# MichaelVorndran/InconsistencyMasks

Measured on AMD Instinct MI355X. Metric: images/sec per IM generation (ensemble infer + IM build + 1 train epoch), 256x256, higher is better.
Workload: dtype f16; 1 GPU; ISIC-2018 binary 256x256x3, 2-model IM ensemble, tiny U-Net alpha=0.5 on MI355X (configs[1]); outputs=1, unlabeled_images=2335, unlabeled_images_per_gpu=2335, labeled_images=259, n_models=2, infer_batch=584, infer_batch_rule=functions.infer_batch_size: 584 at alpha<=0.5 else 128; short tail spread, train_batch_per_gpu=32, global_batch=32, parallelism=dp1, epoch_steps=80, kept=2307, train_images=2566

## Files before the change

inconsistencymasks_amd/csrc/imk_conv.hip:

```cpp
#include <cstdlib>
#include "imk_kernels.h"
#include "imk_elem.h"

#include "imk_stage.h"
#include "imk_switches.h"

#ifndef IMK_INF_WAVES
#define IMK_INF_WAVES 4
#endif
IMK_STAMP_TABLE(conv)
IMK_WGSTAMP_TABLE(conv)

namespace {


struct ImkConvGeom { int tiles_x, tiles_y, mt_total, nc8, nc8p, n_pass, ps, nsp; unsigned magic_tx, magic_pi; };
__host__ __device__ inline size_t imk_chain_w2_offset(size_t stage1_bytes, size_t out_bytes) {
    return ((stage1_bytes > out_bytes ? stage1_bytes : out_bytes) + 15) & ~(size_t)15;
}

template <int TH, int MT, int LM, bool CHAIN = false>
__device__ __forceinline__ void conv_mfma_body(const ImkConvArgs &a, const ImkConvGeom &gm, int bx, int by) {
    const int tiles_x = gm.tiles_x, tiles_y = gm.tiles_y, mt_total = gm.mt_total, nc8 = gm.nc8, nc8p = gm.nc8p;
    const int n_pass = gm.n_pass, ps = gm.ps, nsp = gm.nsp;
    constexpr int NW = 4, NT = 64 * NW;
    constexpr int P = TH / NW;
    extern __shared__ __attribute__((aligned(16))) uint8_t smem[];
    const int ks3 = (a.ksize == 3);
    const int halo = ks3 ? 1 : 0;
    const int T = ks3 ? 9 : 1;
    const int HT = TH + 2 * halo, WT = TW + 2 * halo;
    uint8_t *s_tile = smem;
    float *s_aff = reinterpret_cast<float *>(smem + (size_t)HT * WT * ps * 16);
    f16 *s_w = reinterpret_cast<f16 *>(s_aff + 4 * a.x.cs_in);
    f16 *s_w2 = reinterpret_cast<f16 *>(smem + imk_chain_w2_offset((size_t)HT * WT * ps * 16 + 4 * (size_t)a.x.cs_in * sizeof(float) +
                                                                   (size_t)MT * nsp * 1024, (size_t)TH * 16 * (MT * 16 + 8) * sizeof(f16)));
    const int t = threadIdx.x;
    const int H = a.H, W = a.W;
    const int per_img = tiles_x * tiles_y;
    const int tb = gm.magic_pi ? (int)(((unsigned long long)(unsigned)bx * gm.magic_pi) >> 32) : bx / per_img;
    const PTile tc = ptile_at(tb, bx - tb * per_img, tiles_x, gm.magic_tx);
    const PSrc<LM> src = psrc_of<LM, 0>(a.x, tc, halo, HT, WT, H, W);
    const int ns_total = n_pass * nsp;

    IMK_STAMP_BEGIN(conv, 10000 + LM * 1000 + MT * 100 + n_pass * 10 + ks3);
    stage_affine_table(a.x, s_aff);
    bool aff_pending = (LM != LM_RAW && LM != LM_U8);

    const int lane = t & 63, wave = t >> 6, n = lane & 15, g = lane >> 4;
    const int ct0 = by * MT;
    int base[P];
#pragma unroll
    for (int p = 0; p < P; ++p) base[p] = ((wave * P + p) * WT + n) * ps * 16;
    f32x4 acc[MT][P];
#pragma unroll
    for (int m = 0; m < MT; ++m)
#pragma unroll
        for (int p = 0; p < P; ++p) acc[m][p] = f32x4{0, 0, 0, 0};
    for (int pass = 0; pass < n_pass; ++pass) {
        const int c8_lo = pass * nc8p;
        const int nc8_cur = min(nc8p, nc8 - c8_lo);
        if (pass) __syncthreads();
        {
            const int n16m = nsp * 64;
            if (CHAIN && pass == 0) {
                const int nc8_2 = a.cs_out / 8;
                const int n16 = ((a.cout2 + 15) / 16) * imk_cdiv_d(nc8_2, imk_pass_chunks(nc8_2)) * 64;
                for (int j = t; j < n16; j += NT)
                    __builtin_amdgcn_global_load_lds((const __attribute__((address_space(1))) void *)(a.wpk2 + (size_t)j * 8),
                                                     (__attribute__((address_space(3))) void *)(s_w2 + (size_t)(j - lane) * 8), 16, 0, 0);
            }
#pragma unroll
            for (int m = 0; m < MT; ++m) {
                int ct = by * MT + m;
                if (ct >= mt_total) ct = mt_total - 1;
                const f16 *src = a.wpk + ((size_t)ct * ns_total + (size_t)pass * nsp) * 512;
                f16 *dstm = s_w + (size_t)m * n16m * 8;
                for (int j = t; j < n16m; j += NT)
                    __builtin_amdgcn_global_load_lds((const __attribute__((address_space(1))) void *)(src + (size_t)j * 8),
                                                     (__attribute__((address_space(3))) void *)(dstm + (size_t)(j - lane) * 8), 16, 0, 0);
            }
        }
        const int n_items = HT * WT * nc8_cur;
        if constexpr (LM == LM_U8) {
            for (int i = t; i < n_items; i += NT) {
                const int pix = i / nc8_cur, c8 = i - pix * nc8_cur;
                const int py = pix / WT, px = pix - py * WT;
                const int y = tc.ty0 + py - halo, x = tc.tx0 + px - halo;
                f16x8 v = {0, 0, 0, 0, 0, 0, 0, 0};
                if (y >= 0 && y < H && x >= 0 && x < W) v = load_chunk(a.x, tc.b, y, x, H, W, c8_lo + c8, s_aff);
                *reinterpret_cast<f16x8 *>(s_tile + (pix * ps + c8) * 16) = v;
            }
        } else {
            constexpr int BATCH = 4;
            const int mg_c = (65536 + nc8_cur - 1) / nc8_cur, mg_w = (65536 + WT - 1) / WT;
            const int n_batches = (n_items + BATCH * NT - 1) / (BATCH * NT);
            for (int bt = 0; bt < n_batches; ++bt) {
                const int i0 = t + bt * BATCH * NT;
                RawChunk<LM> r[BATCH];
                int dst[BATCH], c8s[BATCH];
                unsigned ok = 0;
#pragma unroll
                for (int u = 0; u < BATCH; ++u) {
                    const int i = i0 + u * NT;
                    const int ii = i < n_items ? i : t;
                    const int pix = (ii * mg_c) >> 16;
                    const int c8 = ii - pix * nc8_cur;
                    const int py = (pix * mg_w) >> 16, px = pix - py * WT;
                    dst[u] = i < n_items ? (pix * ps + c8) * 16 : -1;
                    c8s[u] = c8_lo + c8;
                    if (psrc_load<LM, 0>(src, py, px, c8s[u], W, r[u])) ok |= 1u << u;
                }
                if (aff_pending) { __syncthreads(); aff_pending = false; }
#pragma unroll
                for (int u = 0; u < BATCH; ++u) {
                    if (dst[u] >= 0) {
                        f16x8 v = raw_transform<LM>(r[u], s_aff, a.x.cs_in, c8s[u], a.x.cin, a.x.u8_div);
                        if (!(ok & (1u << u))) v = f16x8{0, 0, 0, 0, 0, 0, 0, 0};
                        *reinterpret_cast<f16x8 *>(s_tile + dst[u]) = v;
                    }
                }
            }
        }
        __builtin_amdgcn_s_waitcnt(0x0F70);
        __syncthreads();
        if (pass == 0) IMK_STAMP(1);

        const int nq = T * nc8p;
        int q = g;
        const int mg_q = (65536 + nc8p - 1) / nc8p;
        auto k_loop = [&]() {
            int sn = 0;
            const f16 *wsrc[MT];
#pragma unroll
            for (int m = 0; m < MT; ++m) {
                wsrc[m] = s_w + ((size_t)m * nsp * 64 + lane) * 8;
            }
            typedef __attribute__((ext_vector_type(4))) unsigned u32x4;
            auto load_frag = [&](f16x8 (&af)[MT], f16x8 (&bf)[P]) {
                const int tap = (q * mg_q) >> 16, c8 = q - tap * nc8p;
                const int ty = ks3 ? (tap * 11) >> 5 : 0, tx = ks3 ? tap - 3 * ty : 0;
                const bool vq = (q < nq) && (c8 < nc8_cur);
                const int off = vq ? ((ty * WT + tx) * ps + c8) * 16 : 0;
                const unsigned live = sn < nsp ? 0xFFFFFFFFu : 0u;
                const int sc = min(sn, nsp - 1);
#pragma unroll
                for (int m = 0; m < MT; ++m) {
                    const u32x4 w = *reinterpret_cast<const u32x4 *>(wsrc[m] + (size_t)sc * 512) & live;
                    af[m] = __builtin_bit_cast(f16x8, w);
                }
#pragma unroll
                for (int p = 0; p < P; ++p) bf[p] = *reinterpret_cast<const f16x8 *>(s_tile + base[p] + off);
                ++sn;
                q += 4;
            };
            auto mma = [&](const f16x8 (&af)[MT], const f16x8 (&bf)[P]) {
#pragma unroll
                for (int p = 0; p < P; ++p)
#pragma unroll
                    for (int m = 0; m < MT; ++m) acc[m][p] = __builtin_amdgcn_mfma_f32_16x16x32_f16(af[m], bf[p], acc[m][p], 0, 0, 0);
            };
            f16x8 a0[MT], b0[P], a1[MT], b1[P];
            load_frag(a0, b0);
            for (int s = 0; s < nsp; s += 2) {
                load_frag(a1, b1);
                mma(a0, b0);
                load_frag(a0, b0);
                mma(a1, b1);
            }
        };
        k_loop();
        if (pass == 0) IMK_STAMP(2);
    }
    IMK_STAMP(3);

    const int x = tc.tx0 + n;
    const int my = H - 1 - tc.ty0, mx = W - 1 - tc.tx0;
    float s1[MT][4], s2[MT][4];
#pragma unroll
    for (int m = 0; m < MT; ++m)
#pragma unroll
        for (int r = 0; r < 4; ++r) s1[m][r] = s2[m][r] = 0.f;
    const bool dystat = !CHAIN && (a.epi != EP_RELU) && a.dystat_z && a.stats_partial;
    const bool want_stats = !CHAIN && (((a.epi == EP_RELU) && a.stats_partial) || dystat);
    float bias[MT][4];
#pragma unroll
    for (int m = 0; m < MT; ++m)
#pragma unroll
        for (int r = 0; r < 4; ++r) {
            const int co = (ct0 + m) * 16 + 4 * g + r;
            bias[m][r] = (a.epi == EP_RELU && a.bias && co < a.cout) ? a.bias[co] : 0.f;
        }
    constexpr int OPITCH = MT * 16 + 8;
    f16 *s_out = reinterpret_cast<f16 *>(smem);
    __syncthreads();
    auto write_tile = [&](auto EPI_T, auto STAT_T, const f32x4 (&ac)[MT][P], const float (&bs)[MT][4], int cs_o) {
        constexpr int EPI = decltype(EPI_T)::value;
        constexpr int STAT = decltype(STAT_T)::value;
#pragma unroll
        for (int m = 0; m < MT; ++m) {
            const int co0 = (ct0 + m) * 16 + 4 * g;
            f16x4 mk[P], zz[P];
            if (EPI == EP_MASK || STAT == 2) {
#pragma unroll
                for (int p = 0; p < P; ++p) {
                    const unsigned o = __umul24(__umul24(min(wave * P + p, my), W) + min(n, mx), (unsigned)cs_o * 2u) + (co0 < cs_o ? co0 * 2 : 0);
                    if (EPI == EP_MASK) mk[p] = *reinterpret_cast<const f16x4 *>(pix_base(a.mask, tc.b, H, W, tc.ty0, tc.tx0, (unsigned)cs_o * 2u) + o);
                    if (STAT == 2) zz[p] = *reinterpret_cast<const f16x4 *>(pix_base(a.dystat_z, tc.b, H, W, tc.ty0, tc.tx0, (unsigned)cs_o * 2u) + o);
                }
            }
#pragma unroll
            for (int p = 0; p < P; ++p) {
                f16x4 v;
#pragma unroll
                for (int r = 0; r < 4; ++r) {
                    if (EPI == EP_RELU) v[r] = (f16)fmaxf(ac[m][p][r] + bs[m][r], 0.f);
                    else if (EPI == EP_MASK) v[r] = ((float)mk[p][r] > 0.f) ? (f16)ac[m][p][r] : (f16)0.f;
                    else v[r] = (f16)ac[m][p][r];
                }
                *reinterpret_cast<f16x4 *>(s_out + ((wave * P + p) * 16 + n) * OPITCH + m * 16 + 4 * g) = v;
                if (STAT) {
                    const int y = tc.ty0 + wave * P + p;
                    const float live = (co0 < cs_o && y < H && x < W) ? 1.f : 0.f;
#pragma unroll
                    for (int r = 0; r < 4; ++r) {
                        const float f = live * (float)v[r];
                        s1[m][r] += f;
                        s2[m][r] += f * (STAT == 2 ? (float)zz[p][r] : f);
                    }
                }
            }
        }
    };
    auto copy_out = [&](f16 *out, int cs_o) {
        const int cpp = MT * 2;
        const int n_live = min(cpp, (cs_o - ct0 * 16) / 8);
        char *ob = const_cast<char *>(pix_base(out, tc.b, H, W, tc.ty0, tc.tx0, (unsigned)cs_o * 2u)) + ct0 * 32;
        for (int i = t; i < TH * 16 * cpp; i += NT) {
            const int pixl = i / cpp, ch = i - pixl * cpp;
            const int py = pixl >> 4, px = pixl & 15;
            if (ch < n_live && py <= my && px <= mx)
                *reinterpret_cast<f16x8 *>(ob + __umul24(__umul24(py, W) + px, (unsigned)cs_o * 2u) + ch * 16) =
                    *reinterpret_cast<const f16x8 *>(s_out + pixl * OPITCH + ch * 8);
        }
    };
    auto reduce_stats = [&](int cs_o) {
        __syncthreads();
        float *s_red = reinterpret_cast<float *>(smem);
#pragma unroll
        for (int m = 0; m < MT; ++m)
#pragma unroll
            for (int r = 0; r < 4; ++r) {
                const float v1 = wave_sum<16>(s1[m][r]), v2 = wave_sum<16>(s2[m][r]);
                if (n == 0) {
                    s_red[(wave * 2 + 0) * 16 * MT + m * 16 + 4 * g + r] = v1;
                    s_red[(wave * 2 + 1) * 16 * MT + m * 16 + 4 * g + r] = v2;
                }
            }
        __syncthreads();
        if (t < 2 * 16 * MT) {
            const int which = t / (16 * MT), c = t - which * 16 * MT;
            const int co = ct0 * 16 + c;
            if (co < cs_o) {
                float v = 0.f;
#pragma unroll
                for (int w = 0; w < NW; ++w) v += s_red[(w * 2 + which) * 16 * MT + c];
                a.stats_partial[(size_t)bx * 2 * cs_o + which * cs_o + co] = v;
            }
        }
    };
    using I0 = std::integral_constant<int, 0>; using I1 = std::integral_constant<int, 1>; using I2 = std::integral_constant<int, 2>;
    if constexpr (CHAIN) {
        write_tile(I0{}, I0{}, acc, bias, a.cs_out);
        const int nc8_2 = a.cs_out / 8, nc8p2 = imk_pass_chunks(nc8_2), ns2 = imk_cdiv_d(nc8_2, nc8p2);
        const int mt2 = (a.cout2 + 15) / 16;
        f32x4 acc2[MT][P];
#pragma unroll
        for (int m = 0; m < MT; ++m)
#pragma unroll
            for (int p = 0; p < P; ++p) acc2[m][p] = f32x4{0, 0, 0, 0};
        float bias2[MT][4];
#pragma unroll
        for (int m = 0; m < MT; ++m)
#pragma unroll
            for (int r = 0; r < 4; ++r) {
                const int co = m * 16 + 4 * g + r;
                bias2[m][r] = co < a.cout2 ? a.bias2[co] : 0.f;
            }
        for (int s2i = 0; s2i < ns2; ++s2i) {
            const int c8 = s2i * nc8p2 + g;
            const int off = (g < nc8p2 && c8 < nc8_2) ? c8 * 8 : 0;
            f16x8 bf[P];
#pragma unroll
            for (int p = 0; p < P; ++p) bf[p] = *reinterpret_cast<const f16x8 *>(s_out + ((wave * P + p) * 16 + n) * OPITCH + off);
#pragma unroll
            for (int m = 0; m < MT; ++m) {
                if (m < mt2) {
                    const f16x8 af = *reinterpret_cast<const f16x8 *>(s_w2 + ((size_t)(m * ns2 + s2i) * 64 + lane) * 8);
#pragma unroll
                    for (int p = 0; p < P; ++p) acc2[m][p] = __builtin_amdgcn_mfma_f32_16x16x32_f16(af, bf[p], acc2[m][p], 0, 0, 0);
                }
            }
        }
        if (a.out) {
            __syncthreads();
            copy_out(a.out, a.cs_out);
            __syncthreads();
        }
        IMK_STAMP(4);
        if (a.stats_partial) write_tile(I0{}, I1{}, acc2, bias2, a.cs_out2); else write_tile(I0{}, I0{}, acc2, bias2, a.cs_out2);
        __syncthreads();
        copy_out(a.out2, a.cs_out2);
        IMK_STAMP(5);
        if (a.stats_partial) reduce_stats(a.cs_out2);
    } else {
        if (a.epi == EP_RELU) { if (want_stats) write_tile(I0{}, I1{}, acc, bias, a.cs_out); else write_tile(I0{}, I0{}, acc, bias, a.cs_out); }
        else if (a.epi == EP_MASK) { if (dystat) write_tile(I2{}, I2{}, acc, bias, a.cs_out); else write_tile(I2{}, I0{}, acc, bias, a.cs_out); }
        else { if (dystat) write_tile(I1{}, I2{}, acc, bias, a.cs_out); else write_tile(I1{}, I0{}, acc, bias, a.cs_out); }
        __syncthreads();
        IMK_STAMP(4);
        copy_out(a.out, a.cs_out);
        IMK_STAMP(5);
        if (want_stats) reduce_stats(a.cs_out);
    }
    IMK_STAMP_END(6);
}

template <int TH, int MT, int LM, bool CHAIN = false>
__global__ __launch_bounds__(256) void conv_mfma_kernel(ImkConvArgs a, ImkConvGeom gm) {
    conv_mfma_body<TH, MT, LM, CHAIN>(a, gm, blockIdx.x, blockIdx.y);
}

constexpr size_t pipe_lds_base(int nc8, bool pair, int wg) {
    size_t b = (size_t)18 * 18 * imk_lds_pitch(nc8) * 16 + (8 * 16 + 4 * 2 * 16) * sizeof(float) + 1024 +
               ((wg && wg != 4) ? (size_t)(wg == 3 ? 18 * 18 : 256) * ((pair ? 1 : 2) | 1) * 16 + 64 : 0);
    if (wg == 3 && b < 4 * 5 * 256 * sizeof(float)) b = 4 * 5 * 256 * sizeof(float);
    return (b + 15) & ~(size_t)15;
}

template <int LM, int NC8, int CHAIN, bool PAIR, int EPI, bool DYSTAT, bool FULL, int WG = 0, int PRE = 0, bool DYN = false>
__global__ __launch_bounds__(256, (DYN && NC8 == 1) ? IMK_INF_WAVES : 1) void conv_pipe_kernel(ImkConvArgs a, int tiles_x, int tiles_y, int n_tiles,
                                                        unsigned magic_tx, ImkWalk wk) {
    static_assert(!DYN || (EPI == EP_RELU && !DYSTAT && WG == 0), "dynamic walk: results must not depend on the tile -> workgroup map");
    static_assert(PRE == 0 || (WG == 0 && EPI == EP_RELU && !DYSTAT && (LM == LM_U8 || LM == LM_UPADD)), "pre-stage: inference forward only");
    static_assert(WG != 1 || (LM == LM_BNBWD && CHAIN == 0 && EPI == EP_MASK && !DYSTAT && FULL), "fused wgrad: 1x1 dgrad behind a BatchNorm");
    static_assert(WG != 2 || (LM == LM_RAW && CHAIN == 0 && EPI == EP_PLAIN && DYSTAT && FULL), "fused wgrad: 1x1 dgrad in front of a BatchNorm");
    static_assert(WG != 3 || (LM == LM_RAW && CHAIN == 0 && EPI == EP_PLAIN && DYSTAT && FULL), "fused wgrad: 3x3 dgrad in front of a BatchNorm");
    static_assert(WG != 4 || (LM == LM_BNBWD && CHAIN == 0 && EPI == EP_PLAIN && !DYSTAT && FULL && PRE == 0), "2x2-sum epilogue: 1x1 dgrad of a decoder's first conv");
    constexpr int P = PAIR ? 2 : 4;
    constexpr int PS = imk_lds_pitch(NC8);
    constexpr int NCI = PRE ? PRE : NC8;
    constexpr int PSI = imk_lds_pitch(NCI);
    constexpr int MAX_ITEMS = (18 * 18 * NCI + 255) / 256;
    constexpr int MAX_NS = PAIR ? 3 * NC8 : (9 * NC8 + 3) / 4;
    extern __shared__ __attribute__((aligned(16))) uint8_t smem[];
    const int ks3 = (a.ksize == 3);
    const int halo = ks3 ? 1 : 0;
    const int HT = 16 + 2 * halo, WT = TW + 2 * halo;
    const int n_items = HT * WT * NCI;
    const bool shared_taps = PAIR && ks3;
    const int nq = (shared_taps ? 12 : (ks3 ? 9 : 1)) * NC8, ns = shared_taps ? 3 * NC8 : (PAIR ? (nq + 1) / 2 : (nq + 3) / 4);
    uint8_t *s_tile = smem;
    uint8_t *s_t0 = smem + pipe_lds_base(NC8, PAIR, WG);
    float *s_pre = reinterpret_cast<float *>(s_t0 + 18 * 18 * PSI * 16);
    uint8_t *s_stage = PRE ? s_t0 : s_tile;
    float *s_aff = reinterpret_cast<float *>(smem + 18 * 18 * PS * 16);
    float *s_red = s_aff + 8 * 16;
    const int t = threadIdx.x;
    IMK_STAMP_BEGIN(conv, 40000 + LM * 1000 + WG * 100 + CHAIN * 10 + (DYSTAT ? 1 : 0));
    IMK_WGSTAMP_BEGIN(conv, 40000 + LM * 1000 + WG * 100 + CHAIN * 10 + (DYSTAT ? 1 : 0));
    const int lane = t & 63, wave = t >> 6, n = lane & 15, g = lane >> 4;
    const int set = PAIR ? (g >> 1) : 0;
    const int H = a.H, W = a.W;
    constexpr int cs_in = NCI * 8;
    const int per_img = tiles_x * tiles_y;
    auto tile_row = [&](int p) { return wave * 4 + (PAIR ? 2 * p + set : p); };
    constexpr unsigned CSB = NCI * 16;

    f16x8 af[MAX_NS];
    int off[MAX_NS];
#pragma unroll
    for (int s = 0; s < MAX_NS; ++s) {
        const int q = (PAIR && !shared_taps) ? 2 * s + (g & 1) : 4 * s + g;
        const bool vq = (s < ns) && (q < nq);
        const int tap = q / NC8, c8 = q - tap * NC8;
        const int ty = ks3 ? tap / 3 : 0, tx = ks3 ? tap - 3 * (tap / 3) : 0;
        off[s] = vq ? ((ty * WT + tx) * PS + c8) * 16 : 0;
        af[s] = (s < ns) ? *reinterpret_cast<const f16x8 *>(a.wpk + ((size_t)s * 64 + lane) * 8) : f16x8{0, 0, 0, 0, 0, 0, 0, 0};
    }
    int base[P];
#pragma unroll
    for (int p = 0; p < P; ++p) base[p] = ((shared_taps ? wave * 4 + 2 * p : tile_row(p)) * WT + n) * PS * 16;
    int it_lds[MAX_ITEMS], it_py[MAX_ITEMS], it_px[MAX_ITEMS], it_c8[MAX_ITEMS];
#pragma unroll
    for (int k = 0; k < MAX_ITEMS; ++k) {
        const int i = t + 256 * k;
        const bool live = i < n_items;
        const int pix = (live ? i : t % n_items) / NCI;
        it_c8[k] = (live ? i : t % n_items) - pix * NCI;
        it_py[k] = pix / WT;
        it_px[k] = pix - it_py[k] * WT;
        it_lds[k] = live ? (pix * PSI + it_c8[k]) * 16 : -1;
    }
    float bias[4] = {0, 0, 0, 0}, bias2[4] = {0, 0, 0, 0};
    const int co0 = PAIR ? 4 * (g & 1) : 4 * g;
    if (EPI == EP_RELU && a.bias)
#pragma unroll
        for (int r = 0; r < 4; ++r) bias[r] = (co0 + r < a.cout) ? a.bias[co0 + r] : 0.f;
    f16x8 af2 = {0, 0, 0, 0, 0, 0, 0, 0};
    if (CHAIN) {
        af2 = *reinterpret_cast<const f16x8 *>(a.wpk2 + (size_t)lane * 8);
#pragma unroll
        for (int r = 0; r < 4; ++r) bias2[r] = (co0 + r < a.cout2) ? a.bias2[co0 + r] : 0.f;
    }
    const bool want_stats = DYSTAT || WG == 4 || ((EPI == EP_RELU) && a.stats_partial);
    constexpr int NJ = PAIR ? 3 : 6;
    f16x8 af_pre = {0, 0, 0, 0, 0, 0, 0, 0};
    int pre_pix[PRE ? NJ : 1], pre_yx[PRE ? NJ : 1];
    const int pre_c8 = PAIR ? (g & 1) : g;
    const int pre_cb = PAIR ? 4 * (g & 1) : 4 * g;
    if constexpr (PRE) {
        af_pre = *reinterpret_cast<const f16x8 *>(a.pre_wpk + (size_t)lane * 8);
        if (t < 16) {
            s_pre[t] = t < a.pre_cout ? a.pre_bias[t] : 0.f;
            s_pre[16 + t] = t < NC8 * 8 ? a.pre_sc[t] : 0.f;
            s_pre[32 + t] = t < NC8 * 8 ? a.pre_sh[t] : 0.f;
        }
        const int n_pix = HT * WT;
#pragma unroll
        for (int j = 0; j < NJ; ++j) {
            const int grp = wave * NJ + j;
            const int px = min(PAIR ? (grp * 2 + (g >> 1)) * 16 + n : grp * 16 + n, n_pix - 1);
            const int py = px / WT;
            pre_pix[j] = px;
            pre_yx[j] = (py << 8) | (px - py * WT);
        }
    }
    const bool lane_out = FULL || co0 < (CHAIN ? a.cs_out2 : a.cs_out);
    const bool lane_mid = FULL || co0 < a.cs_out;

    float s1[4] = {0, 0, 0, 0}, s2[4] = {0, 0, 0, 0};
    RawChunk<LM> raw[MAX_ITEMS];
    unsigned valid = 0;
    constexpr bool U8ROWS = (LM == LM_U8) && FULL && !PRE;
    uint8_t *s_u8 = reinterpret_cast<uint8_t *>(s_red + 4 * 2 * 16);
    constexpr int NCX = PAIR ? 1 : 2, XS = NCX | 1;
    uint8_t *s_x = s_u8 + 1024;
    constexpr int MAX_XI = WG == 3 ? (18 * 18 * NCX + 255) / 256 : NCX;
    f16x8 xr[MAX_XI];
    unsigned xvalid = 0;
    int xi_lds[MAX_XI], xi_py[MAX_XI], xi_px[MAX_XI], xi_c8[MAX_XI];
    if constexpr (WG == 3) {
#pragma unroll
        for (int k = 0; k < MAX_XI; ++k) {
            const int i = t + 256 * k;
            const bool live = i < 18 * 18 * NCX;
            const int ii = live ? i : t;
            const int pix = ii / NCX;
            xi_c8[k] = ii - pix * NCX;
            xi_py[k] = pix / 18;
            xi_px[k] = pix - xi_py[k] * 18;
            xi_lds[k] = live ? (pix * XS + xi_c8[k]) * 16 : -1;
        }
    }
    f32x4 wacc = {0, 0, 0, 0}, bacc = {0, 0, 0, 0};
    f32x4 wtap[WG == 3 ? 9 : 1];
#pragma unroll
    for (int i = 0; i < (WG == 3 ? 9 : 1); ++i) wtap[i] = f32x4{0, 0, 0, 0};
    float x_sc = 0.f, x_sh = 0.f;
    if constexpr (WG == 2) { if (n < a.cs_out) { x_sc = a.wg_sc[n]; x_sh = a.wg_sh[n]; } }
    uint4 rowseg = {0, 0, 0, 0};
    const int u8_cin = a.x.cin, u8_nseg = 16 * u8_cin;
    const int u8_t = t < u8_nseg ? t : 0;
    const int u8_row = u8_t / u8_cin, u8_seg = u8_t - u8_row * u8_cin;
    const unsigned u8_off = (unsigned)(u8_row * W * u8_cin + u8_seg * 16);
    const unsigned cso_b = (unsigned)a.cs_out * 2u;
    const unsigned xw_off = (unsigned)((t >> 4) * W + (t & 15)) * cso_b;
    auto issue = [&](const PTile &tc) {
        if constexpr (U8ROWS) {
            rowseg = *reinterpret_cast<const uint4 *>(pix_base(a.x.in, tc.b, H, W, tc.ty0, tc.tx0, (unsigned)u8_cin) + u8_off);
            return;
        }
        const PSrc<LM> src = psrc_of<LM, CSB>(a.x, tc, halo, HT, WT, H, W);
        valid = 0;
#pragma unroll
        for (int k = 0; k < MAX_ITEMS; ++k) {
            const bool in_img = psrc_load<LM, CSB>(src, it_py[k], it_px[k], it_c8[k], W, raw[k]);
            valid |= ((it_lds[k] >= 0 && in_img) ? 1u : 0u) << k;
        }
        if constexpr (WG == 1 || WG == 2) {
            const char *px = pix_base(WG == 1 ? a.mask : a.dystat_z, tc.b, H, W, tc.ty0, tc.tx0, cso_b) + xw_off;
#pragma unroll
            for (int q = 0; q < NCX; ++q) xr[q] = *reinterpret_cast<const f16x8 *>(px + q * 16);
        }
        if constexpr (WG == 3) {
            const char *bz = pix_base(a.dystat_z, tc.b, H, W, src.oy, src.ox, cso_b);
            xvalid = 0;
#pragma unroll
            for (int k = 0; k < MAX_XI; ++k) {
                const int ry = min(max(xi_py[k], src.lo_y), src.hi_y), rx = min(max(xi_px[k], src.lo_x), src.hi_x);
                const bool ok = xi_lds[k] >= 0 && ry == xi_py[k] && rx == xi_px[k];
                xr[k] = *reinterpret_cast<const f16x8 *>(bz + __umul24(__umul24(ry, W) + rx, cso_b) + xi_c8[k] * 16);
                xvalid |= (ok ? 1u : 0u) << k;
            }
        }
    };
    const unsigned cso2_b = CHAIN ? (unsigned)a.cs_out2 * 2u : 0u;
    unsigned o1c[P], o2c[P];
#pragma unroll
    for (int p = 0; p < P; ++p) {
        const unsigned lp = (unsigned)(tile_row(p) * W + n);
        o1c[p] = lp * cso_b + co0 * 2;
        o2c[p] = lp * cso2_b + co0 * 2;
    }

    const int wgrp = imk_walk_range(wk, blockIdx.x);
    int tile = wgrp * wk.chunk + (int)(blockIdx.x >> wk.shift);
    const int tile_end = min(n_tiles, (wgrp + 1) * wk.chunk);
    const int tile0 = min(tile, n_tiles - 1);
    PTile tc = ptile_at(tile0 / per_img, tile0 % per_img, tiles_x, magic_tx);
    issue(tc);
    __shared__ int s_tk[2];
    const bool tk_lane = DYN && t == 0;
    unsigned *const tk_head = DYN ? a.sched + wgrp * (IMK_SCHED_STRIDE / 4) : nullptr;
    const int tk_base = wgrp * wk.chunk + wk.step;
    int it_par = 0, tk_pending = 0;
    if constexpr (DYN) {
        const int tk = imk_take_ticket(tk_head, tk_lane);
        tk_pending = imk_take_ticket(tk_head, tk_lane);
        if (tk_lane) s_tk[0] = tk;
    }
    stage_affine_table(a.x, s_aff);
    if constexpr (WG == 3) {
        if (t < a.cs_out) { s_aff[t] = a.wg_sc[t]; s_aff[16 + t] = a.wg_sh[t]; }
    }
    __builtin_amdgcn_s_waitcnt(0x0F70);
    __syncthreads();
    while (tile < tile_end) {
        if constexpr (U8ROWS) {
            if (t < u8_nseg) *reinterpret_cast<uint4 *>(s_u8 + t * 16) = rowseg;
            __syncthreads();
            const uint8_t *pb = s_u8 + (t >> 4) * u8_nseg + (t & 15) * u8_cin;
            f16x8 v;
#pragma unroll
            for (int j = 0; j < 8; ++j) v[j] = (f16)((j < 4 && j < u8_cin) ? (float)pb[j] / a.x.u8_div : 0.0f);
            *reinterpret_cast<f16x8 *>(s_tile + it_lds[0]) = v;
        } else {
#pragma unroll
            for (int k = 0; k < MAX_ITEMS; ++k) {
                if (it_lds[k] >= 0) {
                    f16x8 v = raw_transform<LM>(raw[k], s_aff, cs_in, it_c8[k], a.x.cin, a.x.u8_div, a.x.u8_c);
                    if (!(valid & (1u << k))) v = f16x8{0, 0, 0, 0, 0, 0, 0, 0};
                    *reinterpret_cast<f16x8 *>(s_stage + it_lds[k]) = v;
                }
            }
            if constexpr (WG == 1 || WG == 2) {
#pragma unroll
                for (int q = 0; q < NCX; ++q) *reinterpret_cast<f16x8 *>(s_x + (t * XS + q) * 16) = xr[q];
            }
            if constexpr (WG == 3) {
#pragma unroll
                for (int k = 0; k < MAX_XI; ++k) {
                    if (xi_lds[k] >= 0) {
                        f16x8 v = affine8(xr[k], s_aff + xi_c8[k] * 8, s_aff + 16 + xi_c8[k] * 8);
                        if (!(xvalid & (1u << k))) v = f16x8{0, 0, 0, 0, 0, 0, 0, 0};
                        *reinterpret_cast<f16x8 *>(s_x + xi_lds[k]) = v;
                    }
                }
            }
        }
        __syncthreads();
        const char *b_o1 = pix_base(a.out, tc.b, H, W, tc.ty0, tc.tx0, cso_b);
        const char *b_o2 = CHAIN ? pix_base(a.out2, tc.b, H, W, tc.ty0, tc.tx0, cso2_b) : nullptr;
        const char *b_mk = (EPI == EP_MASK && WG != 1) ? pix_base(a.mask, tc.b, H, W, tc.ty0, tc.tx0, cso_b) : nullptr;
        const char *b_zq = (DYSTAT && WG != 2) ? pix_base(a.dystat_z, tc.b, H, W, tc.ty0, tc.tx0, cso_b) : nullptr;
        unsigned o1[P], o1l[P], o2[P];
        bool inb[P];
#pragma unroll
        for (int p = 0; p < P; ++p) {
            if constexpr (FULL) {
                o1[p] = o1l[p] = o1c[p]; o2[p] = o2c[p]; inb[p] = true;
            } else {
                const int my = H - 1 - tc.ty0, mx = W - 1 - tc.tx0, r = tile_row(p);
                inb[p] = r <= my && n <= mx;
                const unsigned lp = __umul24(min(r, my), W) + min(n, mx);
                const unsigned ob = __umul24(lp, cso_b);
                o1[p] = ob + co0 * 2;
                o1l[p] = ob + (lane_out ? co0 * 2 : 0);
                o2[p] = __umul24(lp, cso2_b) + co0 * 2;
            }
        }
        f16x4 mk[P], zq[P];
        if (EPI == EP_MASK) {
#pragma unroll
            for (int p = 0; p < P; ++p) {
                if constexpr (WG == 1) mk[p] = *reinterpret_cast<const f16x4 *>(s_x + ((tile_row(p) * 16 + n) * XS) * 16 + co0 * 2);
                else mk[p] = *reinterpret_cast<const f16x4 *>(b_mk + o1l[p]);
            }
        }
        if (DYSTAT) {
#pragma unroll
            for (int p = 0; p < P; ++p) {
                if constexpr (WG == 2) zq[p] = *reinterpret_cast<const f16x4 *>(s_x + ((tile_row(p) * 16 + n) * XS) * 16 + co0 * 2);
                else zq[p] = *reinterpret_cast<const f16x4 *>(b_zq + o1l[p]);
            }
        }
        constexpr int NQ = PAIR ? P : P / 2;
        f16x4 zlo[WG == 4 ? NQ : 1];
        unsigned olo[WG == 4 ? NQ : 1];
        const char *b_lo = nullptr;
        if constexpr (WG == 4) {
            const char *bz = pix_base(a.sum2_z, tc.b, H >> 1, W >> 1, tc.ty0 >> 1, tc.tx0 >> 1, cso_b);
            b_lo = pix_base(a.sum2_out, tc.b, H >> 1, W >> 1, tc.ty0 >> 1, tc.tx0 >> 1, cso_b);
#pragma unroll
            for (int q = 0; q < NQ; ++q) {
                olo[q] = (unsigned)((wave * 2 + q) * (W >> 1) + (n >> 1)) * cso_b + co0 * 2;
                zlo[q] = *reinterpret_cast<const f16x4 *>(bz + olo[q]);
            }
        }
        int next;
        PTile tn;
        int tk_new = 0;
        if constexpr (DYN) {
            next = tk_base + __builtin_amdgcn_readfirstlane(s_tk[it_par]);
            tn = next < tile_end ? ptile_of_index(next, per_img, tiles_x, magic_tx, wk.magic_pi) : tc;
        } else {
            next = tile + wk.step;
            tn = next < tile_end ? ptile_next(tc, wk.q, wk.r, per_img, tiles_x, magic_tx) : tc;
        }
        issue(tn);
        if constexpr (DYN) tk_new = imk_take_ticket(tk_head, tk_lane);
        if constexpr (PRE) {
            const int oy = tc.ty0 - halo, ox = tc.tx0 - halo;
            const int lo_y = oy < 0 ? -oy : 0, hi_y = min(HT - 1, H - 1 - oy), lo_x = ox < 0 ? -ox : 0, hi_x = min(WT - 1, W - 1 - ox);
            const f32x4 pb = *reinterpret_cast<const f32x4 *>(s_pre + pre_cb), psc = *reinterpret_cast<const f32x4 *>(s_pre + 16 + pre_cb),
                        psh = *reinterpret_cast<const f32x4 *>(s_pre + 32 + pre_cb);
#pragma unroll
            for (int j = 0; j < NJ; ++j) {
                const f16x8 bfp = *reinterpret_cast<const f16x8 *>(s_t0 + (pre_pix[j] * PSI + (pre_c8 < NCI ? pre_c8 : 0)) * 16);
                const f32x4 pa = __builtin_amdgcn_mfma_f32_16x16x32_f16(af_pre, bfp, f32x4{0, 0, 0, 0}, 0, 0, 0);
                const int py = pre_yx[j] >> 8, px = pre_yx[j] & 255;
                const bool inside = py >= lo_y && py <= hi_y && px >= lo_x && px <= hi_x;
                const float pbv[4] = {pb[0], pb[1], pb[2], pb[3]};
                const f16x4 z4 = imk_bias_relu4(pa, pbv);
                unsigned wd[2];
#pragma unroll
                for (int r = 0; r < 4; r += 2) {
                    const f16x2 z2 = {z4[r], z4[r + 1]};
                    const f16x2 w2 = imk_affine2(z2, f32x2{psc[r], psc[r + 1]}, f32x2{psh[r], psh[r + 1]});
                    wd[r >> 1] = inside ? __builtin_bit_cast(unsigned, w2) : 0u;
                }
                const f16x4 w = __builtin_bit_cast(f16x4, uint2{wd[0], wd[1]});
                if (pre_cb < NC8 * 8)
                    *reinterpret_cast<f16x4 *>(s_tile + (pre_pix[j] * PS + (pre_cb >> 3)) * 16 + (pre_cb & 7) * 2) = w;
            }
            __syncthreads();
        }
        if constexpr (WG == 3) {
            const int qq = n >> 2, pp = n & 3;
            f16x8 ones;
#pragma unroll
            for (int j = 0; j < 8; ++j) ones[j] = (f16)(n == 0 ? 1.0f : 0.0f);
#pragma unroll
            for (int kk = 0; kk < 2; ++kk) {
                const int row = wave * 4 + 2 * kk + (g >> 1), xx = 4 * (g & 1) + qq;
                const uint8_t *pb = s_tile + (size_t)((row + 1) * 18 + xx + 1) * PS * 16 + pp * 8;
                const h4 b0 = __builtin_amdgcn_ds_read_tr16_b64_v4f16(LDS_PTR(h4, pb));
                const h4 b1 = __builtin_amdgcn_ds_read_tr16_b64_v4f16(LDS_PTR(h4, pb + 8 * PS * 16));
                f16x8 bfw;
#pragma unroll
                for (int e = 0; e < 4; ++e) { bfw[e] = (f16)b0[e]; bfw[4 + e] = (f16)b1[e]; }
                const uint8_t *pa = s_x + (size_t)(row * 18 + xx) * XS * 16 + pp * 8;
#pragma unroll
                for (int tap = 0; tap < 9; ++tap) {
                    const uint8_t *p = pa + (size_t)((tap / 3) * 18 + tap % 3) * XS * 16;
                    const h4 a0 = __builtin_amdgcn_ds_read_tr16_b64_v4f16(LDS_PTR(h4, p));
                    const h4 a1 = __builtin_amdgcn_ds_read_tr16_b64_v4f16(LDS_PTR(h4, p + 8 * XS * 16));
                    f16x8 afw;
#pragma unroll
                    for (int e = 0; e < 4; ++e) { afw[e] = (f16)a0[e]; afw[4 + e] = (f16)a1[e]; }
                    wtap[tap] = __builtin_amdgcn_mfma_f32_16x16x32_f16(afw, bfw, wtap[tap], 0, 0, 0);
                }
                bacc = __builtin_amdgcn_mfma_f32_16x16x32_f16(ones, bfw, bacc, 0, 0, 0);
            }
        }
        if constexpr (WG == 1 || WG == 2) {
            const int qq = n >> 2, pp = n & 3;
            f16x8 ones;
#pragma unroll
            for (int j = 0; j < 8; ++j) ones[j] = (f16)(n == 0 ? 1.0f : 0.0f);
#pragma unroll
            for (int kk = 0; kk < 2; ++kk) {
                const int pi = (wave * 4 + 2 * kk + (g >> 1)) * 16 + 4 * (g & 1) + qq;
                const uint8_t *pb = s_tile + (size_t)pi * PS * 16 + pp * 8;
                const uint8_t *pa = s_x + (size_t)pi * XS * 16 + pp * 8;
                const h4 b0 = __builtin_amdgcn_ds_read_tr16_b64_v4f16(LDS_PTR(h4, pb));
                const h4 b1 = __builtin_amdgcn_ds_read_tr16_b64_v4f16(LDS_PTR(h4, pb + 8 * PS * 16));
                const h4 a0 = __builtin_amdgcn_ds_read_tr16_b64_v4f16(LDS_PTR(h4, pa));
                const h4 a1 = __builtin_amdgcn_ds_read_tr16_b64_v4f16(LDS_PTR(h4, pa + 8 * XS * 16));
                f16x8 bfw, afw;
#pragma unroll
                for (int e = 0; e < 4; ++e) { bfw[e] = (f16)b0[e]; bfw[4 + e] = (f16)b1[e]; afw[e] = (f16)a0[e]; afw[4 + e] = (f16)a1[e]; }
                if constexpr (WG == 2) {
#pragma unroll
                    for (int e = 0; e < 8; e += 2) {
                        const f16x2 r2 = imk_affine2(f16x2{afw[e], afw[e + 1]}, f32x2{x_sc, x_sc}, f32x2{x_sh, x_sh});
                        afw[e] = r2[0]; afw[e + 1] = r2[1];
                    }
                }
                wacc = __builtin_amdgcn_mfma_f32_16x16x32_f16(afw, bfw, wacc, 0, 0, 0);
                bacc = __builtin_amdgcn_mfma_f32_16x16x32_f16(ones, bfw, bacc, 0, 0, 0);
            }
        }
        f32x4 acc[P];
#pragma unroll
        for (int p = 0; p < P; ++p) acc[p] = f32x4{0, 0, 0, 0};
#pragma unroll
        for (int s = 0; s < MAX_NS; ++s) {
            if (s < ns) {
#pragma unroll
                for (int p = 0; p < P; ++p) {
                    const f16x8 bf = *reinterpret_cast<const f16x8 *>(s_tile + base[p] + off[s]);
                    acc[p] = __builtin_amdgcn_mfma_f32_16x16x32_f16(af[s], bf, acc[p], 0, 0, 0);
                }
            }
        }
        if (CHAIN) {
#pragma unroll
            for (int p = 0; p < P; ++p) {
                const f16x4 hv = imk_bias_relu4(acc[p], bias);
                if (CHAIN == 1 && (FULL || inb[p]) && lane_mid) *reinterpret_cast<f16x4 *>(const_cast<char *>(b_o1) + o1[p]) = hv;
                const f16x8 bf2 = {hv[0], hv[1], hv[2], hv[3], 0, 0, 0, 0};
                const f32x4 a2 = __builtin_amdgcn_mfma_f32_16x16x32_f16(af2, bf2, f32x4{0, 0, 0, 0}, 0, 0, 0);
                const f16x4 v = imk_bias_relu4(a2, bias2);
                if ((FULL || inb[p]) && lane_out) {
                    *reinterpret_cast<f16x4 *>(const_cast<char *>(b_o2) + o2[p]) = v;
                    if (want_stats)
#pragma unroll
                        for (int r = 0; r < 4; ++r) { const float f = (float)v[r]; s1[r] += f; s2[r] += f * f; }
                }
            }
        } else {
            float hsum[WG == 4 ? P : 1][4];
#pragma unroll
            for (int p = 0; p < P; ++p) {
                f16x4 v;
                if (EPI == EP_RELU) {
                    v = imk_bias_relu4(acc[p], bias);
                } else if (EPI == EP_MASK) {
#pragma unroll
                    for (int r = 0; r < 4; ++r) v[r] = ((float)mk[p][r] > 0.f) ? (f16)acc[p][r] : (f16)0.f;
                } else {
#pragma unroll
                    for (int r = 0; r < 4; ++r) v[r] = (f16)acc[p][r];
                }
                if ((FULL || inb[p]) && lane_out) {
                    *reinterpret_cast<f16x4 *>(const_cast<char *>(b_o1) + o1[p]) = v;
                    if (DYSTAT) {
#pragma unroll
                        for (int r = 0; r < 4; ++r) { const float f = (float)v[r]; s1[r] += f; s2[r] += f * (float)zq[p][r]; }
                    } else if (WG != 4 && want_stats) {
#pragma unroll
                        for (int r = 0; r < 4; ++r) { const float f = (float)v[r]; s1[r] += f; s2[r] += f * f; }
                    }
                }
                if constexpr (WG == 4) {
#pragma unroll
                    for (int r = 0; r < 4; ++r) { const float f = (float)v[r]; hsum[p][r] = f + __shfl_xor(f, 1, 64); }
                }
            }
            if constexpr (WG == 4) {
#pragma unroll
                for (int q = 0; q < NQ; ++q) {
                    f16x4 d;
#pragma unroll
                    for (int r = 0; r < 4; ++r) {
                        const float tot = PAIR ? hsum[q][r] + __shfl_xor(hsum[q][r], 32, 64) : hsum[2 * q][r] + hsum[2 * q + 1][r];
                        d[r] = (f16)tot;
                    }
                    if ((n & 1) == 0 && (!PAIR || set == 0)) {
                        *reinterpret_cast<f16x4 *>(const_cast<char *>(b_lo) + olo[q]) = d;
#pragma unroll
                        for (int r = 0; r < 4; ++r) { const float f = (float)d[r]; s1[r] += f; s2[r] += f * (float)zlo[q][r]; }
                    }
                }
            }
        }
        if constexpr (DYN) { it_par ^= 1; if (tk_lane) s_tk[it_par] = tk_pending; tk_pending = tk_new; }
        __syncthreads();
        tile = next;
        tc = tn;
    }
    if constexpr (WG == 3) {
        float *s_acc = reinterpret_cast<float *>(smem);
        float *dst = a.wg_partial + (size_t)blockIdx.x * 10 * 256;
#pragma unroll
        for (int rd = 0; rd < 2; ++rd) {
            __syncthreads();
#pragma unroll
            for (int i = 0; i < 5; ++i) {
                const f32x4 v = (rd * 5 + i < 9) ? wtap[(rd * 5 + i) % 9] : bacc;
#pragma unroll
                for (int r = 0; r < 4; ++r) s_acc[(wave * 5 + i) * 256 + r * 64 + lane] = v[r];
            }
            __syncthreads();
#pragma unroll
            for (int i = 0; i < 5; ++i)
                dst[(rd * 5 + i) * 256 + t] = s_acc[(0 * 5 + i) * 256 + t] + s_acc[(1 * 5 + i) * 256 + t] + s_acc[(2 * 5 + i) * 256 + t] +
                                              s_acc[(3 * 5 + i) * 256 + t];
        }
        __syncthreads();
    }
    if constexpr (WG == 1 || WG == 2) {
        float *s_acc = reinterpret_cast<float *>(smem);
#pragma unroll
        for (int r = 0; r < 4; ++r) {
            s_acc[(wave * 2 + 0) * 256 + r * 64 + lane] = wacc[r];
            s_acc[(wave * 2 + 1) * 256 + r * 64 + lane] = bacc[r];
        }
        __syncthreads();
        float *dst = a.wg_partial + (size_t)blockIdx.x * 2 * 256;
#pragma unroll
        for (int i = 0; i < 2; ++i)
            dst[i * 256 + t] = s_acc[(0 * 2 + i) * 256 + t] + s_acc[(1 * 2 + i) * 256 + t] + s_acc[(2 * 2 + i) * 256 + t] +
                               s_acc[(3 * 2 + i) * 256 + t];
        __syncthreads();
    }
    if (want_stats) {
#pragma unroll
        for (int r = 0; r < 4; ++r) {
            const float v1 = wave_sum<16>(s1[r]), v2 = wave_sum<16>(s2[r]);
            if (n == 0) { s_red[(wave * 2 + 0) * 16 + 4 * g + r] = v1; s_red[(wave * 2 + 1) * 16 + 4 * g + r] = v2; }
        }
        __syncthreads();
        if (t < 32) {
            const int which = t >> 4, c = t & 15;
            const int cs_st = CHAIN ? a.cs_out2 : a.cs_out;
            if (c < cs_st) {
                float v = (s_red[(0 * 2 + which) * 16 + c] + s_red[(1 * 2 + which) * 16 + c]) +
                          (s_red[(2 * 2 + which) * 16 + c] + s_red[(3 * 2 + which) * 16 + c]);
                if (PAIR) v += (s_red[(0 * 2 + which) * 16 + c + 8] + s_red[(1 * 2 + which) * 16 + c + 8]) +
                               (s_red[(2 * 2 + which) * 16 + c + 8] + s_red[(3 * 2 + which) * 16 + c + 8]);
                a.stats_partial[(size_t)blockIdx.x * 2 * cs_st + which * cs_st + c] = v;
            }
        }
    }
    IMK_WGSTAMP_END();
    IMK_STAMP_END(1);
}

template <int LM, int NC8, int MT, int EPI, bool DYSTAT, bool FULL, bool CHAIN2 = false>
__global__ __launch_bounds__(256) void conv_wide_kernel(ImkConvArgs a, int tiles_x, int tiles_y, int n_tiles,
                                                        unsigned magic_tx, ImkWalk wk) {
    constexpr int P = 4;
    constexpr int PS = imk_lds_pitch(NC8);
    constexpr int MAX_ITEMS = (18 * 18 * NC8 + 255) / 256;
    constexpr int MAX_NS = (9 * NC8 + 3) / 4;
    extern __shared__ __attribute__((aligned(16))) uint8_t smem[];
    const int ks3 = (a.ksize == 3);
    const int halo = ks3 ? 1 : 0;
    const int HT = 16 + 2 * halo, WT = TW + 2 * halo;
    const int n_items = HT * WT * NC8;
    const int nq = (ks3 ? 9 : 1) * NC8, ns = (nq + 3) / 4;
    uint8_t *s_tile = smem;
    float *s_aff = reinterpret_cast<float *>(smem + 18 * 18 * PS * 16);
    float *s_red = s_aff + 4 * 32;
    f16 *s_w = reinterpret_cast<f16 *>(s_red + 4 * 2 * 16 * MT);
    constexpr int MIDP = 48;
    const int t = threadIdx.x;
    f16 *s_mid = s_w + (size_t)MT * ns * 512 + (t >> 6) * 64 * MIDP;
    IMK_STAMP_BEGIN(conv, 50000 + LM * 1000 + MT * 10 + (DYSTAT ? 1 : 0));
    const int lane = t & 63, wave = t >> 6, n = lane & 15, g = lane >> 4;
    const int H = a.H, W = a.W;
    const int cs_in = a.x.cs_in;
    const int per_img = tiles_x * tiles_y;

    int off[MAX_NS];
#pragma unroll
    for (int s = 0; s < MAX_NS; ++s) {
        const int q = 4 * s + g;
        const bool vq = (s < ns) && (q < nq);
        const int tap = q / NC8, c8 = q - tap * NC8;
        const int ty = ks3 ? tap / 3 : 0, tx = ks3 ? tap - 3 * (tap / 3) : 0;
        off[s] = vq ? ((ty * WT + tx) * PS + c8) * 16 : 0;
    }
    int base[P];
#pragma unroll
    for (int p = 0; p < P; ++p) base[p] = ((wave * 4 + p) * WT + n) * PS * 16;
    int it_lds[MAX_ITEMS], it_py[MAX_ITEMS], it_px[MAX_ITEMS], it_c8[MAX_ITEMS];
#pragma unroll
    for (int k = 0; k < MAX_ITEMS; ++k) {
        const int i = t + 256 * k;
        const bool live = i < n_items;
        const int pix = (live ? i : t % n_items) / NC8;
        it_c8[k] = (live ? i : t % n_items) - pix * NC8;
        it_py[k] = pix / WT;
        it_px[k] = pix - it_py[k] * WT;
        it_lds[k] = live ? (pix * PS + it_c8[k]) * 16 : -1;
    }
    {
        const int n16 = MT * ns * 64;
        const int mt_have = (a.cout + 15) / 16;
        for (int j = t; j < n16; j += 256) {
            const int m = j / (ns * 64);
            f16x8 v = {0, 0, 0, 0, 0, 0, 0, 0};
            if (m < mt_have) v = *reinterpret_cast<const f16x8 *>(a.wpk + (size_t)j * 8);
            *reinterpret_cast<f16x8 *>(s_w + (size_t)j * 8) = v;
        }
    }
    float bias[MT][4];
#pragma unroll
    for (int m = 0; m < MT; ++m)
#pragma unroll
        for (int r = 0; r < 4; ++r) {
            const int co = 16 * m + 4 * g + r;
            bias[m][r] = (EPI == EP_RELU && a.bias && co < a.cout) ? a.bias[co] : 0.f;
        }
    const bool want_stats = DYSTAT || ((EPI == EP_RELU) && a.stats_partial);
    const int cs_st = CHAIN2 ? a.cs_out2 : a.cs_out;
    bool lane_out[MT];
#pragma unroll
    for (int m = 0; m < MT; ++m) lane_out[m] = 16 * m + 4 * g < a.cs_out;
    f16x8 a2[2] = {f16x8{0, 0, 0, 0, 0, 0, 0, 0}, f16x8{0, 0, 0, 0, 0, 0, 0, 0}};
    float bias2[2][4] = {{0.f, 0.f, 0.f, 0.f}, {0.f, 0.f, 0.f, 0.f}};
    bool lane_out2[2] = {false, false};
    const unsigned cso2_b = CHAIN2 ? (unsigned)a.cs_out2 * 2u : 0u;
    if constexpr (CHAIN2) {
#pragma unroll
        for (int m = 0; m < 2; ++m) {
            if (16 * m < a.cout2) a2[m] = *reinterpret_cast<const f16x8 *>(a.wpk2 + ((size_t)m * 64 + lane) * 8);
            lane_out2[m] = 16 * m + 4 * g < a.cs_out2;
#pragma unroll
            for (int r = 0; r < 4; ++r) { const int co = 16 * m + 4 * g + r; bias2[m][r] = co < a.cout2 ? a.bias2[co] : 0.f; }
        }
    }

    float s1[MT][4], s2[MT][4];
#pragma unroll
    for (int m = 0; m < MT; ++m)
#pragma unroll
        for (int r = 0; r < 4; ++r) s1[m][r] = s2[m][r] = 0.f;
    RawChunk<LM> raw[MAX_ITEMS];
    unsigned valid = 0;
    constexpr unsigned CSB = NC8 * 16;
    auto issue = [&](const PTile &tc) {
        const PSrc<LM> src = psrc_of<LM, CSB>(a.x, tc, halo, HT, WT, H, W);
        valid = 0;
#pragma unroll
        for (int k = 0; k < MAX_ITEMS; ++k) {
            const bool in_img = psrc_load<LM, CSB>(src, it_py[k], it_px[k], it_c8[k], W, raw[k]);
            valid |= ((it_lds[k] >= 0 && in_img) ? 1u : 0u) << k;
        }
    };
    const unsigned cso_b = (unsigned)a.cs_out * 2u;
    unsigned o1c[P];
#pragma unroll
    for (int p = 0; p < P; ++p) o1c[p] = (unsigned)((wave * 4 + p) * W + n) * cso_b;

    const int wgrp = imk_walk_range(wk, blockIdx.x);
    int tile = wgrp * wk.chunk + (int)(blockIdx.x >> wk.shift);
    const int tile_end = min(n_tiles, (wgrp + 1) * wk.chunk);
    const int tile0 = min(tile, n_tiles - 1);
    PTile tc = ptile_at(tile0 / per_img, tile0 % per_img, tiles_x, magic_tx);
    issue(tc);
    stage_affine_table(a.x, s_aff);
    __builtin_amdgcn_s_waitcnt(0x0F70);
    __syncthreads();
    while (tile < tile_end) {
#pragma unroll
        for (int k = 0; k < MAX_ITEMS; ++k) {
            if (it_lds[k] >= 0) {
                f16x8 v = raw_transform<LM>(raw[k], s_aff, cs_in, it_c8[k], a.x.cin, a.x.u8_div);
                if (!(valid & (1u << k))) v = f16x8{0, 0, 0, 0, 0, 0, 0, 0};
                *reinterpret_cast<f16x8 *>(s_tile + it_lds[k]) = v;
            }
        }
        __syncthreads();
        const char *b_o1 = CHAIN2 ? pix_base(a.out2, tc.b, H, W, tc.ty0, tc.tx0, cso2_b) : pix_base(a.out, tc.b, H, W, tc.ty0, tc.tx0, cso_b);
        const char *b_mk = EPI == EP_MASK ? pix_base(a.mask, tc.b, H, W, tc.ty0, tc.tx0, cso_b) : nullptr;
        const char *b_zq = DYSTAT ? pix_base(a.dystat_z, tc.b, H, W, tc.ty0, tc.tx0, cso_b) : nullptr;
        unsigned o1[P];
        unsigned o_mid[P];
        const char *b_mid = (CHAIN2 && a.out) ? pix_base(a.out, tc.b, H, W, tc.ty0, tc.tx0, cso_b) : nullptr;
        bool inb[P];
#pragma unroll
        for (int p = 0; p < P; ++p) {
            if constexpr (FULL) {
                o1[p] = CHAIN2 ? (unsigned)((wave * 4 + p) * W + n) * cso2_b : o1c[p]; inb[p] = true;
                o_mid[p] = o1c[p];
            } else {
                const int my = H - 1 - tc.ty0, mx = W - 1 - tc.tx0, r = wave * 4 + p;
                inb[p] = r <= my && n <= mx;
                o1[p] = __umul24(__umul24(min(r, my), W) + min(n, mx), CHAIN2 ? cso2_b : cso_b);
                o_mid[p] = __umul24(__umul24(min(r, my), W) + min(n, mx), cso_b);
            }
        }
        f16x4 mk[MT][P], zq[MT][P];
        if (EPI == EP_MASK) {
#pragma unroll
            for (int m = 0; m < MT; ++m)
#pragma unroll
                for (int p = 0; p < P; ++p) mk[m][p] = *reinterpret_cast<const f16x4 *>(b_mk + o1[p] + (lane_out[m] ? 32 * m + 8 * g : 0));
        }
        if (DYSTAT) {
#pragma unroll
            for (int m = 0; m < MT; ++m)
#pragma unroll
                for (int p = 0; p < P; ++p) zq[m][p] = *reinterpret_cast<const f16x4 *>(b_zq + o1[p] + (lane_out[m] ? 32 * m + 8 * g : 0));
        }
        const int next = tile + wk.step;
        const PTile tn = next < tile_end ? ptile_next(tc, wk.q, wk.r, per_img, tiles_x, magic_tx) : tc;
        issue(tn);
        f32x4 acc[MT][P];
#pragma unroll
        for (int m = 0; m < MT; ++m)
#pragma unroll
            for (int p = 0; p < P; ++p) acc[m][p] = f32x4{0, 0, 0, 0};
#pragma unroll
        for (int s = 0; s < MAX_NS; ++s) {
            if (s < ns) {
                f16x8 afm[MT];
#pragma unroll
                for (int m = 0; m < MT; ++m) afm[m] = *reinterpret_cast<const f16x8 *>(s_w + ((size_t)(m * ns + s) * 64 + lane) * 8);
#pragma unroll
                for (int p = 0; p < P; ++p) {
                    const f16x8 bf = *reinterpret_cast<const f16x8 *>(s_tile + base[p] + off[s]);
#pragma unroll
                    for (int m = 0; m < MT; ++m) acc[m][p] = __builtin_amdgcn_mfma_f32_16x16x32_f16(afm[m], bf, acc[m][p], 0, 0, 0);
                }
            }
        }
        if constexpr (CHAIN2) {
#pragma unroll
            for (int p = 0; p < P; ++p) {
#pragma unroll
                for (int m = 0; m < 2; ++m) {
                    f16x4 v = {0, 0, 0, 0};
                    if (m < MT) {
#pragma unroll
                        for (int r = 0; r < 4; ++r) v[r] = (f16)fmaxf(acc[m < MT ? m : 0][p][r] + bias[m < MT ? m : 0][r], 0.f);
                    }
                    *reinterpret_cast<f16x4 *>(s_mid + (p * 16 + n) * MIDP + 16 * m + 4 * g) = v;
// ... 497 lines not shown
    }
    IMK_STAMP_END(1);
}

}

int imk_wgf_add_job(ImkWgFinalJobs &jobs, float *partial, int n_split, int ksize, int cin, int cout, float *dw, float *db) {
    if (jobs.n >= IMK_WGF_MAX_JOBS) return IMK_EUNSUPPORTED;
    const int T = ksize == 3 ? 9 : 1;
    const int cit_n = (imk_pad8(cin) + 15) / 16, cot_n = (imk_pad8(cout) + 15) / 16;
    ImkWgFinalJob &jb = jobs.j[jobs.n++];
    jb.partial = partial;
    jb.n_split = n_split;
    jb.chunk = WG_RED_CHUNK;
    while (imk_cdiv(n_split, jb.chunk) > 64) jb.chunk *= 2;
    jb.n_chunks = imk_cdiv(n_split, jb.chunk);
    jb.n_tiles = cit_n * cot_n * (T + 1);
    jb.red = partial + (size_t)n_split * jb.n_tiles * 256;
    jb.T = T; jb.cin = cin; jb.cout = cout; jb.cot_n = cot_n;
    jb.dw = dw; jb.db = db;
    jb.work1_begin = jobs.total_work1;
    jb.tile_begin = jobs.total_tiles;
    jobs.total_work1 += jb.n_tiles * jb.n_chunks;
    jobs.total_tiles += jb.n_tiles;
    return IMK_OK;
}

int imk_launch_wgrad_finalize_jobs(const ImkWgFinalJobs &jobs, const float *inv_scale_ptr, float *found_inf, hipStream_t stream) {
    if (jobs.n <= 0) return IMK_OK;
    double wgf_bytes = 0;
    for (int i = 0; i < jobs.n; ++i)
        wgf_bytes += ((double)jobs.j[i].n_split + 2.0 * jobs.j[i].n_chunks + 1.0) * jobs.j[i].n_tiles * 256 * 4;
    ImkProfScope prof(PF_WGF, wgf_bytes, stream);
    double b1 = 0, b2 = 0;
    for (int i = 0; i < jobs.n; ++i) {
        b1 += ((double)jobs.j[i].n_split + jobs.j[i].n_chunks) * jobs.j[i].n_tiles * 256 * 4;
        b2 += ((double)jobs.j[i].n_chunks + 1.0) * jobs.j[i].n_tiles * 256 * 4;
    }
    imk_prof_work(b1);
    imk_klaunch(wgf_stage1_kernel, dim3(jobs.total_work1), dim3(256), 0, stream, jobs);
    IMK_LAUNCH_CHECK();
    imk_prof_work(b2);
    imk_klaunch(wgf_stage2_kernel, dim3(jobs.total_tiles), dim3(1024), 0, stream, jobs, inv_scale_ptr, found_inf);
    IMK_LAUNCH_CHECK();
    return IMK_OK;
}

int imk_launch_pack_jobs(const ImkPackJobs &jobs, hipStream_t stream) {
    if (jobs.n <= 0) return IMK_OK;
    double pk_bytes = 0;
    for (int i = 0; i < jobs.n; ++i) pk_bytes += (double)jobs.j[i].ksize * jobs.j[i].ksize * jobs.j[i].cin * jobs.j[i].cout * 6;
    ImkProfScope prof(PF_STEP_TAIL, pk_bytes, stream);
    long long widest = 0;
    for (int i = 0; i < jobs.n; ++i) {
        const long long slots = (long long)jobs.j[i].ksize * jobs.j[i].ksize * ((jobs.j[i].cin + 15) & ~15) * ((jobs.j[i].cout + 15) & ~15);
        widest = slots > widest ? slots : widest;
    }
    int bpj = (int)((widest + 2047) / 2048);
    bpj = bpj < 64 ? 64 : (bpj > 1024 ? 1024 : bpj);
    imk_klaunch(pack_conv_batched_kernel, dim3(dim3(bpj, jobs.n)), dim3(256), 0, stream, jobs);
    IMK_LAUNCH_CHECK();
    return IMK_OK;
}

static inline int odd_ps(int nc8) { return imk_lds_pitch(nc8); }

static inline int conv_tile_h(int cs_in, int ksize) {
    const int halo = ksize == 3 ? 1 : 0;
    const size_t b16 = (size_t)(16 + 2 * halo) * (TW + 2 * halo) * odd_ps(imk_pass_chunks(cs_in / 8)) * 16;
    return b16 > 64 * 1024 ? 8 : 16;
}

int imk_conv_num_tiles(int B, int H, int W, int cs_in, int ksize) {
    const int per_tile = B * imk_cdiv(H, conv_tile_h(cs_in, ksize)) * imk_cdiv(W, TW);
    const int gemm = imk_conv_gemm_num_tiles(B, H, W);
    return per_tile > gemm ? per_tile : gemm;
}

#include <algorithm>
#include <cstdio>
#include <cstring>
#include <cxxabi.h>
#include <map>
#include <mutex>
#include <new>
#include <string>
#include <unordered_map>
#include <vector>
namespace {
struct ProfRec { hipEvent_t e0, e1; int variant; double bytes, flops; };
struct ProfTot { long long launches = 0; double bytes = 0, flops = 0; };
const char *const kFamilyNames[PF_COUNT] = {
    "conv_mfma_kernel<16, 1>", "conv_mfma_kernel<16, 2>", "conv_mfma_kernel<16, 4>", "conv_mfma_kernel<8, 1>", "conv_mfma_kernel<8, 2>",
    "conv_mfma_kernel<8, 4>", "conv_pipe_kernel", "wgrad_mfma_kernel", "bn_bwd_prep_kernel", "bn_bwd_coef_kernel", "bn_finalize_kernel",
    "wgf_stage1+2_kernel", "head_kernel", "head_loss_kernel", "step_tail", "im_kernel", "conv_gemm_kernel", "wgrad_gemm_kernel"};
__global__ void imk_mark_kernel(int id) { (void)id; }
}
struct imk_prof {
    int period = 0;
    long counter = 0;
    std::vector<ProfRec> recs;
    std::vector<hipEvent_t> pool;
    bool totals_on = false;
    std::map<std::string, ProfTot> totals;
    hipEvent_t event() {
        if (!pool.empty()) { hipEvent_t e = pool.back(); pool.pop_back(); return e; }
        hipEvent_t e;
        (void)hipEventCreate(&e);
        return e;
    }
};
static thread_local imk_prof *t_prof = nullptr;

extern "C" int imk_prof_create(int period, imk_prof **out) {
    IMK_CHECK_ARG(out && period >= 0);
    imk_prof *p = new (std::nothrow) imk_prof();
    if (!p) return IMK_EINVAL;
    p->period = period;
    *out = p;
    return IMK_OK;
}
extern "C" void imk_prof_destroy(imk_prof *p) {
    if (!p) return;
    if (t_prof == p) { t_prof = nullptr; imk_tls_totals_on = false; }
    for (auto &r : p->recs) { (void)hipEventDestroy(r.e0); (void)hipEventDestroy(r.e1); }
    for (auto e : p->pool) (void)hipEventDestroy(e);
    delete p;
}
extern "C" int imk_prof_bind(imk_prof *p) { t_prof = p; imk_tls_totals_on = p && p->totals_on; return IMK_OK; }
extern "C" int imk_prof_unbind(imk_prof *p) { if (p && t_prof == p) { t_prof = nullptr; imk_tls_totals_on = false; return 1; } return 0; }
extern "C" int imk_prof_set_period(imk_prof *p, int period) { IMK_CHECK_ARG(p && period >= 0); p->period = period; return IMK_OK; }

static const std::string &kernel_short_name(const void *kern, hipStream_t stream) {
    static std::mutex mu;
    static std::unordered_map<const void *, std::string> names;
    std::lock_guard<std::mutex> lk(mu);
    auto it = names.find(kern);
    if (it != names.end()) return it->second;
    std::string n = "?";
    if (const char *m = hipKernelNameRefByPtr(kern, stream)) {
        int st = 0;
        char *d = abi::__cxa_demangle(m, nullptr, nullptr, &st);
        n = (st == 0 && d) ? d : m;
        free(d);
        if (st != 0) {
            const char *tag = "_ZN12_GLOBAL__N_1";
            const size_t at = n.find(tag);
            if (at != std::string::npos) {
                size_t i = at + strlen(tag), len = 0;
                while (i < n.size() && n[i] >= '0' && n[i] <= '9') len = 10 * len + (size_t)(n[i++] - '0');
                if (len > 0 && i + len <= n.size()) n = n.substr(i, len);
            }
        }
        for (const char *drop : {"void ", "(anonymous namespace)::"})
            for (size_t at; (at = n.find(drop)) != std::string::npos;) n.erase(at, strlen(drop));
        int depth = 0;
        for (size_t i = 0; i < n.size(); ++i) {
            if (n[i] == '<') ++depth;
            else if (n[i] == '>') --depth;
            else if (n[i] == '(' && depth == 0) { n.resize(i); break; }
        }
        if (n.size() > 90) n.resize(90);
    }
    return names.emplace(kern, n).first->second;
}
static thread_local struct { double bytes, flops; bool armed; } t_work = {0.0, 0.0, false};
void imk_prof_work(double bytes, double flops) { t_work.bytes = bytes; t_work.flops = flops; t_work.armed = true; }
void imk_prof_note_launch(const void *kern, hipStream_t stream) {
    imk_prof *p = t_prof;
    if (!p || !p->totals_on) return;
    ProfTot &t = p->totals[kernel_short_name(kern, stream)];
    t.launches += 1;
    if (t_work.armed) { t.bytes += t_work.bytes; t.flops += t_work.flops; t_work.armed = false; }
}

int imk_prof_begin(int family, double bytes, hipStream_t stream, double flops, const char *variant) {
    imk_prof *p = t_prof;
    (void)variant;
    if (p && p->totals_on && family >= 0 && family < PF_COUNT) imk_prof_work(bytes, flops);
    if (!p || p->period <= 0 || (p->counter++ % p->period) != 0) return -1;
    ProfRec pr{p->event(), p->event(), family, bytes, flops};
    if (hipEventRecord(pr.e0, stream) != hipSuccess) { p->pool.push_back(pr.e0); p->pool.push_back(pr.e1); return -1; }
    p->recs.push_back(pr);
    return (int)p->recs.size() - 1;
}
void imk_prof_end(int slot, hipStream_t stream) {
    imk_prof *p = t_prof;
    if (p && slot >= 0 && slot < (int)p->recs.size()) (void)hipEventRecord(p->recs[slot].e1, stream);
}

extern "C" int imk_prof_totals_enable(imk_prof *p, int on) {
    IMK_CHECK_ARG(p);
    p->totals.clear();
    p->totals_on = on != 0;
    if (t_prof == p) imk_tls_totals_on = p->totals_on;
    t_work.armed = false;
    return IMK_OK;
}
extern "C" int64_t imk_prof_totals_dump(imk_prof *p, char *buf, int64_t cap) {
    if (!p) return IMK_EINVAL;
    std::string out;
    char line[160];
    for (auto &kv : p->totals) {
        snprintf(line, sizeof line, ";%lld;%.0f;%.0f\n", kv.second.launches, kv.second.bytes, kv.second.flops);
        out += kv.first; out += line;
    }
    if (buf && cap > 0) {
        const size_t n = std::min((size_t)cap - 1, out.size());
        memcpy(buf, out.data(), n);
        buf[n] = 0;
    }
    return (int64_t)out.size() + 1;
}
extern "C" int imk_prof_mark(int id, void *stream) {
    IMK_CHECK_ARG(id > 0 && id < 65536);
    imk_klaunch(imk_mark_kernel, dim3(id), dim3(64), 0, (hipStream_t)stream, id);
    IMK_LAUNCH_CHECK();
    return IMK_OK;
}

extern "C" int imk_prof_collect(imk_prof *p, int64_t *count, double *ms, double *bytes, double *flops) {
    IMK_CHECK_ARG(p && count && ms && bytes);
    static_assert(IMK_PROF_VARIANTS == PF_COUNT, "include/imk.h and imk_common.h disagree");
    for (int v = 0; v < IMK_PROF_VARIANTS; ++v) { count[v] = 0; ms[v] = 0; bytes[v] = 0; if (flops) flops[v] = 0; }
    for (auto &r : p->recs) {
        float t = 0.f;
        if (hipEventSynchronize(r.e1) == hipSuccess && hipEventElapsedTime(&t, r.e0, r.e1) == hipSuccess) {
            count[r.variant] += 1; ms[r.variant] += t; bytes[r.variant] += r.bytes;
            if (flops) flops[r.variant] += r.flops;
        }
        p->pool.push_back(r.e0); p->pool.push_back(r.e1);
    }
    p->recs.clear();
    return IMK_OK;
}

static inline unsigned div_magic(int d) { return d > 1 ? (unsigned)((1ull << 32) / (unsigned)d + 1) : 0u; }

struct ConvLaunch { ImkConvGeom gm; int th, mt; int gx, gy; size_t lds; };

static int plan_conv_mfma(const ImkConvArgs &a, ConvLaunch &L) {
    const int TH = conv_tile_h(a.x.cs_in, a.ksize);
    const int halo = a.ksize == 3 ? 1 : 0;
    const int nc8 = a.x.cs_in / 8;
    const int nc8p = imk_pass_chunks(nc8), n_pass = imk_cdiv_d(nc8, nc8p);
    const int ps = odd_ps(nc8p);
    const int T = a.ksize == 3 ? 9 : 1;
    const int nsp = (T * nc8p + 3) / 4;
    const int mt_total = (a.cout + 15) / 16;
    const int tiles_x = imk_cdiv(a.W, TW), tiles_y = imk_cdiv(a.H, TH);
    const size_t tile_bytes = (size_t)(TH + 2 * halo) * (TW + 2 * halo) * ps * 16;
    const size_t stats_bytes = 4 * 2 * 16 * 4 * sizeof(float);
    size_t lds = tile_bytes + 4 * (size_t)a.x.cs_in * sizeof(float);
    if (lds < stats_bytes) lds = stats_bytes;
    const size_t lds_base = lds;
    const int n_sp = a.B * tiles_x * tiles_y;
    int mt = mt_total >= 4 ? 4 : (mt_total >= 2 ? 2 : 1);
    while (mt > 1 && n_sp * imk_cdiv(mt_total, mt) < 512) mt >>= 1;
    if (a.wpk2) {
        const int mt2 = (a.cout2 + 15) / 16;
        mt = (mt_total <= 2 && mt2 <= 2) ? 2 : 4;
        if (mt_total > mt || mt2 > mt || TH != 16) return IMK_EUNSUPPORTED;
    }
    lds = lds_base + (size_t)mt * nsp * 1024;
    const size_t out_bytes = (size_t)TH * 16 * (mt * 16 + 8) * sizeof(f16);
    if (a.wpk2) {
        const int nc8_2 = a.cs_out / 8;
        lds = imk_chain_w2_offset(lds_base + (size_t)mt * nsp * 1024, out_bytes) +
              (size_t)((a.cout2 + 15) / 16) * imk_cdiv_d(nc8_2, imk_pass_chunks(nc8_2)) * 1024;
    }
    if (lds < out_bytes) lds = out_bytes;
    if (lds > 160 * 1024) return IMK_EUNSUPPORTED;
    if (!((long long)a.H * a.W < imk_conv_max_pixels() && a.W < (1 << 16))) return IMK_EUNSUPPORTED;
    const long long per_img = (long long)tiles_x * tiles_y;
    L.gm = ImkConvGeom{tiles_x, tiles_y, mt_total, nc8, nc8p, n_pass, ps, nsp, div_magic(tiles_x),
                       (per_img > 1 && (long long)n_sp * per_img < (1ll << 32)) ? div_magic((int)per_img) : 0u};
    L.th = TH; L.mt = mt; L.gx = n_sp; L.gy = imk_cdiv(mt_total, mt); L.lds = lds;
    return IMK_OK;
}

template <typename K>
static int set_lds_limit(K kern, size_t lds) {
    if (lds > 64 * 1024)
        IMK_HIP(hipFuncSetAttribute(reinterpret_cast<const void *>(kern), hipFuncAttributeMaxDynamicSharedMemorySize, (int)lds));
    return IMK_OK;
}

static int launch_conv_mfma(const ImkConvArgs &a, hipStream_t stream) {
    ConvLaunch L{};
    int rc = plan_conv_mfma(a, L);
    if (rc) return rc;
    const dim3 grid(L.gx, L.gy);
    auto launch = [&](auto kern) -> int {
        int r = set_lds_limit(kern, L.lds);
        if (r) return r;
        imk_klaunch(kern, dim3(grid), dim3(256), L.lds, stream, a, L.gm);
        return IMK_OK;
    };
    ImkProfScope prof(PF_CONV_MFMA + (L.th == 8 ? 3 : 0) + (L.mt == 4 ? 2 : (L.mt == 2 ? 1 : 0)), imk_conv_algorithmic_bytes(a), stream, imk_conv_flops(a));
    if (a.wpk2) {
        if (L.gy != 1 || L.th != 16) return IMK_EUNSUPPORTED;
        if (a.x.lmode == LM_POOL) rc = L.mt == 4 ? launch(conv_mfma_kernel<16, 4, LM_POOL, true>) : launch(conv_mfma_kernel<16, 2, LM_POOL, true>);
        else if (a.x.lmode == LM_AFFINE) rc = L.mt == 4 ? launch(conv_mfma_kernel<16, 4, LM_AFFINE, true>) : launch(conv_mfma_kernel<16, 2, LM_AFFINE, true>);
        else return IMK_EUNSUPPORTED;
        if (rc) return rc;
        if (a.stats_rows) *a.stats_rows = L.gx;
        IMK_LAUNCH_CHECK();
        return IMK_OK;
    }
#define IMK_MFMA_MT(TH, LM) \
    (L.mt == 4 ? launch(conv_mfma_kernel<TH, 4, LM>) : (L.mt == 2 ? launch(conv_mfma_kernel<TH, 2, LM>) : launch(conv_mfma_kernel<TH, 1, LM>)))
#define IMK_MFMA_TH(LM) (L.th == 16 ? IMK_MFMA_MT(16, LM) : IMK_MFMA_MT(8, LM))
    switch (a.x.lmode) {
        case LM_RAW: rc = IMK_MFMA_TH(LM_RAW); break;
        case LM_AFFINE: rc = IMK_MFMA_TH(LM_AFFINE); break;
        case LM_POOL: rc = IMK_MFMA_TH(LM_POOL); break;
        case LM_UPADD: rc = IMK_MFMA_TH(LM_UPADD); break;
        case LM_BNBWD: rc = IMK_MFMA_TH(LM_BNBWD); break;
        default: rc = IMK_MFMA_TH(LM_U8); break;
    }
#undef IMK_MFMA_TH
#undef IMK_MFMA_MT
    if (rc) return rc;
    if (a.stats_rows) *a.stats_rows = L.gx;
    IMK_LAUNCH_CHECK();
    return IMK_OK;
}

static bool pipe_fits(const ImkConvArgs &a) { return (long long)a.H * a.W < imk_conv_max_pixels() && a.W < (1 << 16); }


constexpr int PIPE_BLOCKS_PER_CU = 8;

template <int LM, int NC8, int CHAIN, bool PAIR, int EPI, bool DYSTAT, bool FULL, int WG = 0, int PRE = 0, bool DYN = false>
static int launch_conv_pipe_k(const ImkConvArgs &a, hipStream_t stream) {
    if constexpr (!DYN && EPI == EP_RELU && !DYSTAT && WG == 0) {
        if (a.sched && !a.stats_partial && a.B * imk_cdiv(a.H, 16) * imk_cdiv(a.W, TW) >= 2048)
            return launch_conv_pipe_k<LM, NC8, CHAIN, PAIR, EPI, DYSTAT, FULL, WG, PRE, true>(a, stream);
    }
    if (a.x.cs_in != (PRE ? PRE : NC8) * 8) return IMK_EINVAL;
    static int blocks_per_cu = 0;
    const size_t lds = pipe_lds_base(NC8, PAIR, WG) + (PRE ? (size_t)18 * 18 * imk_lds_pitch(PRE) * 16 + 3 * 16 * sizeof(float) : 0);
    auto kern = conv_pipe_kernel<LM, NC8, CHAIN, PAIR, EPI, DYSTAT, FULL, WG, PRE, DYN>;
    if (blocks_per_cu == 0) {
        int nb = 0;
        if (hipOccupancyMaxActiveBlocksPerMultiprocessor(&nb, kern, 256, lds) != hipSuccess || nb < 1) nb = 4;
        blocks_per_cu = nb > PIPE_BLOCKS_PER_CU ? PIPE_BLOCKS_PER_CU : nb;
    }
    const int tiles_x = imk_cdiv(a.W, TW), tiles_y = imk_cdiv(a.H, 16);
    const int n_tiles = a.B * tiles_x * tiles_y;
    int grid = 256 * blocks_per_cu;
    if (grid > n_tiles) grid = n_tiles;
    const ImkWalk wk = imk_walk_make(grid, n_tiles, tiles_x * tiles_y, DYN);
    if (DYN && wk.shift != 5) return IMK_EINVAL;
    ImkProfScope prof(PF_CONV_PIPE, imk_conv_algorithmic_bytes(a), stream, imk_conv_flops(a));
    imk_klaunch(kern, dim3(grid), dim3(256), lds, stream, a, tiles_x, tiles_y, n_tiles, div_magic(tiles_x), wk);
    IMK_LAUNCH_CHECK();
    if (a.stats_rows) *a.stats_rows = grid;
    return IMK_OK;
}

template <int NC8, bool PAIR, bool FULL>
static int launch_conv_pipe_v(const ImkConvArgs &a, hipStream_t stream) {
    if (a.pre_wpk) {
        if constexpr (PAIR && NC8 == 1) {
            if (a.out) return IMK_EUNSUPPORTED;
            if (a.epi != EP_RELU || !a.wpk2 || a.x.lmode != LM_UPADD || a.x.cs_in != 8) return IMK_EUNSUPPORTED;
            return launch_conv_pipe_k<LM_UPADD, 1, 2, true, EP_RELU, false, FULL, 0, 1>(a, stream);
        } else {
            return IMK_EUNSUPPORTED;
        }
    }
    if (a.epi == EP_RELU) {
        const int chain = a.wpk2 ? (a.out ? 1 : 2) : 0;
#define IMK_PIPE_FWD(LM)                                                                              \
        (chain == 0 ? launch_conv_pipe_k<LM, NC8, 0, PAIR, EP_RELU, false, FULL>(a, stream)           \
         : chain == 1 ? launch_conv_pipe_k<LM, NC8, 1, PAIR, EP_RELU, false, FULL>(a, stream)         \
                      : launch_conv_pipe_k<LM, NC8, 2, PAIR, EP_RELU, false, FULL>(a, stream))
        switch (a.x.lmode) {
            case LM_RAW: return IMK_PIPE_FWD(LM_RAW);
            case LM_AFFINE: return IMK_PIPE_FWD(LM_AFFINE);
            case LM_POOL: return IMK_PIPE_FWD(LM_POOL);
            case LM_UPADD: return IMK_PIPE_FWD(LM_UPADD);
            case LM_U8: return IMK_PIPE_FWD(LM_U8);
            case LM_STEM:
                return chain == 2 ? launch_conv_pipe_k<LM_STEM, NC8, 2, PAIR, EP_RELU, false, FULL>(a, stream) : IMK_EUNSUPPORTED;
            default: return IMK_EUNSUPPORTED;
        }
#undef IMK_PIPE_FWD
    }
    if (a.wpk2) return IMK_EUNSUPPORTED;
    if (a.sum2_out) {
        if constexpr (FULL) {
            if (a.wg_partial || a.ksize != 1 || a.x.lmode != LM_BNBWD || a.epi != EP_PLAIN || !a.sum2_z || !a.stats_partial || a.dystat_z ||
                (a.H & 1) || (a.W & 1))
                return IMK_EUNSUPPORTED;
            return launch_conv_pipe_k<LM_BNBWD, NC8, 0, PAIR, EP_PLAIN, false, true, 4>(a, stream);
        } else {
            return IMK_EUNSUPPORTED;
        }
    }
    if (a.wg_partial) {
        if constexpr (FULL) {
            const bool dys = a.dystat_z && a.stats_partial;
            if (a.ksize == 3) {
                if (a.x.lmode == LM_RAW && a.epi == EP_PLAIN && dys && a.wg_sc && a.wg_sh)
                    return launch_conv_pipe_k<LM_RAW, NC8, 0, PAIR, EP_PLAIN, true, true, 3>(a, stream);
                return IMK_EUNSUPPORTED;
            }
            if (a.x.lmode == LM_BNBWD && a.epi == EP_MASK && !dys)
                return launch_conv_pipe_k<LM_BNBWD, NC8, 0, PAIR, EP_MASK, false, true, 1>(a, stream);
            if (a.x.lmode == LM_RAW && a.epi == EP_PLAIN && dys && a.wg_sc && a.wg_sh)
                return launch_conv_pipe_k<LM_RAW, NC8, 0, PAIR, EP_PLAIN, true, true, 2>(a, stream);
            return IMK_EUNSUPPORTED;
        } else {
            return IMK_EUNSUPPORTED;
        }
    }
    const bool dystat = a.dystat_z && a.stats_partial;
#define IMK_PIPE_BWD(LM)                                                                                         \
    (a.epi == EP_MASK ? (dystat ? launch_conv_pipe_k<LM, NC8, 0, PAIR, EP_MASK, true, FULL>(a, stream)           \
                                : launch_conv_pipe_k<LM, NC8, 0, PAIR, EP_MASK, false, FULL>(a, stream))         \
                      : (dystat ? launch_conv_pipe_k<LM, NC8, 0, PAIR, EP_PLAIN, true, FULL>(a, stream)          \
                                : launch_conv_pipe_k<LM, NC8, 0, PAIR, EP_PLAIN, false, FULL>(a, stream)))
    switch (a.x.lmode) {
        case LM_RAW: return IMK_PIPE_BWD(LM_RAW);
        case LM_BNBWD: return IMK_PIPE_BWD(LM_BNBWD);
        default: return IMK_EUNSUPPORTED;
    }
#undef IMK_PIPE_BWD
}

static int launch_conv_pipe_any(const ImkConvArgs &a, hipStream_t stream) {
    const bool all_ch = a.pair || (a.cs_out == 16 && (!a.wpk2 || a.cs_out2 == 16));
    const bool u8_ok = a.x.lmode != LM_U8 || a.pre_wpk || (a.ksize == 1 && ((uintptr_t)a.x.in & 15) == 0);
    const bool full = (a.H % 16 == 0) && (a.W % TW == 0) && all_ch && u8_ok;
    const bool nc1 = (a.pre_wpk ? imk_pad8(a.pre_cout) : a.x.cs_in) == 8;
#define IMK_PIPE_SEL(NC8)                                                                                   \
    (a.pair ? (full ? launch_conv_pipe_v<NC8, true, true>(a, stream) : launch_conv_pipe_v<NC8, true, false>(a, stream)) \
            : (full ? launch_conv_pipe_v<NC8, false, true>(a, stream) : launch_conv_pipe_v<NC8, false, false>(a, stream)))
    return nc1 ? IMK_PIPE_SEL(1) : IMK_PIPE_SEL(2);
#undef IMK_PIPE_SEL
}

template <int LM, int NC8, int MT, int EPI, bool DYSTAT, bool FULL, bool CHAIN2 = false>
static int launch_conv_wide_k(const ImkConvArgs &a, hipStream_t stream) {
    static int blocks_per_cu = 0;
    const int ns = ((a.ksize == 3 ? 9 : 1) * NC8 + 3) / 4;
    const size_t lds = (size_t)18 * 18 * imk_lds_pitch(NC8) * 16 + (4 * 32 + 4 * 2 * 16 * MT) * sizeof(float) + (size_t)MT * ns * 1024 +
                       (CHAIN2 ? (size_t)4 * 64 * 48 * sizeof(f16) : 0);
    auto kern = conv_wide_kernel<LM, NC8, MT, EPI, DYSTAT, FULL, CHAIN2>;
    { int r = set_lds_limit(kern, lds); if (r) return r; }
    if (blocks_per_cu == 0) {
        int nb = 0;
        if (hipOccupancyMaxActiveBlocksPerMultiprocessor(&nb, kern, 256, lds) != hipSuccess || nb < 1) nb = 2;
        blocks_per_cu = nb > 8 ? 8 : nb;
    }
    const int tiles_x = imk_cdiv(a.W, TW), tiles_y = imk_cdiv(a.H, 16);
    const int n_tiles = a.B * tiles_x * tiles_y;
    int grid = 256 * blocks_per_cu;
    if (grid > n_tiles) grid = n_tiles;
    const ImkWalk wk = imk_walk_make(grid, n_tiles, tiles_x * tiles_y);
    ImkProfScope prof(PF_CONV_PIPE, imk_conv_algorithmic_bytes(a), stream, imk_conv_flops(a));
    imk_klaunch(kern, dim3(grid), dim3(256), lds, stream, a, tiles_x, tiles_y, n_tiles, div_magic(tiles_x), wk);
    IMK_LAUNCH_CHECK();
    if (a.stats_rows) *a.stats_rows = grid;
    return IMK_OK;
}

template <int NC8, int MT, bool FULL>
static int launch_conv_wide_v(const ImkConvArgs &a, hipStream_t stream) {
    if (a.epi == EP_RELU) {
        switch (a.x.lmode) {
            case LM_RAW: return launch_conv_wide_k<LM_RAW, NC8, MT, EP_RELU, false, FULL>(a, stream);
            case LM_AFFINE: return launch_conv_wide_k<LM_AFFINE, NC8, MT, EP_RELU, false, FULL>(a, stream);
            case LM_UPADD: return launch_conv_wide_k<LM_UPADD, NC8, MT, EP_RELU, false, FULL>(a, stream);
            case LM_U8: if constexpr (NC8 == 1) return launch_conv_wide_k<LM_U8, 1, MT, EP_RELU, false, FULL>(a, stream); else return IMK_EUNSUPPORTED;
            default: return IMK_EUNSUPPORTED;
        }
    }
    const bool dystat = a.dystat_z && a.stats_partial;
#define IMK_WIDE_BWD(LM)                                                                                          \
    (a.epi == EP_MASK ? (dystat ? launch_conv_wide_k<LM, NC8, MT, EP_MASK, true, FULL>(a, stream)                 \
                                : launch_conv_wide_k<LM, NC8, MT, EP_MASK, false, FULL>(a, stream))               \
                      : (dystat ? launch_conv_wide_k<LM, NC8, MT, EP_PLAIN, true, FULL>(a, stream)                \
                                : launch_conv_wide_k<LM, NC8, MT, EP_PLAIN, false, FULL>(a, stream)))
    switch (a.x.lmode) {
        case LM_RAW: return IMK_WIDE_BWD(LM_RAW);
        case LM_BNBWD: return IMK_WIDE_BWD(LM_BNBWD);
        default: return IMK_EUNSUPPORTED;
    }
#undef IMK_WIDE_BWD
}

static bool conv_wide_ok(const ImkConvArgs &a) {
    if (!imk_switches().conv_wide || a.wpk2 || a.x.cs_in > 32 || a.cout > 32 || !pipe_fits(a)) return false;
    if (a.x.lmode == LM_POOL || a.x.lmode == LM_STEM) return false;
    if (a.x.lmode == LM_U8 && a.x.cin > 4) return false;
    return true;
}

static bool conv_wide_chain_ok(const ImkConvArgs &a) {
    const ImkSwitches &sw = imk_switches();
    if (!sw.wide_chain || !a.wpk2 || a.epi != EP_RELU || a.ksize != 3) return false;
    if ((a.out || a.stats_partial) && (!sw.wide_chain_train || a.cout2 > a.cout)) return false;
    if (a.x.cs_in < 16 || a.x.cs_in > 32 || a.cout > 32 || a.cout2 > 32 || (a.x.cs_in <= 16 && a.cout <= 16)) return false;
    if (a.x.lmode != LM_AFFINE) return false;
    ImkConvArgs plain = a;
    plain.wpk2 = nullptr;
    return conv_wide_ok(plain);
}
static int launch_conv_wide_chain(const ImkConvArgs &a, hipStream_t stream) {
    const bool full = (a.H % 16 == 0) && (a.W % TW == 0);
    const int nc8 = a.x.cs_in / 8;
    const bool mt2 = a.cout > 16;
#define IMK_WC(NC8V, MTV) (full ? launch_conv_wide_k<LM_AFFINE, NC8V, MTV, EP_RELU, false, true, true>(a, stream)  \
                                : launch_conv_wide_k<LM_AFFINE, NC8V, MTV, EP_RELU, false, false, true>(a, stream))
    switch (nc8) {
        case 2: return mt2 ? IMK_WC(2, 2) : IMK_EUNSUPPORTED;
        case 3: return mt2 ? IMK_WC(3, 2) : IMK_WC(3, 1);
        case 4: return mt2 ? IMK_WC(4, 2) : IMK_WC(4, 1);
        default: return IMK_EUNSUPPORTED;
    }
#undef IMK_WC
}

static int launch_conv_wide_any(const ImkConvArgs &a, hipStream_t stream) {
    const bool full = (a.H % 16 == 0) && (a.W % TW == 0);
    const int nc8 = a.x.cs_in / 8;
    const int mt = a.cout > 16 ? 2 : 1;
#define IMK_WIDE_SEL(NC8V, MTV) (full ? launch_conv_wide_v<NC8V, MTV, true>(a, stream) : launch_conv_wide_v<NC8V, MTV, false>(a, stream))
#define IMK_WIDE_MT(NC8V) (mt == 2 ? IMK_WIDE_SEL(NC8V, 2) : IMK_WIDE_SEL(NC8V, 1))
    switch (nc8) {
        case 1: return IMK_WIDE_MT(1);
        case 2: return IMK_WIDE_MT(2);
        case 3: return IMK_WIDE_MT(3);
        case 4: return IMK_WIDE_MT(4);
        default: return IMK_EUNSUPPORTED;
    }
#undef IMK_WIDE_MT
#undef IMK_WIDE_SEL
}

struct PipeChoice { bool ok, pair; };
static PipeChoice pipe_choice(const ImkConvArgs &a) {
    const bool ok = pipe_fits(a) && a.x.cs_in <= 16 && a.cout <= 16 && (a.x.lmode != LM_U8 || a.x.cin <= 4) &&
                    (!a.pre_wpk || imk_pad8(a.pre_cout) <= 16);
    return {ok, ok && a.cout <= 8};
}

bool imk_conv_pair_layout(int k_in, int m_out, bool u8_input) {
    return imk_pad8(k_in) <= 16 && m_out <= 8 && (!u8_input || k_in <= 4);
}

bool imk_conv_stem_fusable(int u8_c, int ch0, int cout_next) {
    return u8_c <= 4 && ch0 <= 16 && cout_next <= 16;
}

bool imk_conv_can_chain(const ImkConvArgs &a, int cout2) {
    const PipeChoice p = pipe_choice(a);
    if (!p.ok || (p.pair && cout2 > 8)) return false;
    return a.epi == EP_RELU && cout2 <= 16;
}

bool imk_conv_can_prestage(const ImkConvArgs &a, int lm_pre, int cin_pre, int cout_pre) {
    if (!imk_switches().conv_prestage || !pipe_fits(a)) return false;
    if (a.epi != EP_RELU || a.ksize != 3 || !a.wpk2 || a.out) return false;
    if (lm_pre != LM_UPADD || imk_pad8(cin_pre) != 8 || cout_pre > 8 || a.cout > 8 || a.cout2 > 8) return false;
    return imk_conv_pair_layout(cin_pre, cout_pre, false) && imk_conv_pair_layout(cout_pre, a.cout, false);
}

bool imk_conv_can_chain_tile(const ImkConvArgs &a, int cout2, bool store_mid) {
    const ImkSwitches &sw = imk_switches();
    if (sw.conv_chain_tile == 0) return false;
    ImkConvArgs plain = a;
    plain.wpk2 = nullptr;
    if (a.epi == EP_RELU && a.ksize == 3 && (a.x.lmode == LM_POOL || a.x.lmode == LM_AFFINE) && a.cout <= 128 &&
        cout2 <= 128 && imk_pad8(cout2) <= (a.cout > 64 ? 128 : 64) && sw.gemm_chain && imk_conv_gemm_ok(plain))
        return true;
    if ((sw.gemm_over_chain == 2 || (sw.gemm_over_chain == 1 && store_mid)) && imk_conv_gemm_ok(plain)) return false;
    if (pipe_choice(a).ok || a.epi != EP_RELU || a.ksize != 3 || a.cout > 64 || cout2 > 64) return false;
    if (a.x.lmode != LM_POOL && a.x.lmode != LM_AFFINE) return false;
    const bool wide = a.x.cs_in <= 32 && a.cout <= 32 && a.x.lmode != LM_POOL;
    const bool wide_chain = sw.wide_chain_train && wide && a.x.lmode == LM_AFFINE && a.x.cs_in >= 16 && cout2 <= a.cout && pipe_fits(a);
    if (sw.conv_chain_tile == 1 && wide && store_mid && !wide_chain && (long long)a.B * imk_cdiv(a.H, 16) * imk_cdiv(a.W, TW) > 2048)
        return false;
    const int mt1 = (a.cout + 15) / 16, mt2 = (cout2 + 15) / 16, mt = (mt1 <= 2 && mt2 <= 2) ? 2 : 4;
    return mt1 <= mt && mt2 <= mt && conv_tile_h(a.x.cs_in, 3) == 16;
}

bool imk_conv_can_fuse_wgrad(const ImkConvArgs &a) {
    const PipeChoice p = pipe_choice(a);
    if (!p.ok || a.wpk2) return false;
    const bool form1 = a.ksize == 1 && a.x.lmode == LM_BNBWD && a.epi == EP_MASK && a.mask && !(a.dystat_z && a.stats_partial);
    const bool form2 = a.x.lmode == LM_RAW && a.epi == EP_PLAIN && a.dystat_z && a.stats_partial;
    if (!form1 && !form2) return false;
    const bool all_ch = p.pair ? a.cs_out == 8 : a.cs_out == 16;
    return (a.H % 16 == 0) && (a.W % TW == 0) && all_ch;
}
int imk_conv_fused_wgrad_rows_max() { return 256 * 8; }

bool imk_conv_can_sum2(const ImkConvArgs &a) {
    const PipeChoice p = pipe_choice(a);
    if (!p.ok || a.wpk2 || a.wg_partial) return false;
    if (a.ksize != 1 || a.x.lmode != LM_BNBWD || a.epi != EP_PLAIN || (a.dystat_z && a.stats_partial)) return false;
    const bool all_ch = p.pair ? a.cs_out == 8 : a.cs_out == 16;
    return (a.H % 16 == 0) && (a.W % TW == 0) && all_ch;
}

int imk_launch_conv(const ImkConvArgs &a_in, hipStream_t stream) {
    ImkConvArgs a = a_in;
    IMK_CHECK_ARG(a.x.in && a.wpk && (a.out || a.wpk2) && a.B > 0 && a.H > 0 && a.W > 0);
    IMK_CHECK_ARG(a.ksize == 1 || a.ksize == 3);
    IMK_CHECK_ARG(a.x.cs_in % 8 == 0 && a.cs_out % 8 == 0 && a.x.cs_in >= a.x.cin && a.cs_out >= a.cout);
    IMK_CHECK_ARG(a.x.lmode != LM_U8 || (a.x.cs_in == 8 && a.x.cin <= 8));
    if (a.x.cs_in > 512) return IMK_EUNSUPPORTED;
    const PipeChoice p = pipe_choice(a);
    a.pair = p.pair;
    if (a.pre_wpk && !(p.ok && a.wpk2 && a.pre_bias && a.pre_sc && a.pre_sh && a.pre_cout > 0)) return IMK_EUNSUPPORTED;
    if (a.wpk2 && a.pair && a.cout2 > 8) return IMK_EUNSUPPORTED;
    if (a.wpk2) {
        if (a.epi != EP_RELU || !a.out2 || !a.bias2 || a.cs_out2 % 8) return IMK_EUNSUPPORTED;
        if (p.ok) return a.cout2 > 16 ? IMK_EUNSUPPORTED : launch_conv_pipe_any(a, stream);
        if (!imk_conv_can_chain_tile(a, a.cout2, a.out != nullptr)) return IMK_EUNSUPPORTED;
        if (conv_wide_chain_ok(a)) return launch_conv_wide_chain(a, stream);
        if (imk_conv_gemm_chain_ok(a)) return imk_launch_conv_gemm(a, stream);
        return launch_conv_mfma(a, stream);
    }
    if (p.ok) return launch_conv_pipe_any(a, stream);
    if (a.x.lmode == LM_STEM) return IMK_EUNSUPPORTED;
    if (conv_wide_ok(a)) return launch_conv_wide_any(a, stream);
    if (imk_conv_gemm_ok(a)) return imk_launch_conv_gemm(a, stream);
    return launch_conv_mfma(a, stream);
}

int imk_wgrad_splits(int B, int H, int W, int cin, int cout) {
    const int n_tiles = B * imk_cdiv(H, 16) * imk_cdiv(W, TW);
    const int n_pairs = ((imk_pad8(cin) + 15) / 16) * ((imk_pad8(cout) + 15) / 16);
    constexpr int target = 768;
    int s = target / n_pairs;
    if (s < 1) s = 1;
    if (s > n_tiles) s = n_tiles;
    return s;
}

size_t imk_wgrad_partial_floats(int B, int H, int W, int ksize, int cin, int cout) {
    const int n_pairs = ((imk_pad8(cin) + 15) / 16) * ((imk_pad8(cout) + 15) / 16);
    const int T = ksize == 3 ? 9 : 1;
    size_t ns = (size_t)imk_wgrad_splits(B, H, W, cin, cout);
    if (imk_pad8(cin) <= 16 && imk_pad8(cout) <= 16 && ns < (size_t)imk_conv_fused_wgrad_rows_max())
        ns = (size_t)imk_conv_fused_wgrad_rows_max();
    if (imk_wgrad_gemm_wide(imk_pad8(cin), imk_pad8(cout), (long long)B * H * W)) {
        for (int lm : {(int)LM_RAW, (int)LM_POOL, (int)LM_AFFINE}) {
            const size_t ng = (size_t)imk_wgrad_gemm_splits(lm, B, H, W, ksize, imk_pad8(cin), imk_pad8(cout));
            if (ns < ng) ns = ng;
        }
    }
    if (ksize == 1 && imk_pad8(cin) >= 24 && imk_pad8(cin) <= 64 && imk_pad8(cout) >= 24 && imk_pad8(cout) <= 64 &&
        ns < (size_t)imk_bwd1x1_rows((long long)B * H * W, imk_pad8(cin), imk_pad8(cout)))
        ns = (size_t)imk_bwd1x1_rows((long long)B * H * W, imk_pad8(cin), imk_pad8(cout));
    if (ksize == 1 && n_pairs <= 8 && ns < (size_t)imk_loss_blocks((long long)B * H * W)) ns = (size_t)imk_loss_blocks((long long)B * H * W);
    return (ns + (ns + WG_RED_CHUNK - 1) / WG_RED_CHUNK) * n_pairs * (T + 1) * 256;
}

struct WgradLaunch { ImkWgradGeom gm; int gx, gy; size_t lds; };

static int plan_wgrad(const ImkWgradArgs &a, WgradLaunch &L) {
    IMK_CHECK_ARG(a.x.in && a.dA && a.partial && a.B > 0 && a.H > 0 && a.W > 0 && a.n_split > 0);
    IMK_CHECK_ARG(a.ksize == 1 || a.ksize == 3);
    IMK_CHECK_ARG(a.x.cs_in % 8 == 0 && a.cs_out % 8 == 0);
    if (a.x.lmode == LM_BNBWD) return IMK_EUNSUPPORTED;
    if (a.x.lmode == LM_U8 && a.x.cin > 4) return IMK_EUNSUPPORTED;
    const int cit_n = (a.x.cs_in + 15) / 16, cot_n = (a.cs_out + 15) / 16;
    const int tiles_x = imk_cdiv(a.W, TW), tiles_y = imk_cdiv(a.H, 16);
    size_t lds = ((size_t)18 * 18 + 256) * WG_STRIDE_H * sizeof(f16) + (4 * (size_t)a.x.cs_in + 3 * (size_t)a.cs_out) * sizeof(float);
    const size_t red = 4 * (size_t)(a.ksize == 3 ? 10 : 2) * 256 * sizeof(float);
    if (lds < red) lds = red;
    L.gm = ImkWgradGeom{tiles_x, tiles_y, a.B * tiles_x * tiles_y, cit_n, cot_n, a.x.cs_in / 8, a.cs_out / 8, ImkWalk{}};
    L.gx = a.n_split; L.gy = cit_n * cot_n; L.lds = lds;
    {
        int g = a.n_split;
        L.gm.wk = imk_walk_make(g, L.gm.n_tiles, tiles_x * tiles_y);
        if (g != a.n_split) { g = a.n_split; L.gm.wk = ImkWalk{L.gm.n_tiles, 0, g, 0, 0}; }
    }
    return IMK_OK;
}

static double wgrad_algorithmic_bytes(const ImkWgradArgs &a, const WgradLaunch &L) {
    const double px = (double)a.B * a.H * a.W;
    double in_b;
    switch (a.x.lmode) {
        case LM_POOL: in_b = 4.0 * px * a.x.cs_in * 2; break;
        case LM_UPADD: in_b = 1.25 * px * a.x.cs_in * 2; break;
        case LM_U8: in_b = px * a.x.cin; break;
        default: in_b = px * a.x.cs_in * 2;
    }
    const int T = a.ksize == 3 ? 9 : 1;
    return in_b + px * a.cs_out * 2 * (a.dA_z ? 2 : 1) + (double)L.gx * L.gy * (T + 1) * 256 * 4;
}

int imk_launch_wgrad(const ImkWgradArgs &a, hipStream_t stream) {
    if (a.x.lmode == LM_U8 && a.ksize == 1 && a.dA_z && a.dA_coef && a.cs_out == 8 && a.x.cin <= 4 && a.n_split >= 1) {
        const long long n_pix = (long long)a.B * a.H * a.W;
        ImkProfScope prof(PF_WGRAD, (double)n_pix * (a.x.cin + 32) + (double)a.n_split * 2 * 1024, stream, imk_wgrad_flops(a));
        imk_klaunch(stem_wgrad_kernel, dim3(a.n_split), dim3(256), 0, stream, reinterpret_cast<const uint8_t *>(a.x.in), a.x.cin, a.x.u8_div, a.dA, a.dA_z, a.dA_coef,
                                                        n_pix, a.partial);
        IMK_LAUNCH_CHECK();
        return IMK_OK;
    }
    if (imk_wgrad_gemm_ok(a.x.lmode, a.dA_z != nullptr, a.ksize, a.x.cs_in, a.cs_out, (long long)a.B * a.H * a.W)) return imk_launch_wgrad_gemm(a, stream);
    WgradLaunch L{};
    int rc = plan_wgrad(a, L);
    if (rc) return rc;
    const dim3 grid(L.gx, L.gy);
    ImkProfScope prof(PF_WGRAD, wgrad_algorithmic_bytes(a, L), stream, imk_wgrad_flops(a));
    switch (a.x.lmode) {
#define IMK_WG(LM) do { if (a.ksize == 3) { if (a.dA_z) imk_klaunch(wgrad_mfma_kernel<LM, true, true>, dim3(grid), dim3(256), L.lds, stream, a, L.gm); \
                                           else imk_klaunch(wgrad_mfma_kernel<LM, false, true>, dim3(grid), dim3(256), L.lds, stream, a, L.gm); } \
                        else { if (a.dA_z) imk_klaunch(wgrad_mfma_kernel<LM, true, false>, dim3(grid), dim3(256), L.lds, stream, a, L.gm); \
                               else imk_klaunch(wgrad_mfma_kernel<LM, false, false>, dim3(grid), dim3(256), L.lds, stream, a, L.gm); } } while (0)
        case LM_RAW: IMK_WG(LM_RAW); break;
        case LM_AFFINE: IMK_WG(LM_AFFINE); break;
        case LM_POOL: IMK_WG(LM_POOL); break;
        case LM_UPADD: IMK_WG(LM_UPADD); break;
        default: IMK_WG(LM_U8); break;
#undef IMK_WG
    }
    IMK_LAUNCH_CHECK();
    return IMK_OK;
}

size_t imk_packed_conv_halfs(int ksize, int cin, int cout, int transposed, bool pair) {
    if (transposed == 2) return 512;
    const int T = ksize == 3 ? 9 : 1;
    const int m_dim = transposed ? cin : cout, k_dim = transposed ? cout : cin;
    const int nc8 = imk_pad8(k_dim) / 8;
    if (pair) return (size_t)(T == 9 ? 3 * nc8 : (nc8 + 1) / 2) * 512;
    const int nc8p = imk_pass_chunks(nc8);
    const int ns = imk_cdiv_d(nc8, nc8p) * ((T * nc8p + 3) / 4);
    return (size_t)((m_dim + 15) / 16) * ns * 512;
}
```

inconsistencymasks_amd/csrc/imk_gemm.hip:

```cpp
#include <cstdlib>
#include <type_traits>
#include "imk_stage.h"
#include "imk_switches.h"

IMK_STAMP_TABLE(gemm)

namespace {

constexpr int G_PM = 4, G_WM = 2, G_WN = 2;
constexpr int G_TH = G_PM * G_WM;
constexpr int G_BM = 16 * G_TH;

struct GemmGeom {
    int tiles_x, tiles_y, n_sp, gy, mt_total;
    int nc8, nc8p, n_pass, nsp, ns_total;
    int spp, cps, n_stage, ps;
    int nc8_2, nc8p_2, ns_2, mt_2;
};

template <int LM, bool KS3, int PN, bool NC4, bool CH2 = false, int AD = 1>
__global__ __launch_bounds__(256, 2) void conv_gemm_kernel(ImkConvArgs a, GemmGeom gm) {
    constexpr int NT = 256, PM = G_PM, WN = G_WN, TH = G_TH;
    constexpr int BN = 16 * PN * WN;
    constexpr int halo = KS3 ? 1 : 0, T = KS3 ? 9 : 1;
// ... 53 lines not shown
    auto commit = [&](int st, uint8_t *buf) {
#pragma unroll
        for (int u = 0; u < NX; ++u) {
            if (x_dst[u] >= 0) {
                const int c8 = min(st * cps + x_c8[u], nc8 - 1);
                f16x8 v = raw_transform<LM>(xr[u], s_aff, a.x.cs_in, c8, a.x.cin, a.x.u8_div);
                if (!(xok & (1u << u))) v = f16x8{0, 0, 0, 0, 0, 0, 0, 0};
                *reinterpret_cast<f16x8 *>(buf + x_dst[u]) = v;
            }
        }
    };

    const int ct0 = by * (BN / 16);
    const int wn_u = __builtin_amdgcn_readfirstlane(wn);
    const __amdgpu_buffer_rsrc_t wrsrc = __builtin_amdgcn_make_buffer_rsrc(const_cast<f16 *>(a.wpk), 0, 0x7fffffff, 0x00020000);
    int wso[PN];
#pragma unroll
    for (int m = 0; m < PN; ++m) {
        int ct = ct0 + wn_u * PN + m;
        if (ct >= gm.mt_total) ct = gm.mt_total - 1;
        wso[m] = ct * ns_total * 1024;
    }
    const int lane16 = lane * 16;
    typedef __attribute__((ext_vector_type(4))) unsigned int u32x4_t;
    auto loadA = [&](f16x8 (&af)[PN], int F) {
        const int fo = min(F, ns_total - 1) * 1024;
#pragma unroll
        for (int m = 0; m < PN; ++m) {
            const u32x4_t v = __builtin_amdgcn_raw_buffer_load_b128(wrsrc, lane16, wso[m] + fo, 0);
            af[m] = __builtin_bit_cast(f16x8, v);
        }
    };
    int base[PM];
#pragma unroll
    for (int p = 0; p < PM; ++p) base[p] = ((wm * PM + p) * WT + n) * ps * 16;
    f32x4 acc[PN][PM];
#pragma unroll
    for (int m = 0; m < PN; ++m)
#pragma unroll
        for (int p = 0; p < PM; ++p) acc[m][p] = f32x4{0, 0, 0, 0};
    auto mma = [&](const f16x8 (&af)[PN], const f16x8 (&bf)[PM]) {
#pragma unroll
        for (int p = 0; p < PM; ++p)
#pragma unroll
            for (int m = 0; m < PN; ++m) acc[m][p] = __builtin_amdgcn_mfma_f32_16x16x32_f16(af[m], bf[p], acc[m][p], 0, 0, 0);
    };

    const int n_stage = gm.n_stage;
    issue(0);
    f16x8 af[AD + 1][PN];
    f16x8 (&a0)[PN] = af[0], (&a1)[PN] = af[1];
    if constexpr (AD == 1) loadA(af[0], 0);
    __syncthreads();
    commit(0, s_tile0);
    issue(min(1, n_stage - 1));
    if constexpr (AD > 1) {
#pragma unroll
        for (int i = 0; i < AD; ++i) loadA(af[i], i);
    }
    __syncthreads();
    IMK_STAMP(1);
    const int mg_q = (65536 + nc8p - 1) / nc8p;
    int F = 0;
    using I0 = std::integral_constant<int, 0>; using I1 = std::integral_constant<int, 1>; using I2 = std::integral_constant<int, 2>;
    auto run_stage = [&](int st, const uint8_t *cur) {
        const int np = min(spp, gm.n_pass - st * spp);
        constexpr bool NK9 = KS3 && NC4 && AD > 1;
        const int nk = NK9 ? 9 : np * nsp;
        int pi = 0, s = 0;
        int bg[PM];
#pragma unroll
        for (int p = 0; p < PM; ++p) bg[p] = base[p] + (NC4 ? g * 16 : 0);
        auto loadB = [&](f16x8 (&bf)[PM]) {
            int off;
            if constexpr (NC4) {
                const int ty = KS3 ? (s * 11) >> 5 : 0, tx = KS3 ? s - 3 * ty : 0;
                off = ((ty * WT + tx) * ps + pi * 4) * 16;
                if (pi >= np) off = 0;
            } else {
                const int q = 4 * s + g;
                const int tap = (q * mg_q) >> 16, c8 = q - tap * nc8p;
                const int ty = KS3 ? (tap * 11) >> 5 : 0, tx = KS3 ? tap - 3 * ty : 0;
                const bool vq = (q < T * nc8p) && ((st * spp + pi) * nc8p + c8 < nc8) && (pi < np);
                off = vq ? ((ty * WT + tx) * ps + pi * nc8p + c8) * 16 : 0;
            }
#pragma unroll
            for (int p = 0; p < PM; ++p) bf[p] = *reinterpret_cast<const f16x8 *>(cur + bg[p] + off);
            if (++s == nsp) { s = 0; ++pi; }
        };
        if constexpr (AD > 1) {
            constexpr int NA = AD + 1, U = (NA % 2 == 0) ? NA : 2 * NA;
            f16x8 bb[2][PM];
            loadB(bb[0]);
            auto step = [&](auto U_T, int f) {
                constexpr int u = decltype(U_T)::value;
                loadA(af[(u + AD) % NA], F + f + u + AD);
                loadB(bb[(u + 1) & 1]);
                __builtin_amdgcn_sched_barrier(0);
                mma(af[u % NA], bb[u & 1]);
                __builtin_amdgcn_sched_barrier(0);
            };
            int f = 0;
            for (; f + U <= nk; f += U) {
                step(std::integral_constant<int, 0>{}, f); step(std::integral_constant<int, 1>{}, f);
                step(std::integral_constant<int, 2>{}, f); step(std::integral_constant<int, 3>{}, f);
                if constexpr (U == 6) { step(std::integral_constant<int, 4>{}, f); step(std::integral_constant<int, 5>{}, f); }
            }
            const int rem = nk - f;
            if (rem >= 1) {
                step(std::integral_constant<int, 0>{}, f);
                if (rem >= 2) {
                    step(std::integral_constant<int, 1>{}, f);
                    if (rem >= 3) {
                        step(std::integral_constant<int, 2>{}, f);
                        if constexpr (U == 6) {
                            if (rem >= 4) {
                                step(std::integral_constant<int, 3>{}, f);
                                if (rem >= 5) step(std::integral_constant<int, 4>{}, f);
                            }
                        }
                    }
                }
            }
            const int rot = nk % NA;
#pragma unroll
            for (int r = 1; r < NA; ++r) {
                if (rot == r) {
#pragma unroll
                    for (int m = 0; m < PN; ++m) {
                        f16x8 t[NA];
#pragma unroll
                        for (int i = 0; i < NA; ++i) t[i] = af[i][m];
#pragma unroll
                        for (int i = 0; i < NA; ++i) af[i][m] = t[(i + r) % NA];
                    }
                }
            }
            F += nk;
            return;
        }
        f16x8 b0[PM], b1[PM];
        loadB(b0);
        for (int f = 0; f < nk; f += 2) {
            loadA(a1, F + f + 1);
            loadB(b1);
            mma(a0, b0);
            loadA(a0, F + f + 2);
            loadB(b0);
            if (f + 1 < nk) mma(a1, b1);
        }
        if (nk & 1) {
#pragma unroll
            for (int m = 0; m < PN; ++m) a0[m] = a1[m];
        }
        F += nk;
    };
    for (int st = 0; st < n_stage; ++st) {
        const uint8_t *cur = (st & 1) ? s_tile1 : s_tile0;
        uint8_t *nxt = (st & 1) ? s_tile0 : s_tile1;
        if (st + 1 < n_stage) commit(st + 1, nxt);
        issue(min(st + 2, n_stage - 1));
        run_stage(st, cur);
        if (st == 0) IMK_STAMP(2);
        __syncthreads();
        if (st == 0) IMK_STAMP(3);
    }
    IMK_STAMP(4);

    constexpr int OP = BN + 8;
    f16 *s_out = reinterpret_cast<f16 *>(smem);
    const int cs_o = CH2 ? a.cs_out2 : a.cs_out;
    f16 *const out_t = CH2 ? a.out2 : a.out;
    {
        float bias[PN][4];
#pragma unroll
        for (int m = 0; m < PN; ++m)
#pragma unroll
            for (int r = 0; r < 4; ++r) {
                const int co = (ct0 + wn * PN + m) * 16 + 4 * g + r;
                bias[m][r] = (a.epi == EP_RELU && a.bias && co < a.cout) ? a.bias[co] : 0.f;
            }
        const bool relu = a.epi == EP_RELU;
#pragma unroll
        for (int m = 0; m < PN; ++m)
#pragma unroll
            for (int p = 0; p < PM; ++p) {
                f16x4 v;
#pragma unroll
                for (int r = 0; r < 4; ++r) v[r] = relu ? (f16)fmaxf(acc[m][p][r] + bias[m][r], 0.f) : (f16)acc[m][p][r];
                *reinterpret_cast<f16x4 *>(s_out + ((wm * PM + p) * 16 + n) * OP + (wn * PN + m) * 16 + 4 * g) = v;
            }
    }
    __syncthreads();
    if constexpr (CH2) {
        if (a.out) {
            constexpr int CPP1 = BN / 8, RPI1 = NT / CPP1, IT1 = G_BM / RPI1;
            const int cj1 = t % CPP1, prow1 = t / CPP1;
            if (cj1 * 8 < a.cs_out) {
                const unsigned pitch1 = (unsigned)a.cs_out * 2u;
                char *ob = const_cast<char *>(pix_base(a.out, tc.b, H, W, tc.ty0, tc.tx0, pitch1)) + cj1 * 16;
                const int my1 = H - 1 - tc.ty0, mx1 = W - 1 - tc.tx0;
#pragma unroll
                for (int k = 0; k < IT1; ++k) {
                    const int pixel = prow1 + k * RPI1, py = pixel >> 4, px = pixel & 15;
                    if (py <= my1 && px <= mx1)
                        *reinterpret_cast<f16x8 *>(ob + __umul24(__umul24(py, W) + px, pitch1)) = *reinterpret_cast<const f16x8 *>(s_out + pixel * OP + cj1 * 8);
                }
            }
        }
        f32x4 acc2[PN][PM];
#pragma unroll
        for (int m = 0; m < PN; ++m)
#pragma unroll
            for (int p = 0; p < PM; ++p) acc2[m][p] = f32x4{0, 0, 0, 0};
        for (int ks = 0; ks < gm.ns_2; ++ks) {
            int c8 = ks * gm.nc8p_2 + g;
            if (g >= gm.nc8p_2 || c8 >= gm.nc8_2) c8 = 0;
            f16x8 af[PN], bf[PM];
#pragma unroll
            for (int m = 0; m < PN; ++m) {
                const int mt = wn * PN + m;
                af[m] = f16x8{0, 0, 0, 0, 0, 0, 0, 0};
                if (mt < gm.mt_2) af[m] = *reinterpret_cast<const f16x8 *>(a.wpk2 + ((size_t)(mt * gm.ns_2 + ks) * 64 + lane) * 8);
            }
#pragma unroll
            for (int p = 0; p < PM; ++p) bf[p] = *reinterpret_cast<const f16x8 *>(s_out + ((wm * PM + p) * 16 + n) * OP + c8 * 8);
#pragma unroll
            for (int m = 0; m < PN; ++m)
#pragma unroll
                for (int p = 0; p < PM; ++p) acc2[m][p] = __builtin_amdgcn_mfma_f32_16x16x32_f16(af[m], bf[p], acc2[m][p], 0, 0, 0);
        }
        float bias2[PN][4];
#pragma unroll
        for (int m = 0; m < PN; ++m)
#pragma unroll
            for (int r = 0; r < 4; ++r) { const int co = (wn * PN + m) * 16 + 4 * g + r; bias2[m][r] = co < a.cout2 ? a.bias2[co] : 0.f; }
        __syncthreads();
#pragma unroll
        for (int m = 0; m < PN; ++m)
#pragma unroll
            for (int p = 0; p < PM; ++p) {
                f16x4 v;
#pragma unroll
                for (int r = 0; r < 4; ++r) v[r] = (f16)fmaxf(acc2[m][p][r] + bias2[m][r], 0.f);
                *reinterpret_cast<f16x4 *>(s_out + ((wm * PM + p) * 16 + n) * OP + (wn * PN + m) * 16 + 4 * g) = v;
            }
        __syncthreads();
    }
    IMK_STAMP(5);
    auto finish = [&](auto BNV_T) {
    constexpr int BNV = decltype(BNV_T)::value;
    constexpr int CPP = BNV / 8, RPI = NT / CPP, IT = G_BM / RPI;
    const int cj = t % CPP, prow = t / CPP;
    const int ch0 = ct0 * 16 + cj * 8;
    const bool ch_live = ch0 < cs_o;
    const int my = H - 1 - tc.ty0, mx = W - 1 - tc.tx0;
    const unsigned pitch = (unsigned)cs_o * 2u;
    const unsigned cho = ch_live ? (unsigned)ch0 * 2u : 0u;
    float s1[8], s2[8];
#pragma unroll
    for (int e = 0; e < 8; ++e) s1[e] = s2[e] = 0.f;
    auto sweep = [&](auto EPI_T, auto STAT_T) {
        constexpr int EPI = decltype(EPI_T)::value;
        constexpr int STAT = decltype(STAT_T)::value;
        char *ob = const_cast<char *>(pix_base(out_t, tc.b, H, W, tc.ty0, tc.tx0, pitch)) + cho;
        const char *mb = EPI == EP_MASK ? pix_base(a.mask, tc.b, H, W, tc.ty0, tc.tx0, pitch) + cho : nullptr;
        const char *zb = STAT == 2 ? pix_base(a.dystat_z, tc.b, H, W, tc.ty0, tc.tx0, pitch) + cho : nullptr;
        f16x8 mk[IT], zz[IT];
        unsigned off[IT];
#pragma unroll
        for (int k = 0; k < IT; ++k) {
            const int pixel = prow + k * RPI, py = pixel >> 4, px = pixel & 15;
            off[k] = __umul24(__umul24(min(py, my), W) + min(px, mx), pitch);
            if (EPI == EP_MASK) mk[k] = *reinterpret_cast<const f16x8 *>(mb + off[k]);
            if (STAT == 2) zz[k] = *reinterpret_cast<const f16x8 *>(zb + off[k]);
        }
#pragma unroll
        for (int k = 0; k < IT; ++k) {
            const int pixel = prow + k * RPI, py = pixel >> 4, px = pixel & 15;
            f16x8 v = *reinterpret_cast<const f16x8 *>(s_out + pixel * OP + cj * 8);
            if (EPI == EP_MASK) {
#pragma unroll
                for (int e = 0; e < 8; ++e) v[e] = ((float)mk[k][e] > 0.f) ? v[e] : (f16)0.f;
            }
            const bool live = ch_live && py <= my && px <= mx;
            if (live) *reinterpret_cast<f16x8 *>(ob + off[k]) = v;
            if (STAT) {
                const float lf = live ? 1.f : 0.f;
#pragma unroll
                for (int e = 0; e < 8; ++e) {
                    const float f = lf * (float)v[e];
                    s1[e] += f;
                    s2[e] += f * (STAT == 2 ? (float)zz[k][e] : f);
                }
            }
        }
    };
    const bool dystat = !CH2 && (a.epi != EP_RELU) && a.dystat_z && a.stats_partial;
    const bool want_stats = ((a.epi == EP_RELU) && a.stats_partial) || dystat;
    if (a.epi == EP_RELU) { if (want_stats) sweep(I0{}, I1{}); else sweep(I0{}, I0{}); }
    else if (a.epi == EP_MASK) { if (dystat) sweep(I2{}, I2{}); else sweep(I2{}, I0{}); }
    else { if (dystat) sweep(I1{}, I2{}); else sweep(I1{}, I0{}); }
    IMK_STAMP(6);
    if (want_stats) {
        __syncthreads();
        float *s_red = reinterpret_cast<float *>(smem);
#pragma unroll
        for (int e = 0; e < 8; ++e) {
            s_red[(0 * RPI + prow) * BNV + cj * 8 + e] = s1[e];
            s_red[(1 * RPI + prow) * BNV + cj * 8 + e] = s2[e];
        }
        __syncthreads();
        for (int i = t; i < 2 * BNV; i += NT) {
            const int which = i / BNV, c = i - which * BNV;
            const int co = ct0 * 16 + c;
            if (co < cs_o) {
                float v = 0.f;
                for (int r = 0; r < RPI; ++r) v += s_red[(which * RPI + r) * BNV + c];
                a.stats_partial[(size_t)sp * 2 * cs_o + which * cs_o + co] = v;
            }
        }
    }
    };
    if (CH2 && BN == 128 && cs_o <= 64) finish(std::integral_constant<int, 64>{});
    else finish(std::integral_constant<int, BN>{});
    IMK_STAMP_END(7);
}

inline int odd_up(int v) { return v | 1; }

int plan_conv_gemm(const ImkConvArgs &a, GemmGeom &gm, int &pn, size_t &lds, int &grid) {
    const int nc8 = a.x.cs_in / 8;
    const int nc8p = imk_pass_chunks(nc8), n_pass = imk_cdiv_d(nc8, nc8p);
    const bool ks3 = a.ksize == 3;
    const int T = ks3 ? 9 : 1;
    const int nsp = (T * nc8p + 3) / 4;
    const int spp = ks3 ? 1 : (8 / nc8p < n_pass ? 8 / nc8p : n_pass);
    const int cps = spp * nc8p;
    const int mt_total = (a.cout + 15) / 16;
    const int g128 = imk_cdiv_d(mt_total, 8), g64 = imk_cdiv_d(mt_total, 4);
    pn = (g128 * 8 <= g64 * 4) ? 4 : 2;
    if (a.wpk2) {
        pn = mt_total > 4 ? 4 : 2;
        const int nc8_2 = a.cs_out / 8;
        gm.nc8_2 = nc8_2; gm.nc8p_2 = imk_pass_chunks(nc8_2); gm.ns_2 = imk_cdiv_d(nc8_2, gm.nc8p_2);
        gm.mt_2 = (a.cout2 + 15) / 16;
    }
    const int bn = 16 * pn * G_WN;
    const int halo = ks3 ? 1 : 0;
    gm.tiles_x = imk_cdiv(a.W, TW); gm.tiles_y = imk_cdiv(a.H, G_TH);
    gm.n_sp = a.B * gm.tiles_x * gm.tiles_y;
    gm.gy = imk_cdiv_d(mt_total, bn / 16);
    gm.mt_total = mt_total;
    gm.nc8 = nc8; gm.nc8p = nc8p; gm.n_pass = n_pass; gm.nsp = nsp; gm.ns_total = n_pass * nsp;
    gm.spp = spp; gm.cps = cps; gm.n_stage = imk_cdiv_d(n_pass, spp); gm.ps = imk_lds_pitch(cps);
    const size_t tile_bytes = (size_t)(G_TH + 2 * halo) * (TW + 2 * halo) * gm.ps * 16;
    lds = 2 * tile_bytes + 4 * (size_t)a.x.cs_in * sizeof(float);
    const size_t out_bytes = (size_t)G_BM * (bn + 8) * sizeof(f16);
    const size_t red_bytes = 2 * (size_t)256 * 8 * sizeof(float);
    if (lds < out_bytes) lds = out_bytes;
    if (lds < red_bytes) lds = red_bytes;
    if (lds > 64 * 1024) return IMK_EUNSUPPORTED;
    grid = imk_cdiv_d(gm.n_sp, 8) * 8 * gm.gy;
    return IMK_OK;
}

int gemm_ad3_max_wgs() { return imk_switches().gemm_ad3_wgs; }

template <int LM, bool KS3, bool NC4> constexpr int gemm_deep_ad() { return (KS3 && NC4) || LM == LM_POOL || LM == LM_UPADD ? 2 : 3; }

template <int LM>
int launch_conv_gemm_chain(const ImkConvArgs &a, const GemmGeom &gm, int pn, size_t lds, int grid, hipStream_t stream) {
    if (grid <= gemm_ad3_max_wgs()) {
        if (gm.nc8p == 4) {
            constexpr int AD = gemm_deep_ad<LM, true, true>();
            if (pn == 4) imk_klaunch(conv_gemm_kernel<LM, true, 4, true, true, AD>, dim3(grid), dim3(256), lds, stream, a, gm);
            else imk_klaunch(conv_gemm_kernel<LM, true, 2, true, true, AD>, dim3(grid), dim3(256), lds, stream, a, gm);
        } else {
            constexpr int AD = gemm_deep_ad<LM, true, false>();
            if (pn == 4) imk_klaunch(conv_gemm_kernel<LM, true, 4, false, true, AD>, dim3(grid), dim3(256), lds, stream, a, gm);
            else imk_klaunch(conv_gemm_kernel<LM, true, 2, false, true, AD>, dim3(grid), dim3(256), lds, stream, a, gm);
        }
        return IMK_OK;
    }
    if (gm.nc8p == 4) {
        if (pn == 4) imk_klaunch(conv_gemm_kernel<LM, true, 4, true, true>, dim3(grid), dim3(256), lds, stream, a, gm);
        else imk_klaunch(conv_gemm_kernel<LM, true, 2, true, true>, dim3(grid), dim3(256), lds, stream, a, gm);
    } else {
        if (pn == 4) imk_klaunch(conv_gemm_kernel<LM, true, 4, false, true>, dim3(grid), dim3(256), lds, stream, a, gm);
        else imk_klaunch(conv_gemm_kernel<LM, true, 2, false, true>, dim3(grid), dim3(256), lds, stream, a, gm);
    }
    return IMK_OK;
}

template <int LM, bool KS3>
int launch_conv_gemm_k(const ImkConvArgs &a, const GemmGeom &gm, int pn, size_t lds, int grid, hipStream_t stream) {
    if (grid <= gemm_ad3_max_wgs()) {
        if (gm.nc8p == 4) {
            constexpr int AD = gemm_deep_ad<LM, KS3, true>();
            if (pn == 4) imk_klaunch(conv_gemm_kernel<LM, KS3, 4, true, false, AD>, dim3(grid), dim3(256), lds, stream, a, gm);
            else imk_klaunch(conv_gemm_kernel<LM, KS3, 2, true, false, AD>, dim3(grid), dim3(256), lds, stream, a, gm);
        } else {
            constexpr int AD = gemm_deep_ad<LM, KS3, false>();
            if (pn == 4) imk_klaunch(conv_gemm_kernel<LM, KS3, 4, false, false, AD>, dim3(grid), dim3(256), lds, stream, a, gm);
            else imk_klaunch(conv_gemm_kernel<LM, KS3, 2, false, false, AD>, dim3(grid), dim3(256), lds, stream, a, gm);
        }
        return IMK_OK;
    }
    if (gm.nc8p == 4) {
        if (pn == 4) imk_klaunch(conv_gemm_kernel<LM, KS3, 4, true>, dim3(grid), dim3(256), lds, stream, a, gm);
        else imk_klaunch(conv_gemm_kernel<LM, KS3, 2, true>, dim3(grid), dim3(256), lds, stream, a, gm);
    } else {
        if (pn == 4) imk_klaunch(conv_gemm_kernel<LM, KS3, 4, false>, dim3(grid), dim3(256), lds, stream, a, gm);
        else imk_klaunch(conv_gemm_kernel<LM, KS3, 2, false>, dim3(grid), dim3(256), lds, stream, a, gm);
    }
    return IMK_OK;
}

}

bool imk_conv_gemm_ok(const ImkConvArgs &a) {
    if (!imk_switches().conv_gemm) return false;
    if (a.wpk2 || a.pre_wpk || a.wg_partial) return false;
    if (a.x.cs_in <= 32 && a.cout <= 32) return false;
    if (a.x.cs_in > 512) return false;
    switch (a.x.lmode) {
        case LM_RAW: case LM_AFFINE: case LM_POOL: case LM_UPADD: case LM_BNBWD: break;
        default: return false;
    }
    if (a.epi == EP_RELU) { if (a.x.lmode == LM_BNBWD) return false; }
    else if (a.x.lmode != LM_RAW && a.x.lmode != LM_BNBWD) return false;
    return (long long)a.H * a.W < imk_conv_max_pixels() && a.W < (1 << 16);
}

bool imk_conv_gemm_chain_ok(const ImkConvArgs &a) {
    if (!imk_switches().gemm_chain || !a.wpk2 || !a.out2 || a.epi != EP_RELU || a.ksize != 3) return false;
    if (a.x.lmode != LM_POOL && a.x.lmode != LM_AFFINE) return false;
    if (a.cout > 128 || a.cout2 > 128 || a.cs_out2 > (a.cout > 64 ? 128 : 64)) return false;
    ImkConvArgs plain = a;
    plain.wpk2 = nullptr; plain.out = a.out2;
    return imk_conv_gemm_ok(plain);
}

int imk_conv_gemm_num_tiles(int B, int H, int W) { return B * imk_cdiv(H, G_TH) * imk_cdiv(W, TW); }

int imk_launch_conv_gemm(const ImkConvArgs &a, hipStream_t stream) {
    GemmGeom gm{};
    int pn = 4, grid = 0;
    size_t lds = 0;
    int rc = plan_conv_gemm(a, gm, pn, lds, grid);
    if (rc) return rc;
    ImkProfScope prof(PF_CONV_GEMM, imk_conv_algorithmic_bytes(a), stream, imk_conv_flops(a));
    const bool ks3 = a.ksize == 3;
    if (a.wpk2) {
        if (!imk_conv_gemm_chain_ok(a) || gm.gy != 1) return IMK_EUNSUPPORTED;
        rc = a.x.lmode == LM_POOL ? launch_conv_gemm_chain<LM_POOL>(a, gm, pn, lds, grid, stream)
                                  : launch_conv_gemm_chain<LM_AFFINE>(a, gm, pn, lds, grid, stream);
        if (rc) return rc;
        IMK_LAUNCH_CHECK();
        if (a.stats_rows) *a.stats_rows = gm.n_sp;
        return IMK_OK;
    }
#define IMK_GEMM_LM(LM) (ks3 ? launch_conv_gemm_k<LM, true>(a, gm, pn, lds, grid, stream) : launch_conv_gemm_k<LM, false>(a, gm, pn, lds, grid, stream))
    switch (a.x.lmode) {
        case LM_RAW: rc = IMK_GEMM_LM(LM_RAW); break;
        case LM_AFFINE: rc = IMK_GEMM_LM(LM_AFFINE); break;
        case LM_POOL: rc = IMK_GEMM_LM(LM_POOL); break;
        case LM_UPADD: rc = IMK_GEMM_LM(LM_UPADD); break;
        case LM_BNBWD: rc = IMK_GEMM_LM(LM_BNBWD); break;
        default: return IMK_EUNSUPPORTED;
    }
#undef IMK_GEMM_LM
    if (rc) return rc;
    IMK_LAUNCH_CHECK();
    if (a.stats_rows) *a.stats_rows = gm.n_sp;
    return IMK_OK;
}
```

inconsistencymasks_amd/csrc/imk_kernels.h:

```cpp
#pragma once
#include "imk_common.h"

enum ImkLoadMode {
    LM_RAW = 0,
    LM_AFFINE = 1,
    LM_POOL = 2,
    LM_UPADD = 3,
    LM_U8 = 4,
    LM_BNBWD = 5,
    LM_STEM = 6,
};
enum ImkEpilogue {
    EP_RELU = 0,
    EP_PLAIN = 1,
    EP_MASK = 2,
};

struct ImkInput {
    const void *in;
    const void *in2;
    const float *sc, *sh;
    const float *sc2, *sh2;
    int lmode;
    int cin, cs_in;
    float u8_div;
    int u8_c;
    int src_h, src_w;
};

#define IMK_SCHED_HEADS 32
#define IMK_SCHED_STRIDE 256
#define IMK_SCHED_BYTES (IMK_SCHED_HEADS * IMK_SCHED_STRIDE)
struct ImkConvArgs {
    ImkInput x;
    int B, H, W;
    int ksize;
    int cout, cs_out;
    const f16 *wpk;
    const float *bias;
    f16 *out;
    const f16 *mask;
    const f16 *wpk2;
    const float *bias2;
    f16 *out2;
    int cout2, cs_out2;
    const f16 *dystat_z;
    float *stats_partial;
    int *stats_rows;
    int epi;
    int pair;
    const f16 *pre_wpk;
    const float *pre_bias, *pre_sc, *pre_sh;
    int pre_cout;
    float *wg_partial;
    const float *wg_sc, *wg_sh;
    f16 *sum2_out;
    const f16 *sum2_z;
    unsigned *sched;
};
inline double imk_conv_flops(const ImkConvArgs &a) {
    const double px = (double)a.B * a.H * a.W;
    const int cin_main = a.pre_wpk ? a.pre_cout : a.x.cin;
    double f = 2.0 * px * (a.ksize == 3 ? 9 : 1) * cin_main * a.cout;
    if (a.wpk2) f += 2.0 * px * a.cout * a.cout2;
    if (a.pre_wpk) f += 2.0 * px * a.x.cin * a.pre_cout;
    return f;
}
bool imk_conv_can_fuse_wgrad(const ImkConvArgs &dgrad_args);
bool imk_conv_can_sum2(const ImkConvArgs &dgrad_args);
bool imk_conv_gemm_ok(const ImkConvArgs &a);
int imk_launch_conv_gemm(const ImkConvArgs &a, hipStream_t stream);
bool imk_conv_gemm_chain_ok(const ImkConvArgs &a);
int imk_conv_gemm_num_tiles(int B, int H, int W);
inline double imk_conv_algorithmic_bytes(const ImkConvArgs &a) {
    const double px = (double)a.B * a.H * a.W;
    double in_b;
    switch (a.x.lmode) {
        case LM_POOL: in_b = 4.0 * px * a.x.cs_in * 2; break;
        case LM_UPADD: in_b = px * a.x.cs_in * 2 + 0.25 * px * a.x.cs_in * 2; break;
        case LM_BNBWD: in_b = 2.0 * px * a.x.cs_in * 2; break;
        case LM_U8: in_b = px * a.x.cin; break;
        case LM_STEM: in_b = px * a.x.u8_c; break;
        default: in_b = px * a.x.cs_in * 2;
    }
    double out_b = (a.wpk2 && !a.out) ? 0.0 : px * a.cs_out * 2;
    if (a.wpk2) out_b += px * a.cs_out2 * 2;
    if (a.epi == EP_MASK) out_b += px * a.cs_out * 2;
    if (a.epi != EP_RELU && a.dystat_z) out_b += px * a.cs_out * 2;
    return in_b + out_b;
}
int imk_conv_fused_wgrad_rows_max();
int imk_conv_num_tiles(int B, int H, int W, int cs_in, int ksize);
int imk_launch_conv(const ImkConvArgs &a, hipStream_t stream);

struct ImkWgradArgs {
    ImkInput x;
    const f16 *dA;
    const f16 *dA_z;
    const float *dA_coef;
    int B, H, W, ksize, cout, cs_out;
    float *partial;
    int n_split;
};
inline double imk_wgrad_flops(const ImkWgradArgs &a) {
    return 2.0 * a.B * a.H * a.W * (a.ksize == 3 ? 9 : 1) * (double)a.x.cin * a.cout;
}
bool imk_bwd1x1_ok(int lmode, int cs_in, int cs_out, bool masked);
int imk_bwd1x1_rows(long long n_pix, int cs_in, int cs_out);
int imk_launch_bwd1x1(const ImkInput &x, const f16 *dy, const f16 *z, const float *coef, const f16 *wpk_bwd, f16 *dx,
                      float *wg_partial, int B, int H, int W, int cout, hipStream_t stream);
int imk_wgrad_splits(int B, int H, int W, int cin, int cout);
bool imk_wgrad_gemm_ok(int lmode, bool bnb, int ksize, int cs_in, int cs_out, long long pixels);
bool imk_wgrad_gemm_wide(int cs_in, int cs_out, long long pixels);
int imk_wgrad_gemm_splits(int lmode, int B, int H, int W, int ksize, int cs_in, int cs_out);
int imk_launch_wgrad_gemm(const ImkWgradArgs &a, hipStream_t stream);
size_t imk_wgrad_partial_floats(int B, int H, int W, int ksize, int cin, int cout);
int imk_launch_wgrad(const ImkWgradArgs &a, hipStream_t stream);

inline long long imk_conv_max_pixels() { return 1ll << 24; }
bool imk_conv_can_chain(const ImkConvArgs &first, int cout2);
bool imk_conv_can_prestage(const ImkConvArgs &main, int lm_pre, int cin_pre, int cout_pre);
bool imk_conv_can_chain_tile(const ImkConvArgs &first, int cout2, bool store_intermediate);
bool imk_conv_stem_fusable(int u8_c, int ch0, int cout_next);
bool imk_conv_pair_layout(int k_in, int m_out, bool u8_input);
size_t imk_packed_conv_halfs(int ksize, int cin, int cout, int transposed, bool pair);

#define IMK_PACK_MAX_JOBS 80
struct ImkPackJob { const float *w; f16 *dst; int ksize, cin, cout, transposed, pair; };
struct ImkCtl;
struct ImkPackJobs {
    ImkPackJob j[IMK_PACK_MAX_JOBS];
    int n;
    ImkCtl *ctl;
    const float *stats;
};
int imk_launch_pack_jobs(const ImkPackJobs &jobs, hipStream_t stream);

#define IMK_WGF_MAX_JOBS 32
struct ImkWgFinalJob {
    const float *partial;
    float *red;
    float *dw, *db;
    int n_split, n_chunks, chunk, n_tiles, T, cin, cout, cot_n;
    int work1_begin;
    int tile_begin;
};
struct ImkWgFinalJobs { ImkWgFinalJob j[IMK_WGF_MAX_JOBS]; int n, total_work1, total_tiles; };
int imk_wgf_add_job(ImkWgFinalJobs &jobs, float *partial, int n_split, int ksize, int cin, int cout, float *dw, float *db);
int imk_launch_wgrad_finalize_jobs(const ImkWgFinalJobs &jobs, const float *inv_scale_ptr, float *found_inf, hipStream_t stream);

struct ImkSelectArgs {
    const float *scores;
    const int32_t *counts;
    const uint8_t *cand;
    int n_models, batch, n_cand, n_heads, n_out, miou;
    long long cand_bytes;
    float thr;
    int32_t *best_idx;
    float *best_score;
    uint8_t *keep, *out;
    int gated;
};
int imk_launch_evalnet_select(const ImkSelectArgs &a, hipStream_t stream);
int imk_select_check(int n_models, int batch, int n_cand, int n_heads, int n_out, const int32_t *counts, const uint8_t *cand,
                     int64_t cand_bytes, int mode, const uint8_t *out, hipStream_t stream);
int imk_launch_repeat_rows(const uint8_t *src, int batch, int n_rep, long long row_bytes, uint8_t *dst, hipStream_t stream);

hipStream_t imk_side_pool_stream(int i);
```

inconsistencymasks_amd/csrc/imk_net.h:

```cpp
#pragma once
#include <algorithm>
#include <cstdlib>
#include <cstring>
#include <mutex>
#include <new>
#include "imk_elem.h"
#include "imk_kernels.h"
#include "imk_plan.h"


namespace {

constexpr size_t ALIGN = 256;
inline size_t up(size_t v) { return (v + ALIGN - 1) / ALIGN * ALIGN; }

inline int add_conv(imk_unet_plan *p, const char *name, int k, int cin, int cout, int res) {
    ImkLayer l{};
    l.name = name; l.kind = 0; l.ksize = k; l.cin = cin; l.cout = cout; l.res = res;
    p->layers.push_back(l);
    return (int)p->layers.size() - 1;
}
inline int add_bn(imk_unet_plan *p, const char *name, int c, int res, int producer) {
    ImkLayer l{};
    l.name = name; l.kind = 1; l.ksize = 0; l.cin = c; l.cout = c; l.res = res; l.producer = producer;
    p->layers.push_back(l);
    const int idx = (int)p->layers.size() - 1;
    p->layers[producer].bn_after = idx;
    return idx;
}
inline void set_src(imk_unet_plan *p, int conv, int lmode, int src, int src_bn = -1, int src2 = -1, int src2_bn = -1) {
    ImkLayer &l = p->layers[conv];
    l.lmode = lmode; l.src = src; l.src_bn = src_bn; l.src2 = src2; l.src2_bn = src2_bn;
}

inline void finish_layout(imk_unet_plan *p) {
    int64_t off = 0;
    for (auto &l : p->layers) {
        if (l.kind == 0) { l.off_w = off; off += (int64_t)l.ksize * l.ksize * l.cin * l.cout; l.off_b = off; off += l.cout; }
        else { l.off_w = off; off += l.cout; l.off_b = off; off += l.cout; }
        l.off_mean = l.off_var = -1;
    }
    p->n_trainable = off;
    for (auto &l : p->layers)
        if (l.kind == 1) { l.off_mean = off; off += l.cout; l.off_var = off; off += l.cout; }
    p->n_total = off;

    size_t pk = 0;
    for (auto &l : p->layers) {
        l.pk_fwd = l.pk_bwd = l.pk_chain = -1;
        if (l.kind == 0) {
            if (l.flags & IMK_LF_DENSE) continue;
            const bool u8 = l.lmode == LM_U8;
            l.pk_bytes_fwd = (int64_t)imk_packed_conv_halfs(l.ksize, l.cin, l.cout, 0, imk_conv_pair_layout(l.cin, l.cout, u8)) * 2;
            l.pk_bytes_bwd = (int64_t)imk_packed_conv_halfs(l.ksize, l.cin, l.cout, 1, imk_conv_pair_layout(l.cout, l.cin, false)) * 2;
            l.pk_fwd = (int64_t)pk; pk = up(pk + l.pk_bytes_fwd);
            l.pk_bwd = (int64_t)pk; pk = up(pk + l.pk_bytes_bwd);
            if (l.ksize == 1 && l.cin <= 16 && l.cout <= 16) { l.pk_chain = (int64_t)pk; pk = up(pk + 1024); }
        } else {
            l.pk_scale = (int64_t)pk; pk = up(pk + 2 * (size_t)imk_pad8(l.cout) * sizeof(float));
        }
    }
    p->packed_bytes = (int64_t)pk;
}

struct LayerWs {
    size_t out = 0;
    size_t dA = 0;
    size_t dy = 0;
    size_t stats_partial = 0;
    size_t scale = 0;
    size_t save = 0;
    size_t bwd_partial = 0;
    size_t coef = 0;
    size_t wg_partial = 0;
    int n_stats_tiles = 0;
    int n_bwd_rows = 0;
};
struct Ws {
    std::vector<LayerWs> L;
    size_t dU[4] = {0, 0, 0, 0};
    size_t dP[8] = {0, 0, 0, 0, 0, 0, 0, 0};
    size_t probs = 0, dlogit = 0, loss_partial = 0;
    size_t dice_partial = 0, dice_coef = 0, dice_val = 0;
    size_t cat = 0, dcat = 0;
    size_t dT[2][3] = {{0, 0, 0}, {0, 0, 0}};
    size_t onehot = 0;
    size_t head_partial = 0;
    size_t sched = 0;
    bool has_sched = false;
    size_t total = 0;
};

struct Dim { int h, w; };
inline Dim res_dim(const imk_unet_cfg &c, int res) { return Dim{c.h >> res, c.w >> res}; }

template <typename Take>
inline void make_ws_layers(const imk_unet_plan *p, int B, int mode, Ws &w, Take &&take) {
    const int n = (int)p->layers.size();
    w.L.resize(n);
    for (int i = 0; i < n; ++i) {
        const ImkLayer &l = p->layers[i];
        const Dim d = res_dim(p->cfg, l.res);
        const size_t px = (size_t)B * d.h * d.w;
        if (l.kind == 0) {
            if (l.flags & IMK_LF_DENSE) continue;
            if (!(l.flags & IMK_LF_HEAD)) w.L[i].out = take(px * imk_pad8(l.cout) * 2);
            if (mode == 1) {
                w.L[i].dA = take(px * imk_pad8(l.cout) * 2);
                w.L[i].wg_partial = take(imk_wgrad_partial_floats(B, d.h, d.w, l.ksize, l.cin, l.cout) * sizeof(float));
            }
        } else if (mode == 1) {
            const int cs = imk_pad8(l.cout);
            const ImkLayer &pc = p->layers[l.producer];
            w.L[i].n_stats_tiles = imk_conv_num_tiles(B, d.h, d.w, imk_pad8(pc.cin), pc.ksize);
            w.L[i].stats_partial = take((size_t)w.L[i].n_stats_tiles * 2 * cs * sizeof(float));
            w.L[i].scale = take(2 * (size_t)cs * sizeof(float));
            w.L[i].save = take(2 * (size_t)cs * sizeof(float));
            w.L[i].n_bwd_rows = imk_bn_prep_blocks(B, d.h, d.w, cs);
            const int conv_rows = B * imk_cdiv(d.h, 8) * imk_cdiv(d.w, 16);
            if (conv_rows > w.L[i].n_bwd_rows) w.L[i].n_bwd_rows = conv_rows;
            const int up_rows = std::min(imk_conv_fused_wgrad_rows_max(), B * imk_cdiv(2 * d.h, 16) * imk_cdiv(2 * d.w, 16));
            if (up_rows > w.L[i].n_bwd_rows) w.L[i].n_bwd_rows = up_rows;
            w.L[i].bwd_partial = take((size_t)w.L[i].n_bwd_rows * 2 * cs * sizeof(float));
            w.L[i].coef = take(3 * (size_t)cs * sizeof(float));
            w.L[i].dy = take(px * cs * 2);
        }
    }
}

struct Ctx {
    const imk_unet_plan *p;
    Ws ws;
    uint8_t *base;
    const float *params;
    const uint8_t *packed;
    int B;
    bool train;
    hipStream_t stream;
    const uint8_t *x_in[2] = {nullptr, nullptr};
    unsigned *sched(int conv) const {
        return (!train && ws.has_sched) ? reinterpret_cast<unsigned *>(base + ws.sched + IMK_SCHED_BYTES * (size_t)conv) : nullptr;
    }
    int ovr_conv = -1;
    f16 *ovr_out = nullptr;
    f16 *act(int conv) const { return conv == ovr_conv ? ovr_out : reinterpret_cast<f16 *>(base + ws.L[conv].out); }
    f16 *dA(int conv) const { return reinterpret_cast<f16 *>(base + ws.L[conv].dA); }
    f16 *dy(int bn) const { return reinterpret_cast<f16 *>(base + ws.L[bn].dy); }
    const float *bn_scale(int bn) const {
        return train ? reinterpret_cast<const float *>(base + ws.L[bn].scale)
                     : reinterpret_cast<const float *>(packed + p->layers[bn].pk_scale);
    }
    const float *bn_shift(int bn) const { return bn_scale(bn) + imk_pad8(p->layers[bn].cout); }
    const f16 *wfwd(int conv) const { return reinterpret_cast<const f16 *>(packed + p->layers[conv].pk_fwd); }
    const f16 *wbwd(int conv) const { return reinterpret_cast<const f16 *>(packed + p->layers[conv].pk_bwd); }
};

inline ImkInput conv_input(const Ctx &c, int conv) {
    const ImkLayer &l = c.p->layers[conv];
    ImkInput in{};
    in.cin = l.cin;
    in.cs_in = imk_pad8(l.cin);
    in.lmode = l.lmode;
    if (l.lmode == LM_U8) {
        in.in = c.x_in[l.src == IMK_SRC_XB ? 1 : 0];
        in.cs_in = 8;
        in.u8_div = (l.flags & IMK_LF_U8_RAW) ? 1.0f : 255.0f;
        return in;
    }
    in.in = l.src == IMK_SRC_CAT ? reinterpret_cast<const void *>(c.base + c.ws.cat)
          : l.src == IMK_SRC_ONEHOT ? reinterpret_cast<const void *>(c.base + c.ws.onehot) : c.act(l.src);
    if (l.src_bn >= 0) { in.sc = c.bn_scale(l.src_bn); in.sh = c.bn_shift(l.src_bn); }
    if (l.lmode == LM_POOL) { const Dim ds = res_dim(c.p->cfg, c.p->layers[l.src].res); in.src_h = ds.h; in.src_w = ds.w; }
    if (l.src2 >= 0) { in.in2 = c.act(l.src2); in.sc2 = c.bn_scale(l.src2_bn); in.sh2 = c.bn_shift(l.src2_bn); }
    return in;
}

inline int run_conv_fwd(Ctx &c, int conv, float *params_rw, int conv2 = -1, bool *fused = nullptr,
                        const ImkInput *x_override = nullptr) {
    const ImkLayer &l = c.p->layers[conv];
    const Dim d = res_dim(c.p->cfg, l.res);
    ImkConvArgs a{};
    a.x = x_override ? *x_override : conv_input(c, conv);
    a.B = c.B; a.H = d.h; a.W = d.w; a.ksize = l.ksize;
    a.cout = l.cout; a.cs_out = imk_pad8(l.cout);
    a.wpk = c.wfwd(conv);
    a.bias = c.params + l.off_b;
    a.out = c.act(conv);
    a.epi = EP_RELU;
    a.sched = c.sched(conv);
    int stat_conv = conv;
    if (fused) *fused = false;
    if (conv2 >= 0) {
        const ImkLayer &l2 = c.p->layers[conv2];
        const bool pipe_chain = l2.pk_chain >= 0 && imk_conv_can_chain(a, l2.cout);
        if (pipe_chain || (!x_override && l2.ksize == 1 && imk_conv_can_chain_tile(a, l2.cout, c.train || c.p->dbg_materialize))) {
            a.wpk2 = pipe_chain ? reinterpret_cast<const f16 *>(c.packed + l2.pk_chain) : c.wfwd(conv2);
            a.bias2 = c.params + l2.off_b;
            a.out2 = c.act(conv2);
            a.cout2 = l2.cout; a.cs_out2 = imk_pad8(l2.cout);
            if (!c.train && !c.p->dbg_materialize) a.out = nullptr;
            stat_conv = conv2;
            if (fused) *fused = true;
        }
    }
    if (x_override && !(a.wpk2 && !a.out)) return IMK_EUNSUPPORTED;
    const int bn = c.p->layers[stat_conv].bn_after;
    int rows = 0;
    if (c.train && bn >= 0) {
        a.stats_partial = reinterpret_cast<float *>(c.base + c.ws.L[bn].stats_partial);
        a.stats_rows = &rows;
    }
    int rc = imk_launch_conv(a, c.stream);
    if (rc) return rc;
    if (c.train && bn >= 0) {
        const ImkLayer &b = c.p->layers[bn];
        const int cs = imk_pad8(b.cout);
        float *sc = reinterpret_cast<float *>(c.base + c.ws.L[bn].scale);
        float *sv = reinterpret_cast<float *>(c.base + c.ws.L[bn].save);
        if (rows <= 0 || rows > c.ws.L[bn].n_stats_tiles) return IMK_EWORKSPACE;
        rc = imk_launch_bn_finalize(a.stats_partial, rows, b.cout, cs, (double)c.B * d.h * d.w,
                                    c.params + b.off_w, c.params + b.off_b, params_rw + b.off_mean, params_rw + b.off_var,
                                    sc, sc + cs, sv, sv + cs, c.stream, c.p->bn_momentum);
    }
    return rc;
}

inline int run_conv_pre_pair(Ctx &c, int pre, int c3, int c1) {
    if (c.train || c.p->dbg_materialize) return IMK_EUNSUPPORTED;
    const ImkLayer &lp = c.p->layers[pre], &l = c.p->layers[c3], &l2 = c.p->layers[c1];
    if (lp.ksize != 1 || lp.bn_after < 0 || l.src != pre || l.src_bn != lp.bn_after || l.lmode != LM_AFFINE || l2.pk_chain < 0)
        return IMK_EUNSUPPORTED;
    const Dim d = res_dim(c.p->cfg, l.res);
    ImkConvArgs a{};
    a.x = conv_input(c, pre);
    a.B = c.B; a.H = d.h; a.W = d.w; a.ksize = l.ksize;
    a.cout = l.cout; a.cs_out = imk_pad8(l.cout);
    a.wpk = c.wfwd(c3);
    a.bias = c.params + l.off_b;
    a.out = nullptr;
    a.epi = EP_RELU;
    a.sched = c.sched(c3);
    a.wpk2 = reinterpret_cast<const f16 *>(c.packed + l2.pk_chain);
    a.bias2 = c.params + l2.off_b;
    a.out2 = c.act(c1);
    a.cout2 = l2.cout; a.cs_out2 = imk_pad8(l2.cout);
    {
        ImkConvArgs plain = a;
        plain.x = conv_input(c, c3);
        if (!imk_conv_can_chain(plain, l2.cout)) return IMK_EUNSUPPORTED;
    }
    if (!imk_conv_can_prestage(a, lp.lmode, lp.cin, lp.cout)) return IMK_EUNSUPPORTED;
    a.pre_wpk = c.wfwd(pre);
    a.pre_bias = c.params + lp.off_b;
    a.pre_sc = c.bn_scale(lp.bn_after); a.pre_sh = c.bn_shift(lp.bn_after);
    a.pre_cout = lp.cout;
    return imk_launch_conv(a, c.stream);
}

inline int run_conv_pair(Ctx &c, int c3, int c1, float *params_rw) {
    bool f = false;
    int rc = run_conv_fwd(c, c3, params_rw, c1, &f);
    if (rc || f) return rc;
    return run_conv_fwd(c, c1, params_rw);
}

struct StateView { float *m, *v; ImkCtl *ctl; };
inline StateView state_view(const imk_unet_plan *p, void *state) {
    uint8_t *b = (uint8_t *)state;
    const size_t n = up((size_t)p->n_trainable * sizeof(float));
    return StateView{(float *)b, (float *)(b + n), (ImkCtl *)(b + 2 * n)};
}

struct Bwd {
    Ctx &c;
    float *grads;
    ImkCtl *ctl;
    float *found_inf;
    int n_side;
    ImkWgFinalJobs jobs{};
    int n_fork = 0;
    bool used_side[imk_unet_plan::MAX_SIDE] = {};

    int dy_rows[64] = {};
    int sum2_bn = -1;

    void grad_input(int conv, ImkInput &in) const {
        const ImkLayer &l = c.p->layers[conv];
        in.cin = l.cout; in.cs_in = imk_pad8(l.cout);
        const int bn = l.bn_after;
        if (bn >= 0) {
            in.in = c.dy(bn); in.in2 = c.act(conv); in.lmode = LM_BNBWD;
            in.sc = reinterpret_cast<const float *>(c.base + c.ws.L[bn].coef);
        } else {
            in.in = c.dA(conv); in.lmode = LM_RAW;
        }
    }
    void dgrad_args(int conv, f16 *dst, const f16 *mask, int stat_bn, int *rows, ImkConvArgs &a) const {
        const ImkLayer &l = c.p->layers[conv];
        const Dim d = res_dim(c.p->cfg, l.res);
        grad_input(conv, a.x);
        a.B = c.B; a.H = d.h; a.W = d.w; a.ksize = l.ksize;
        a.cout = l.cin; a.cs_out = imk_pad8(l.cin);
        a.wpk = c.wbwd(conv);
        a.out = dst;
        a.mask = mask;
        a.epi = mask ? EP_MASK : EP_PLAIN;
        if (stat_bn >= 0) {
            a.dystat_z = c.act(c.p->layers[stat_bn].producer);
            a.stats_partial = reinterpret_cast<float *>(c.base + c.ws.L[stat_bn].bwd_partial);
            a.stats_rows = rows;
        }
    }
    int dgrad_done(int stat_bn, int rows) {
        if (stat_bn >= 0) {
            if (rows <= 0 || rows > c.ws.L[stat_bn].n_bwd_rows) return IMK_EWORKSPACE;
            dy_rows[stat_bn] = rows;
        }
        return IMK_OK;
    }
    int dgrad(int conv, f16 *dst, const f16 *mask, int stat_bn = -1, int s2_bn = -1) {
        ImkConvArgs a{};
        int rows = 0;
        dgrad_args(conv, dst, mask, stat_bn, &rows, a);
        bool s2 = false;
        if (s2_bn >= 0 && stat_bn < 0 && !mask) {
            a.sum2_out = c.dy(s2_bn);
            a.sum2_z = c.act(c.p->layers[s2_bn].producer);
            a.stats_partial = reinterpret_cast<float *>(c.base + c.ws.L[s2_bn].bwd_partial);
            a.stats_rows = &rows;
            s2 = imk_conv_can_sum2(a);
            if (!s2) { a.sum2_out = nullptr; a.sum2_z = nullptr; a.stats_partial = nullptr; a.stats_rows = nullptr; }
        }
        int rc = imk_launch_conv(a, c.stream);
        if (rc) return rc;
        if (s2) return dgrad_done(s2_bn, rows);
        return dgrad_done(stat_bn, rows);
    }
    void wgrad_args(int conv, const f16 *dA_override, ImkWgradArgs &a) const {
        const ImkLayer &l = c.p->layers[conv];
        const Dim d = res_dim(c.p->cfg, l.res);
        a.x = conv_input(c, conv);
        if (dA_override) {
            a.dA = dA_override;
        } else {
            ImkInput gi{};
            grad_input(conv, gi);
            a.dA = reinterpret_cast<const f16 *>(gi.in);
            if (gi.lmode == LM_BNBWD) { a.dA_z = reinterpret_cast<const f16 *>(gi.in2); a.dA_coef = gi.sc; }
        }
        a.B = c.B; a.H = d.h; a.W = d.w; a.ksize = l.ksize; a.cout = l.cout; a.cs_out = imk_pad8(l.cout);
        a.partial = reinterpret_cast<float *>(c.base + c.ws.L[conv].wg_partial);
        a.n_split = imk_wgrad_splits(c.B, d.h, d.w, l.cin, l.cout);
        if (imk_wgrad_gemm_ok(a.x.lmode, a.dA_z != nullptr, l.ksize, a.x.cs_in, a.cs_out, (long long)c.B * d.h * d.w)) {
            a.n_split = imk_wgrad_gemm_splits(a.x.lmode, c.B, d.h, d.w, l.ksize, a.x.cs_in, a.cs_out);
            return;
        }
        if (l.ksize == 3 && l.lmode == LM_POOL) {
            constexpr int pool_wgs = 512;
            const int n_pairs = ((imk_pad8(l.cin) + 15) / 16) * ((imk_pad8(l.cout) + 15) / 16);
            a.n_split = std::max(1, std::min(a.n_split, pool_wgs / n_pairs));
        }
    }
    int wgrad_job(int conv, const ImkWgradArgs &a) {
        const ImkLayer &l = c.p->layers[conv];
        return imk_wgf_add_job(jobs, a.partial, a.n_split, l.ksize, l.cin, l.cout, grads + l.off_w, grads + l.off_b);
    }
    struct Pending { int conv; const f16 *dA_override; };
    Pending pending[8];
    int n_pending = 0;
    bool defer_finalize = false;
    int hold_conv = -1;
    Pending held{};
    bool has_held = false;
    bool tail_early = false;
    int launch_wgrad(int conv, const f16 *dA_override, hipStream_t ws) {
        ImkWgradArgs a{};
        wgrad_args(conv, dA_override, a);
        int rc = imk_launch_wgrad(a, ws);
        if (rc) return rc;
        return wgrad_job(conv, a);
    }
    int wgrad(int conv, const f16 *dA_override = nullptr, bool last = false) {
        const ImkLayer &l = c.p->layers[conv];
        if (n_side > 0 && conv == hold_conv) { held = Pending{conv, dA_override}; has_held = true; return IMK_OK; }
        if (n_side > 0) {
            if (n_pending == 8) { int rc = flush_wgrads(); if (rc) return rc; }
            pending[n_pending++] = Pending{conv, dA_override};
            return (l.res == 0 && !last) ? flush_wgrads() : IMK_OK;
        }
        return launch_wgrad(conv, dA_override, c.stream);
    }
    int flush_block() { return flush_wgrads(); }
    int flush_wgrads() {
        if (n_pending == 0) return IMK_OK;
        const int si = n_fork % n_side;
        hipStream_t ws = c.p->side[si];
        ImkStopRing *ring = imk_tls_stop_ring;
        if (ring && ring->stream == c.stream && ring->last) {
            IMK_HIP(hipStreamWaitEvent(ws, ring->last, 0));
            ++n_fork;
        } else {
            hipEvent_t ev = c.p->ev_fork[n_fork++];
            IMK_HIP(hipEventRecord(ev, c.stream));
            IMK_HIP(hipStreamWaitEvent(ws, ev, 0));
        }
        used_side[si] = true;
        for (int i = 0; i < n_pending; ++i) {
            int rc = launch_wgrad(pending[i].conv, pending[i].dA_override, ws);
            if (rc) return rc;
        }
        n_pending = 0;
        if (defer_finalize) return IMK_OK;
        int rc = imk_launch_wgrad_finalize_jobs(jobs, &ctl->inv_loss_scale, found_inf, ws);
        jobs = ImkWgFinalJobs{};
        return rc;
    }
    int wgrad_dgrad(int conv, f16 *dst, const f16 *mask, int stat_bn = -1) {
        const int s2_bn = sum2_bn;
        sum2_bn = -1;
        const ImkLayer &l = c.p->layers[conv];
        if (mask && stat_bn < 0 && l.ksize == 1 && l.lmode == LM_RAW && l.src >= 0 && mask == c.act(l.src)) {
            ImkConvArgs a{};
            int rows = 0;
            dgrad_args(conv, dst, mask, -1, nullptr, a);
            if (imk_conv_can_fuse_wgrad(a)) {
                a.wg_partial = reinterpret_cast<float *>(c.base + c.ws.L[conv].wg_partial);
                a.stats_rows = &rows;
                int rc = imk_launch_conv(a, c.stream);
                if (rc) return rc;
                if (rows <= 0 || rows > imk_conv_fused_wgrad_rows_max()) return IMK_EWORKSPACE;
                return imk_wgf_add_job(jobs, a.wg_partial, rows, l.ksize, l.cin, l.cout, grads + l.off_w, grads + l.off_b);
            }
        }
        if (stat_bn < 0 && l.ksize == 1 && l.bn_after >= 0 && l.src >= 0 &&
            ((l.lmode == LM_RAW && mask && mask == c.act(l.src)) || (l.lmode == LM_UPADD && !mask)) &&
            imk_bwd1x1_ok(l.lmode, imk_pad8(l.cin), imk_pad8(l.cout), mask != nullptr)) {
            const Dim d = res_dim(c.p->cfg, l.res);
            const int rows = imk_bwd1x1_rows((long long)c.B * d.h * d.w, imk_pad8(l.cin), imk_pad8(l.cout));
            float *wgp = reinterpret_cast<float *>(c.base + c.ws.L[conv].wg_partial);
            const int bn = l.bn_after;
            int rc = imk_launch_bwd1x1(conv_input(c, conv), c.dy(bn), c.act(conv), reinterpret_cast<const float *>(c.base + c.ws.L[bn].coef),
                                       c.wbwd(conv), dst, wgp, c.B, d.h, d.w, l.cout, c.stream);
            if (rc) return rc;
            return imk_wgf_add_job(jobs, wgp, rows, l.ksize, l.cin, l.cout, grads + l.off_w, grads + l.off_b);
        }
        if (!mask && stat_bn >= 0 && l.ksize == 3 && l.lmode == LM_AFFINE && l.src_bn == stat_bn &&
            l.src == c.p->layers[stat_bn].producer) {
            ImkConvArgs a{};
            int rows = 0;
            dgrad_args(conv, dst, nullptr, stat_bn, &rows, a);
            a.wg_sc = c.bn_scale(stat_bn); a.wg_sh = c.bn_shift(stat_bn);
            if (imk_conv_can_fuse_wgrad(a)) {
                a.wg_partial = reinterpret_cast<float *>(c.base + c.ws.L[conv].wg_partial);
                int rc = imk_launch_conv(a, c.stream);
                if (rc) return rc;
                rc = dgrad_done(stat_bn, rows);
                if (rc) return rc;
                if (rows > imk_conv_fused_wgrad_rows_max()) return IMK_EWORKSPACE;
                return imk_wgf_add_job(jobs, a.wg_partial, rows, l.ksize, l.cin, l.cout, grads + l.off_w, grads + l.off_b);
            }
        }
        const bool wide = imk_pad8(l.cin) >= 24 || imk_pad8(l.cout) >= 24;
        if (l.res == 0 && !tail_early && wide) {
            int rc = dgrad(conv, dst, mask, stat_bn, s2_bn);
            if (rc) return rc;
            return wgrad(conv);
        }
        int rc = wgrad(conv);
        if (rc) return rc;
        return dgrad(conv, dst, mask, stat_bn, s2_bn);
    }
    int finish_wgrads() {
        for (int i = 0; i < n_pending; ++i) {
            int rc = launch_wgrad(pending[i].conv, pending[i].dA_override, c.stream);
            if (rc) return rc;
        }
        n_pending = 0;
        for (int si = 0; si < n_side; ++si) {
            if (!used_side[si]) continue;
            IMK_HIP(hipEventRecord(c.p->ev_join[si], c.p->side[si]));
            IMK_HIP(hipStreamWaitEvent(c.stream, c.p->ev_join[si], 0));
        }
        return imk_launch_wgrad_finalize_jobs(jobs, &ctl->inv_loss_scale, found_inf, c.stream);
    }
    int bn_bwd(int bn, int mode, const f16 *g_direct, const f16 *g_other, int g_other_cs = 0) {
        const ImkLayer &b = c.p->layers[bn];
        const Dim d = res_dim(c.p->cfg, b.res);
        const int cs = imk_pad8(b.cout);
        const int prod = b.producer;
        const LayerWs &lw = c.ws.L[bn];
        float *partial = reinterpret_cast<float *>(c.base + lw.bwd_partial);
        float *coef = reinterpret_cast<float *>(c.base + lw.coef);
        const float *save = reinterpret_cast<const float *>(c.base + lw.save);
        const f16 *z = c.act(prod);
        int rows = dy_rows[bn];
        if (mode == 1 || rows == 0) {
            int rc = imk_launch_bn_bwd_prep(mode, mode == 0 ? c.dy(bn) : g_direct, g_other, z, c.bn_scale(bn), c.bn_shift(bn),
                                            c.dy(bn), partial, c.B, d.h, d.w, cs, c.stream, g_other_cs);
            if (rc) return rc;
            rows = imk_bn_prep_blocks(c.B, d.h, d.w, cs);
        }
        return imk_launch_bn_bwd_coef(partial, rows, b.cout, cs, (double)c.B * d.h * d.w, c.params + b.off_w, save, save + cs,
                                      &ctl->inv_loss_scale, coef, grads + b.off_w, grads + b.off_b, found_inf, c.stream);
    }
};

struct ImkStopRingScope {
    ImkStopRing ring{};
    ImkStopRing *prev = nullptr;
    bool on = false;
    ImkStopRingScope(const imk_unet_plan *plan, hipStream_t stream, int n_side) {
        if (n_side <= 0 || !plan->ev_ring[0]) return;
        ring = ImkStopRing{plan->ev_ring, 128, 0, stream, nullptr};
        prev = imk_tls_stop_ring;
        imk_tls_stop_ring = &ring;
        on = true;
// ... 58 lines not shown
```

inconsistencymasks_amd/csrc/imk_switches.cpp:

```cpp
#include "imk_switches.h"
#include <cstdlib>
#include "imk_plan.h"

namespace {
bool on_unless_zero(const char *name) {
    const char *e = getenv(name);
    return !(e && e[0] == '0');
}
int int_or(const char *name, int dflt) {
    const char *e = getenv(name);
    return e ? atoi(e) : dflt;
}
}

const ImkSwitches &imk_switches() {
    static const ImkSwitches s = []() {
        ImkSwitches v{};
        v.conv_wide = on_unless_zero("IMK_CONV_WIDE");
        v.conv_gemm = on_unless_zero("IMK_CONV_GEMM");
        v.conv_chain_tile = int_or("IMK_CONV_CHAIN_TILE", 1);
        v.conv_prestage = on_unless_zero("IMK_CONV_PRESTAGE");
        v.wide_chain = on_unless_zero("IMK_WIDE_CHAIN");
        v.wide_chain_train = on_unless_zero("IMK_WIDE_CHAIN_TRAIN");
        v.gemm_chain = on_unless_zero("IMK_GEMM_CHAIN");
        v.gemm_over_chain = int_or("IMK_GEMM_OVER_CHAIN", 1);
        v.gemm_ad3_wgs = int_or("IMK_GEMM_AD3_WGS", 1024);
        v.wgrad_gemm_min = int_or("IMK_WGRAD_GEMM_MIN", 0);
        v.wgrad_nfo2 = on_unless_zero("IMK_WGRAD_NFO2");
        v.student_fused = on_unless_zero("IMK_STUDENT_FUSED");
        v.consistency_fused = on_unless_zero("IMK_CONSISTENCY_FUSED");
        v.dice_fused = on_unless_zero("IMK_DICE_FUSED");
        v.select_shared = on_unless_zero("IMK_SELECT_SHARED");
        const int n = int_or("IMK_SIDE_STREAMS", 1);
        v.side_streams = n < 0 ? 0 : (n > imk_unet_plan::MAX_SIDE ? imk_unet_plan::MAX_SIDE : n);
        return v;
    }();
    return s;
}
```

inconsistencymasks_amd/csrc/imk_switches.h:

```cpp
#pragma once

struct ImkSwitches {
    bool conv_wide;
    bool conv_gemm;
    int conv_chain_tile;
    bool conv_prestage;
    bool wide_chain;
    bool wide_chain_train;
    bool gemm_chain;
    int gemm_over_chain;
    int gemm_ad3_wgs;
    int wgrad_gemm_min;
    bool wgrad_nfo2;
    bool student_fused;
    bool consistency_fused;
    bool dice_fused;
    bool select_shared;
    int side_streams;
};

const ImkSwitches &imk_switches();
```

inconsistencymasks_amd/csrc/imk_unet.hip:

```cpp
#include <atomic>
#include <cstdio>
#include <vector>
#include "imk_net.h"
#include "imk_head.h"
#include "imk_switches.h"

namespace {


struct Topo {
    int in_c, in_bn;
    int e_c3[4], e_c1[4], e_bn[4];
    int b_c3, b_c1, b_bn;
    int d_ca[4], d_bna[4], d_c3[4], d_c1[4], d_bnb[4];
    int out;
};

Topo make_topo(const imk_unet_plan *p) {
    Topo t{};
    t.in_c = p->find("in.c"); t.in_bn = p->find("in.bn");
    char nm[16];
    for (int i = 0; i < 4; ++i) {
        snprintf(nm, sizeof nm, "e%d.c3", i + 1); t.e_c3[i] = p->find(nm);
        snprintf(nm, sizeof nm, "e%d.c1", i + 1); t.e_c1[i] = p->find(nm);
        snprintf(nm, sizeof nm, "e%d.bn", i + 1); t.e_bn[i] = p->find(nm);
    }
    t.b_c3 = p->find("b.c3"); t.b_c1 = p->find("b.c1"); t.b_bn = p->find("b.bn");
    for (int j = 0; j < 4; ++j) {
        snprintf(nm, sizeof nm, "d%d.ca", j + 6); t.d_ca[j] = p->find(nm);
        snprintf(nm, sizeof nm, "d%d.bna", j + 6); t.d_bna[j] = p->find(nm);
        snprintf(nm, sizeof nm, "d%d.c3", j + 6); t.d_c3[j] = p->find(nm);
        snprintf(nm, sizeof nm, "d%d.c1", j + 6); t.d_c1[j] = p->find(nm);
        snprintf(nm, sizeof nm, "d%d.bnb", j + 6); t.d_bnb[j] = p->find(nm);
    }
    t.out = p->find("out");
    return t;
}

void build_layers(imk_unet_plan *p) {
    const int *ch = p->cfg.ch;
    int c = add_conv(p, "in.c", 1, p->cfg.c_in, ch[0], 0);
    add_bn(p, "in.bn", ch[0], 0, c);
    const int enc_in[4] = {ch[0], ch[0], ch[1], ch[2]};
    const int enc_f[4] = {ch[0], ch[1], ch[2], ch[3]};
    char nm[16];
    for (int i = 0; i < 4; ++i) {
        snprintf(nm, sizeof nm, "e%d.c3", i + 1); add_conv(p, nm, 3, enc_in[i], enc_f[i], i);
        snprintf(nm, sizeof nm, "e%d.c1", i + 1); c = add_conv(p, nm, 1, enc_f[i], enc_f[i], i);
        snprintf(nm, sizeof nm, "e%d.bn", i + 1); add_bn(p, nm, enc_f[i], i, c);
    }
    add_conv(p, "b.c3", 3, ch[3], ch[4], 4);
    c = add_conv(p, "b.c1", 1, ch[4], ch[3], 4);
    add_bn(p, "b.bn", ch[3], 4, c);
    const int dec_in[4] = {ch[3], ch[2], ch[1], ch[0]};
    const int dec_f1[4] = {ch[3], ch[2], ch[1], ch[0]};
    const int dec_f2[4] = {ch[2], ch[1], ch[0], ch[0]};
    for (int j = 0; j < 4; ++j) {
        const int res = 3 - j;
        snprintf(nm, sizeof nm, "d%d.ca", j + 6); c = add_conv(p, nm, 1, dec_in[j], dec_f1[j], res);
        snprintf(nm, sizeof nm, "d%d.bna", j + 6); add_bn(p, nm, dec_f1[j], res, c);
        snprintf(nm, sizeof nm, "d%d.c3", j + 6); add_conv(p, nm, 3, dec_f1[j], dec_f1[j], res);
        snprintf(nm, sizeof nm, "d%d.c1", j + 6); c = add_conv(p, nm, 1, dec_f1[j], dec_f2[j], res);
        snprintf(nm, sizeof nm, "d%d.bnb", j + 6); add_bn(p, nm, dec_f2[j], res, c);
    }
    c = add_conv(p, "out", 1, ch[0], p->cfg.n_out, 0);
    p->layers[c].flags = IMK_LF_HEAD;

    const Topo t = make_topo(p);
    set_src(p, t.in_c, LM_U8, IMK_SRC_XA);
    set_src(p, t.e_c3[0], LM_AFFINE, t.in_c, t.in_bn);
    for (int i = 1; i < 4; ++i) set_src(p, t.e_c3[i], LM_POOL, t.e_c1[i - 1], t.e_bn[i - 1]);
    for (int i = 0; i < 4; ++i) set_src(p, t.e_c1[i], LM_RAW, t.e_c3[i]);
    set_src(p, t.b_c3, LM_POOL, t.e_c1[3], t.e_bn[3]);
    set_src(p, t.b_c1, LM_RAW, t.b_c3);
    for (int j = 0; j < 4; ++j) {
        const int lo_c = j == 0 ? t.b_c1 : t.d_c1[j - 1], lo_bn = j == 0 ? t.b_bn : t.d_bnb[j - 1];
        set_src(p, t.d_ca[j], LM_UPADD, lo_c, lo_bn, t.e_c1[3 - j], t.e_bn[3 - j]);
        set_src(p, t.d_c3[j], LM_AFFINE, t.d_ca[j], t.d_bna[j]);
        set_src(p, t.d_c1[j], LM_RAW, t.d_c3[j]);
    }
    set_src(p, t.out, LM_AFFINE, t.d_c1[3], t.d_bnb[3]);
    finish_layout(p);
}

Ws make_ws(const imk_unet_plan *p, int B, int mode) {
    Ws w;
    const Topo t = make_topo(p);
    size_t off = 0;
    auto take = [&](size_t bytes) { size_t o = off; off = up(off + bytes); return o; };
    make_ws_layers(p, B, mode, w, take);
    if (mode == 0) { w.sched = take(IMK_SCHED_BYTES * p->layers.size()); w.has_sched = true; }

    if (mode == 1) {
        for (int j = 0; j < 4; ++j) {
            const ImkLayer &ca = p->layers[t.d_ca[j]];
            const Dim d = res_dim(p->cfg, ca.res);
            w.dU[j] = take((size_t)B * d.h * d.w * imk_pad8(ca.cin) * 2);
        }
        for (int i = 0; i < 4; ++i) {
            const ImkLayer &e = p->layers[t.e_c1[i]];
            const Dim d = res_dim(p->cfg, i + 1);
            w.dP[i] = take((size_t)B * d.h * d.w * imk_pad8(e.cout) * 2);
        }
        const size_t px = (size_t)B * p->cfg.h * p->cfg.w;
        w.dlogit = take(px * imk_pad8(p->cfg.n_out) * 2);
        w.loss_partial = take((size_t)imk_loss_blocks((long long)px) * sizeof(float));
        w.probs = take(px * p->cfg.n_out * sizeof(float));
        w.dice_partial = take((size_t)B * imk_dice_rows(B, p->cfg.h * p->cfg.w) * 3 * sizeof(float));
        w.dice_coef = take((size_t)B * 2 * sizeof(float));
        w.dice_val = take((size_t)B * sizeof(double));
    }
    w.total = off;
    return w;
}

int run_forward(Ctx &c, const Topo &t, float *probs, float *params_rw) {
    int rc;
    if (!c.train && c.ws.has_sched) IMK_HIP(hipMemsetAsync(c.base + c.ws.sched, 0, IMK_SCHED_BYTES * c.p->layers.size(), c.stream));
#define RUN(conv) do { rc = run_conv_fwd(c, (conv), params_rw); if (rc) return rc; } while (0)
#define RUN_PAIR(c3, c1) do { rc = run_conv_pair(c, (c3), (c1), params_rw); if (rc) return rc; } while (0)
    bool stem_fused = false;
    {
        const ImkLayer &st = c.p->layers[t.in_c], &c3 = c.p->layers[t.e_c3[0]];
        if (!c.train && !c.p->dbg_materialize && imk_conv_stem_fusable(st.cin, st.cout, c3.cout)) {
            ImkInput x{};
            x.in = c.x_in[0]; x.lmode = LM_STEM; x.cin = c3.cin; x.cs_in = imk_pad8(c3.cin); x.u8_c = st.cin;
            x.sc = c.bn_scale(t.in_bn); x.sh = c.bn_shift(t.in_bn);
            x.sc2 = c.params + st.off_w; x.sh2 = c.params + st.off_b;
            bool f = false;
            rc = run_conv_fwd(c, t.e_c3[0], params_rw, t.e_c1[0], &f, &x);
            if (rc == IMK_OK) stem_fused = true;
            else if (rc != IMK_EUNSUPPORTED) return rc;
        }
    }
    if (!stem_fused) { RUN(t.in_c); RUN_PAIR(t.e_c3[0], t.e_c1[0]); }
    for (int i = 1; i < 4; ++i) RUN_PAIR(t.e_c3[i], t.e_c1[i]);
    RUN_PAIR(t.b_c3, t.b_c1);
    for (int j = 0; j < 4; ++j) {
        rc = run_conv_pre_pair(c, t.d_ca[j], t.d_c3[j], t.d_c1[j]);
        if (rc == IMK_OK) continue;
        if (rc != IMK_EUNSUPPORTED) return rc;
        RUN(t.d_ca[j]); RUN_PAIR(t.d_c3[j], t.d_c1[j]);
    }
#undef RUN_PAIR
#undef RUN
    if (!probs) return IMK_OK;
    const ImkLayer &o = c.p->layers[t.out];
    const int bn = t.d_bnb[3];
    return imk_launch_head(c.act(t.d_c1[3]), c.bn_scale(bn), c.bn_shift(bn), c.params + o.off_w, c.params + o.off_b,
                           o.cin, imk_pad8(o.cin), o.cout, c.p->cfg.act_out, (long long)c.B * c.p->cfg.h * c.p->cfg.w,
                           probs, c.stream);
}

bool cfg_ok(const imk_unet_cfg *c) {
    if (!c) return false;
    if (c->h <= 0 || c->w <= 0 || (c->h % 16) || (c->w % 16)) return false;
    if (c->c_in < 1 || c->c_in > 8 || c->n_out < 1 || c->n_out > 64) return false;
    for (int i = 0; i < 5; ++i) if (c->ch[i] < 1 || c->ch[i] > 512) return false;
    if (imk_pad8(c->ch[0]) > 32) return false;
    return c->act_out == 0 || c->act_out == 1;
}

}

static std::atomic<int> g_runtime_warnings{0};
hipStream_t imk_side_pool_stream(int i) {
    struct Pool { std::mutex mu; hipStream_t s[imk_unet_plan::MAX_SIDE] = {}; };
    static Pool pools[64];
    if (i < 0 || i >= imk_unet_plan::MAX_SIDE) return nullptr;
    static std::once_flag hwq_once;
    std::call_once(hwq_once, []() {
        const char *e = getenv("GPU_MAX_HW_QUEUES");
        if (!e || atoi(e) < 8) {
            g_runtime_warnings.fetch_or(IMK_WARN_HW_QUEUES);
            fprintf(stderr, "libimk: GPU_MAX_HW_QUEUES=%s (< 8): side streams may serialise behind the caller's stream; "
                            "export GPU_MAX_HW_QUEUES=8 before the HIP runtime starts\n", e ? e : "unset");
        }
    });
    int dev = 0;
    (void)hipGetDevice(&dev);
    Pool &pool = pools[dev & 63];
    std::lock_guard<std::mutex> lock(pool.mu);
    if (!pool.s[i] && hipStreamCreateWithFlags(&pool.s[i], hipStreamNonBlocking) != hipSuccess) pool.s[i] = nullptr;
    return pool.s[i];
}

extern "C" int imk_runtime_warnings(void) { return g_runtime_warnings.load(); }

extern "C" int imk_unet_plan_side_stream(const imk_unet_plan *plan, int i, void **stream_out) {
    IMK_CHECK_ARG(plan && stream_out && i >= 0 && i < imk_unet_plan::MAX_SIDE);
    if (!ensure_side_streams(plan, i + 1)) return IMK_EINVAL;
    *stream_out = (void *)plan->side[i];
    return IMK_OK;
}

extern "C" int imk_unet_plan_create(const imk_unet_cfg *cfg, imk_unet_plan **out) {
    IMK_CHECK_ARG(out);
    if (!cfg_ok(cfg)) return IMK_EINVAL;
    if ((long long)cfg->h * cfg->w >= imk_conv_max_pixels() || cfg->w >= (1 << 16)) return IMK_EUNSUPPORTED;
    imk_unet_plan *p = new (std::nothrow) imk_unet_plan();
    if (!p) return IMK_EINVAL;
    p->cfg = *cfg;
    build_layers(p);
    *out = p;
    return IMK_OK;
}

extern "C" void imk_unet_plan_destroy(imk_unet_plan *plan) {
    if (!plan) return;
    for (int i = 0; i < imk_unet_plan::MAX_SIDE; ++i) {
        if (!plan->side[i]) continue;
        (void)hipStreamSynchronize(plan->side[i]);
        if (plan->ev_join[i]) (void)hipEventDestroy(plan->ev_join[i]);
    }
    for (auto &e : plan->ev_fork) if (e) (void)hipEventDestroy(e);
    for (auto &e : plan->ev_ring) if (e) (void)hipEventDestroy(e);
    delete plan;
}

extern "C" int imk_unet_param_count(const imk_unet_plan *plan, int64_t *total, int64_t *trainable) {
    IMK_CHECK_ARG(plan);
    if (total) *total = plan->n_total;
    if (trainable) *trainable = plan->n_trainable;
    return IMK_OK;
}

extern "C" int imk_unet_num_layers(const imk_unet_plan *plan) { return plan ? (int)plan->layers.size() : IMK_EINVAL; }

extern "C" int imk_unet_layer_info(const imk_unet_plan *plan, int idx, imk_layer_info *out) {
    IMK_CHECK_ARG(plan && out && idx >= 0 && idx < (int)plan->layers.size());
    const ImkLayer &l = plan->layers[idx];
    memset(out, 0, sizeof *out);
    strncpy(out->name, l.name.c_str(), sizeof(out->name) - 1);
    out->kind = l.kind; out->ksize = l.ksize; out->cin = l.cin; out->cout = l.cout;
    out->off_w = l.off_w; out->off_b = l.off_b; out->off_mean = l.off_mean; out->off_var = l.off_var;
    return IMK_OK;
}

extern "C" int imk_unet_plan_set_bn_momentum(imk_unet_plan *plan, float momentum) {
    IMK_CHECK_ARG(plan && momentum >= 0.f && momentum < 1.f);
    plan->bn_momentum = momentum;
    return IMK_OK;
}

extern "C" int imk_unet_plan_get_bn_momentum(const imk_unet_plan *plan, float *momentum) {
    IMK_CHECK_ARG(plan && momentum);
    *momentum = plan->bn_momentum;
    return IMK_OK;
}

extern "C" int imk_unet_plan_debug(imk_unet_plan *plan, int materialize, int single_stream) {
    IMK_CHECK_ARG(plan);
    if (materialize >= 0) plan->dbg_materialize = materialize != 0;
    if (single_stream >= 0) plan->dbg_single_stream = single_stream != 0;
    return IMK_OK;
}

extern "C" int64_t imk_unet_packed_bytes(const imk_unet_plan *plan) { return plan ? plan->packed_bytes : IMK_EINVAL; }


extern "C" int imk_unet_pack_weights(const imk_unet_plan *plan, const float *params, void *packed, void *stream_) {
    IMK_CHECK_ARG(plan && params && packed);
    IMK_HIP(hipMemsetAsync(packed, 0, (size_t)plan->packed_bytes, (hipStream_t)stream_));
    return pack_weights(plan, params, packed, (hipStream_t)stream_, nullptr, nullptr, true);
}

extern "C" int64_t imk_unet_workspace_bytes(const imk_unet_plan *plan, int batch, int mode) {
    if (!plan || batch <= 0 || (mode != 0 && mode != 1)) return IMK_EINVAL;
    return (int64_t)make_ws(plan, batch, mode).total;
}

extern "C" int imk_unet_forward(const imk_unet_plan *plan, const float *params, const void *packed, const uint8_t *x,
                                int batch, float *probs, void *workspace, int64_t workspace_bytes, void *stream_) {
    IMK_CHECK_ARG(plan && params && packed && x && probs && workspace && batch > 0);
    Ctx c{plan, make_ws(plan, batch, 0), (uint8_t *)workspace, params, (const uint8_t *)packed, batch, false,
          (hipStream_t)stream_};
    if ((int64_t)c.ws.total > workspace_bytes) return IMK_EWORKSPACE;
    c.x_in[0] = x;
    return run_forward(c, make_topo(plan), probs, nullptr);
}

extern "C" int imk_unet_tensor_info(const imk_unet_plan *plan, int batch, int mode, int layer_idx, int which,
                                    int64_t *byte_offset, int *h, int *w, int *c, int *c_stride) {
    IMK_CHECK_ARG(plan && batch > 0 && layer_idx >= 0 && layer_idx < (int)plan->layers.size());
    IMK_CHECK_ARG(mode == 0 || mode == 1);
    const Ws ws = make_ws(plan, batch, mode);
    const ImkLayer &l = plan->layers[layer_idx];
    const Dim d = res_dim(plan->cfg, l.res);
    size_t off = 0;
    if (which == 0 && l.kind == 0 && layer_idx != plan->find("out")) off = ws.L[layer_idx].out;
    else if (which == 1 && l.kind == 0 && mode == 1) off = ws.L[layer_idx].dA;
    else if (which == 2 && l.kind == 1 && mode == 1) off = ws.L[layer_idx].dy;
    else return IMK_EINVAL;
    if (byte_offset) *byte_offset = (int64_t)off;
    if (h) *h = d.h;
    if (w) *w = d.w;
    if (c) *c = l.cout;
    if (c_stride) *c_stride = imk_pad8(l.cout);
    return IMK_OK;
}

static size_t head_slab_bytes(const imk_unet_plan *plan, int batch, bool fused) {
    const imk_unet_cfg &cf = plan->cfg;
    const size_t px = (size_t)batch * cf.h * cf.w;
    const size_t probs = px * cf.n_out * sizeof(float), zlast = px * imk_pad8(cf.ch[0]) * sizeof(f16);
    return up(fused && zlast > probs ? zlast : probs);
}

extern "C" int64_t imk_unet_forward_im_workspace_bytes(const imk_unet_plan *plan, int n_models, int batch, int n_streams) {
    if (!plan || plan->net != 0 || n_models <= 0 || batch <= 0 || n_streams <= 0) return IMK_EINVAL;
    return (int64_t)(head_slab_bytes(plan, batch, true) * n_models + make_ws(plan, batch, 0).total * n_streams);
}

struct EnsembleHeads {
    const f16 **z;
    const float **sc, **sh, **w, **bias;
};

struct ForwardJob {
    int model, batch;
    const int64_t *gather;
    const Ws *ws;
    f16 *slab;
    float *probs;
};

static int run_ensemble_forwards(const imk_unet_plan *plan, const Topo &topo, const ForwardJob *jobs, int n_jobs,
                                 const float *const *params, const void *const *packed, const uint8_t *x, uint8_t *regions,
                                 size_t per_stream, size_t xbuf, int64_t regions_bytes, const EnsembleHeads *heads,
                                 hipStream_t main_stream) {
    const imk_unet_cfg &cf = plan->cfg;
    const int max_streams = 1 + imk_unet_plan::MAX_SIDE;
    int n_slabs = (int)((size_t)regions_bytes / per_stream);
    if (n_slabs > n_jobs) n_slabs = n_jobs;
    if (n_slabs > max_streams) n_slabs = max_streams;
    if (n_slabs > 1 && (plan->dbg_single_stream || !ensure_side_streams(plan, n_slabs - 1))) n_slabs = 1;
    if (n_slabs > 1) {
        IMK_HIP(hipEventRecord(plan->ev_fork[0], main_stream));
        for (int s = 1; s < n_slabs; ++s) IMK_HIP(hipStreamWaitEvent(plan->side[s - 1], plan->ev_fork[0], 0));
    }
    const ImkLayer &o = plan->layers[topo.out];
    const int64_t row_img = (int64_t)cf.h * cf.w * cf.c_in;
    for (int i = 0; i < n_jobs; ++i) {
        const ForwardJob &j = jobs[i];
        const int sl = i % n_slabs, m = j.model;
        hipStream_t st = sl == 0 ? main_stream : plan->side[sl - 1];
        uint8_t *region = regions + per_stream * sl;
        if (j.gather) {
            int rc = imk_gather_pairs(x, row_img, nullptr, 0, 0, 0, nullptr, j.gather, j.batch, region, nullptr, st);
            if (rc) return rc;
        }
        Ctx c{plan, *j.ws, region + xbuf, params[m], (const uint8_t *)packed[m], j.batch, false, st};
        c.x_in[0] = j.gather ? region : x;
        if (heads) {
            c.ovr_conv = topo.d_c1[3];
            c.ovr_out = j.slab;
            heads->z[m] = c.ovr_out;
            heads->sc[m] = c.bn_scale(topo.d_bnb[3]); heads->sh[m] = c.bn_shift(topo.d_bnb[3]);
            heads->w[m] = params[m] + o.off_w; heads->bias[m] = params[m] + o.off_b;
        }
        int rc = run_forward(c, topo, heads ? nullptr : j.probs, nullptr);
        if (rc) return rc;
    }
    for (int s = 1; s < n_slabs; ++s) {
        IMK_HIP(hipEventRecord(plan->ev_join[s - 1], plan->side[s - 1]));
        IMK_HIP(hipStreamWaitEvent(main_stream, plan->ev_join[s - 1], 0));
    }
    return IMK_OK;
}

static int run_ensemble_forwards(const imk_unet_plan *plan, const Topo &topo, const Ws &ws, int n_models, const float *const *params,
                                 const void *const *packed, const uint8_t *x, int batch, size_t slab, uint8_t *base,
                                 int64_t workspace_bytes, const EnsembleHeads *heads, hipStream_t main_stream) {
    const imk_unet_cfg &cf = plan->cfg;
    const size_t probs_exact = (size_t)batch * cf.h * cf.w * cf.n_out * sizeof(float);
    std::vector<ForwardJob> jobs;
    jobs.reserve(n_models);
    for (int m = 0; m < n_models; ++m)
        jobs.push_back({m, batch, nullptr, &ws, reinterpret_cast<f16 *>(base + slab * m), (float *)(base + probs_exact * m)});
    return run_ensemble_forwards(plan, topo, jobs.data(), n_models, params, packed, x, base + slab * n_models, ws.total, 0,
                                 workspace_bytes - (int64_t)(slab * n_models), heads, main_stream);
}

extern "C" int imk_unet_forward_im(const imk_unet_plan *plan, int n_models, const float *const *params,
                                   const void *const *packed, const uint8_t *x, int batch, float thr, int cmp_ge,
                                   const uint8_t *img, int block_in, int block_out, uint8_t *img_out, uint8_t *masks_out,
                                   uint8_t *im_out, int64_t *im_size, int64_t *pred_size, uint8_t *presence,
                                   void *workspace, int64_t workspace_bytes, void *stream_) {
    IMK_CHECK_ARG(plan && params && packed && x && workspace && batch > 0 && n_models > 0);
    const imk_unet_cfg &cf = plan->cfg;
    const Ws ws = make_ws(plan, batch, 0);
    const Topo topo = make_topo(plan);
    ImkHeadImArgs ha{};
    ha.n_models = n_models; ha.cin = cf.ch[0]; ha.cs = imk_pad8(cf.ch[0]); ha.K = cf.n_out; ha.softmax = cf.act_out;
// ... 621 lines not shown
```

Before: 25810 images/s.

## Fuse BN-affine 2x2 max-pool output into inference conv chain epilogues

During inference, encoder chain convs (3x3 then 1x1) now also write a half-resolution tensor that already has the next BatchNorm affine and 2x2 max-pool applied. Register shuffles and DPP handle this in the pipe kernel, and LDS sweeps handle it in the chain-tile and GEMM paths. The following layer then reads the pooled tensor as a plain raw input (LM_RAW with pooled=1) instead of pooling the full-resolution activation on load. This cuts the next conv's input traffic by a factor of four. In exchange it adds workspace buffers, extra epilogue work and stores, new template instantiations, and a raised occupancy hint of 5 in launch bounds for one variant.

Measured after the change: 25690 images/s. About the same (-0.5%).

```diff
diff --git a/inconsistencymasks_amd/csrc/imk_conv.hip b/inconsistencymasks_amd/csrc/imk_conv.hip
--- a/inconsistencymasks_amd/csrc/imk_conv.hip
+++ b/inconsistencymasks_amd/csrc/imk_conv.hip
@@ -311,6 +311,22 @@
         if (a.stats_partial) write_tile(I0{}, I1{}, acc2, bias2, a.cs_out2); else write_tile(I0{}, I0{}, acc2, bias2, a.cs_out2);
         __syncthreads();
         copy_out(a.out2, a.cs_out2);
+        if (a.pool_out) {
+            const int cpp = MT * 2, n_live = min(cpp, a.cs_out2 / 8);
+            const unsigned pitch = (unsigned)a.cs_out2 * 2u;
+            char *pb = const_cast<char *>(pix_base(a.pool_out, tc.b, H >> 1, W >> 1, tc.ty0 >> 1, tc.tx0 >> 1, pitch));
+            for (int i = t; i < (TH / 2) * 8 * cpp; i += NT) {
+                const int win = i / cpp, ch = i - win * cpp;
+                const int wy = win >> 3, wx = win & 7;
+                if (ch < n_live && 2 * wy <= my && 2 * wx <= mx) {
+                    const f16 *s0 = s_out + (2 * wy * 16 + 2 * wx) * OPITCH + ch * 8;
+                    const f16x8 z00 = *reinterpret_cast<const f16x8 *>(s0), z01 = *reinterpret_cast<const f16x8 *>(s0 + OPITCH);
+                    const f16x8 z10 = *reinterpret_cast<const f16x8 *>(s0 + 16 * OPITCH), z11 = *reinterpret_cast<const f16x8 *>(s0 + 17 * OPITCH);
+                    *reinterpret_cast<f16x8 *>(pb + __umul24(__umul24(wy, W >> 1) + wx, pitch) + ch * 16) =
+                        imk_affine_pool8(z00, z01, z10, z11, a.pool_sc + ch * 8, a.pool_sh + ch * 8);
+                }
+            }
+        }
         IMK_STAMP(5);
         if (a.stats_partial) reduce_stats(a.cs_out2);
     } else {
@@ -338,8 +354,8 @@
     return (b + 15) & ~(size_t)15;
 }
 
-template <int LM, int NC8, int CHAIN, bool PAIR, int EPI, bool DYSTAT, bool FULL, int WG = 0, int PRE = 0, bool DYN = false>
-__global__ __launch_bounds__(256, (DYN && NC8 == 1) ? IMK_INF_WAVES : 1) void conv_pipe_kernel(ImkConvArgs a, int tiles_x, int tiles_y, int n_tiles,
+template <int LM, int NC8, int CHAIN, bool PAIR, int EPI, bool DYSTAT, bool FULL, int WG = 0, int PRE = 0, bool DYN = false, bool POOLOUT = false>
+__global__ __launch_bounds__(256, (POOLOUT && PAIR && FULL && NC8 == 1 && LM != LM_POOL) ? 5 : ((DYN && NC8 == 1) ? IMK_INF_WAVES : 1)) void conv_pipe_kernel(ImkConvArgs a, int tiles_x, int tiles_y, int n_tiles,
                                                         unsigned magic_tx, ImkWalk wk) {
     static_assert(!DYN || (EPI == EP_RELU && !DYSTAT && WG == 0), "dynamic walk: results must not depend on the tile -> workgroup map");
     static_assert(PRE == 0 || (WG == 0 && EPI == EP_RELU && !DYSTAT && (LM == LM_U8 || LM == LM_UPADD)), "pre-stage: inference forward only");
@@ -347,6 +363,7 @@
     static_assert(WG != 2 || (LM == LM_RAW && CHAIN == 0 && EPI == EP_PLAIN && DYSTAT && FULL), "fused wgrad: 1x1 dgrad in front of a BatchNorm");
     static_assert(WG != 3 || (LM == LM_RAW && CHAIN == 0 && EPI == EP_PLAIN && DYSTAT && FULL), "fused wgrad: 3x3 dgrad in front of a BatchNorm");
     static_assert(WG != 4 || (LM == LM_BNBWD && CHAIN == 0 && EPI == EP_PLAIN && !DYSTAT && FULL && PRE == 0), "2x2-sum epilogue: 1x1 dgrad of a decoder's first conv");
+    static_assert(!POOLOUT || (CHAIN == 2 && EPI == EP_RELU && !DYSTAT && WG == 0 && PRE == 0 && LM != LM_U8), "pooled output: inference chains");
     constexpr int P = PAIR ? 2 : 4;
     constexpr int PS = imk_lds_pitch(NC8);
     constexpr int NCI = PRE ? PRE : NC8;
@@ -444,6 +461,7 @@
     unsigned valid = 0;
     constexpr bool U8ROWS = (LM == LM_U8) && FULL && !PRE;
     uint8_t *s_u8 = reinterpret_cast<uint8_t *>(s_red + 4 * 2 * 16);
+    float *s_pool = reinterpret_cast<float *>(s_u8);
     constexpr int NCX = PAIR ? 1 : 2, XS = NCX | 1;
     uint8_t *s_x = s_u8 + 1024;
     constexpr int MAX_XI = WG == 3 ? (18 * 18 * NCX + 255) / 256 : NCX;
@@ -513,6 +531,7 @@
         o1c[p] = lp * cso_b + co0 * 2;
         o2c[p] = lp * cso2_b + co0 * 2;
     }
+    const unsigned opc = POOLOUT ? (unsigned)(wave * 2 * (W >> 1) + (n >> 1)) * cso2_b + co0 * 2 : 0u;
 
     const int wgrp = imk_walk_range(wk, blockIdx.x);
     int tile = wgrp * wk.chunk + (int)(blockIdx.x >> wk.shift);
@@ -531,6 +550,9 @@
         if (tk_lane) s_tk[0] = tk;
     }
     stage_affine_table(a.x, s_aff);
+    if constexpr (POOLOUT) {
+        if (t < 16) { s_pool[t] = t < a.cs_out2 ? a.pool_sc[t] : 0.f; s_pool[16 + t] = t < a.cs_out2 ? a.pool_sh[t] : 0.f; }
+    }
     if constexpr (WG == 3) {
         if (t < a.cs_out) { s_aff[t] = a.wg_sc[t]; s_aff[16 + t] = a.wg_sh[t]; }
     }
@@ -726,6 +748,7 @@
             }
         }
         if (CHAIN) {
+            f16x4 pv[POOLOUT ? P : 1];
 #pragma unroll
             for (int p = 0; p < P; ++p) {
                 const f16x4 hv = imk_bias_relu4(acc[p], bias);
@@ -738,6 +761,37 @@
                     if (want_stats)
 #pragma unroll
                         for (int r = 0; r < 4; ++r) { const float f = (float)v[r]; s1[r] += f; s2[r] += f * f; }
+                }
+                if constexpr (POOLOUT) pv[p] = v;
+            }
+            if constexpr (POOLOUT) {
+                const f32x4 qsc = *reinterpret_cast<const f32x4 *>(s_pool + co0), qsh = *reinterpret_cast<const f32x4 *>(s_pool + 16 + co0);
+                f16x2 pw[P][2];
+#pragma unroll
+                for (int p = 0; p < P; ++p) {
+                    pw[p][0] = imk_affine2(f16x2{pv[p][0], pv[p][1]}, f32x2{qsc[0], qsc[1]}, f32x2{qsh[0], qsh[1]});
+                    pw[p][1] = imk_affine2(f16x2{pv[p][2], pv[p][3]}, f32x2{qsc[2], qsc[3]}, f32x2{qsh[2], qsh[3]});
+                }
+                char *b_po = const_cast<char *>(pix_base(a.pool_out, tc.b, H >> 1, W >> 1, tc.ty0 >> 1, tc.tx0 >> 1, cso2_b));
+#pragma unroll
+                for (int q = 0; q < 2; ++q) {
+                    unsigned wd[2];
+#pragma unroll
+                    for (int h = 0; h < 2; ++h) {
+                        f16x2 m;
+                        if constexpr (PAIR) {
+                            const unsigned mine = __builtin_bit_cast(unsigned, pw[q][h]);
+                            m = imk_pk_max(pw[q][h], __builtin_bit_cast(f16x2, (unsigned)__shfl_xor((int)mine, 32, 64)));
+                        } else {
+                            m = imk_pk_max(pw[2 * q][h], pw[2 * q + 1][h]);
+                        }
+                        const unsigned mu = __builtin_bit_cast(unsigned, m);
+                        const unsigned nb = (unsigned)__builtin_amdgcn_mov_dpp((int)mu, 0xB1, 0xF, 0xF, true);
+                        wd[h] = __builtin_bit_cast(unsigned, imk_pk_max(m, __builtin_bit_cast(f16x2, nb)));
+                    }
+                    const bool win_in = FULL || (wave * 4 + 2 * q <= H - 1 - tc.ty0 && (n & ~1) <= W - 1 - tc.tx0);
+                    if ((n & 1) == 0 && (!PAIR || set == 0) && lane_out && win_in)
+                        *reinterpret_cast<uint2 *>(b_po + (size_t)q * (W >> 1) * cso2_b + opc) = uint2{wd[0], wd[1]};
                 }
             }
         } else {
@@ -1841,6 +1895,7 @@
         if (L.gy != 1 || L.th != 16) return IMK_EUNSUPPORTED;
         if (a.x.lmode == LM_POOL) rc = L.mt == 4 ? launch(conv_mfma_kernel<16, 4, LM_POOL, true>) : launch(conv_mfma_kernel<16, 2, LM_POOL, true>);
         else if (a.x.lmode == LM_AFFINE) rc = L.mt == 4 ? launch(conv_mfma_kernel<16, 4, LM_AFFINE, true>) : launch(conv_mfma_kernel<16, 2, LM_AFFINE, true>);
+        else if (a.x.lmode == LM_RAW && a.x.pooled) rc = L.mt == 4 ? launch(conv_mfma_kernel<16, 4, LM_RAW, true>) : launch(conv_mfma_kernel<16, 2, LM_RAW, true>);
         else return IMK_EUNSUPPORTED;
         if (rc) return rc;
         if (a.stats_rows) *a.stats_rows = L.gx;
@@ -1871,16 +1926,17 @@
 
 constexpr int PIPE_BLOCKS_PER_CU = 8;
 
-template <int LM, int NC8, int CHAIN, bool PAIR, int EPI, bool DYSTAT, bool FULL, int WG = 0, int PRE = 0, bool DYN = false>
+template <int LM, int NC8, int CHAIN, bool PAIR, int EPI, bool DYSTAT, bool FULL, int WG = 0, int PRE = 0, bool DYN = false, bool POOLOUT = false>
 static int launch_conv_pipe_k(const ImkConvArgs &a, hipStream_t stream) {
     if constexpr (!DYN && EPI == EP_RELU && !DYSTAT && WG == 0) {
         if (a.sched && !a.stats_partial && a.B * imk_cdiv(a.H, 16) * imk_cdiv(a.W, TW) >= 2048)
-            return launch_conv_pipe_k<LM, NC8, CHAIN, PAIR, EPI, DYSTAT, FULL, WG, PRE, true>(a, stream);
-    }
+            return launch_conv_pipe_k<LM, NC8, CHAIN, PAIR, EPI, DYSTAT, FULL, WG, PRE, true, POOLOUT>(a, stream);
+    }
+    if (POOLOUT != (a.pool_out != nullptr)) return IMK_EINVAL;
     if (a.x.cs_in != (PRE ? PRE : NC8) * 8) return IMK_EINVAL;
     static int blocks_per_cu = 0;
     const size_t lds = pipe_lds_base(NC8, PAIR, WG) + (PRE ? (size_t)18 * 18 * imk_lds_pitch(PRE) * 16 + 3 * 16 * sizeof(float) : 0);
-    auto kern = conv_pipe_kernel<LM, NC8, CHAIN, PAIR, EPI, DYSTAT, FULL, WG, PRE, DYN>;
+    auto kern = conv_pipe_kernel<LM, NC8, CHAIN, PAIR, EPI, DYSTAT, FULL, WG, PRE, DYN, POOLOUT>;
     if (blocks_per_cu == 0) {
         int nb = 0;
         if (hipOccupancyMaxActiveBlocksPerMultiprocessor(&nb, kern, 256, lds) != hipSuccess || nb < 1) nb = 4;
@@ -1908,6 +1964,22 @@
             return launch_conv_pipe_k<LM_UPADD, 1, 2, true, EP_RELU, false, FULL, 0, 1>(a, stream);
         } else {
             return IMK_EUNSUPPORTED;
+        }
+    }
+    if (a.pool_out) {
+        if constexpr (PAIR && NC8 == 2) {
+            return IMK_EUNSUPPORTED;
+        } else {
+            if (a.epi != EP_RELU || !a.wpk2 || a.out || a.stats_partial || (a.H & 1) || (a.W & 1)) return IMK_EUNSUPPORTED;
+#define IMK_PIPE_POOL(LM) launch_conv_pipe_k<LM, NC8, 2, PAIR, EP_RELU, false, FULL, 0, 0, false, true>(a, stream)
+            switch (a.x.lmode) {
+                case LM_RAW: return IMK_PIPE_POOL(LM_RAW);
+                case LM_STEM:
+                    if constexpr (PAIR && !FULL) return IMK_EUNSUPPORTED;
+                    else return IMK_PIPE_POOL(LM_STEM);
+                default: return IMK_EUNSUPPORTED;
+            }
+#undef IMK_PIPE_POOL
         }
     }
     if (a.epi == EP_RELU) {
@@ -2034,7 +2106,7 @@
 
 static bool conv_wide_ok(const ImkConvArgs &a) {
     if (!imk_switches().conv_wide || a.wpk2 || a.x.cs_in > 32 || a.cout > 32 || !pipe_fits(a)) return false;
-    if (a.x.lmode == LM_POOL || a.x.lmode == LM_STEM) return false;
+    if (imk_route_lmode(a.x) == LM_POOL || a.x.lmode == LM_STEM) return false;
     if (a.x.lmode == LM_U8 && a.x.cin > 4) return false;
     return true;
 }
@@ -2114,13 +2186,14 @@
     if (sw.conv_chain_tile == 0) return false;
     ImkConvArgs plain = a;
     plain.wpk2 = nullptr;
-    if (a.epi == EP_RELU && a.ksize == 3 && (a.x.lmode == LM_POOL || a.x.lmode == LM_AFFINE) && a.cout <= 128 &&
+    const int rlm = imk_route_lmode(a.x);
+    if (a.epi == EP_RELU && a.ksize == 3 && (rlm == LM_POOL || rlm == LM_AFFINE) && a.cout <= 128 &&
         cout2 <= 128 && imk_pad8(cout2) <= (a.cout > 64 ? 128 : 64) && sw.gemm_chain && imk_conv_gemm_ok(plain))
         return true;
     if ((sw.gemm_over_chain == 2 || (sw.gemm_over_chain == 1 && store_mid)) && imk_conv_gemm_ok(plain)) return false;
     if (pipe_choice(a).ok || a.epi != EP_RELU || a.ksize != 3 || a.cout > 64 || cout2 > 64) return false;
-    if (a.x.lmode != LM_POOL && a.x.lmode != LM_AFFINE) return false;
-    const bool wide = a.x.cs_in <= 32 && a.cout <= 32 && a.x.lmode != LM_POOL;
+    if (rlm != LM_POOL && rlm != LM_AFFINE) return false;
+    const bool wide = a.x.cs_in <= 32 && a.cout <= 32 && rlm != LM_POOL;
     const bool wide_chain = sw.wide_chain_train && wide && a.x.lmode == LM_AFFINE && a.x.cs_in >= 16 && cout2 <= a.cout && pipe_fits(a);
     if (sw.conv_chain_tile == 1 && wide && store_mid && !wide_chain && (long long)a.B * imk_cdiv(a.H, 16) * imk_cdiv(a.W, TW) > 2048)
         return false;
@@ -2145,6 +2218,22 @@
     if (a.ksize != 1 || a.x.lmode != LM_BNBWD || a.epi != EP_PLAIN || (a.dystat_z && a.stats_partial)) return false;
     const bool all_ch = p.pair ? a.cs_out == 8 : a.cs_out == 16;
     return (a.H % 16 == 0) && (a.W % TW == 0) && all_ch;
+}
+
+bool imk_conv_can_pool_out(const ImkConvArgs &a) {
+    if (!imk_switches().pool_out || !a.wpk2 || !a.out2 || a.out || a.epi != EP_RELU || a.stats_partial || a.pre_wpk) return false;
+    if ((a.H & 1) || (a.W & 1) || a.ksize != 3) return false;
+    const PipeChoice p = pipe_choice(a);
+    if (p.ok) {
+        if (a.cout2 > 16 || (p.pair && (a.cout2 > 8 || a.x.cs_in > 8))) return false;
+        if (a.x.lmode != LM_RAW && a.x.lmode != LM_STEM) return false;
+        if (a.x.lmode == LM_STEM && p.pair && ((a.H % 16) || (a.W % TW))) return false;
+        return true;
+    }
+    if (!imk_conv_can_chain_tile(a, a.cout2, false) || conv_wide_chain_ok(a)) return false;
+    if (imk_conv_gemm_chain_ok(a)) return true;
+    const int rlm = imk_route_lmode(a.x);
+    return rlm == LM_POOL || a.x.lmode == LM_AFFINE;
 }
 
 int imk_launch_conv(const ImkConvArgs &a_in, hipStream_t stream) {
@@ -2158,6 +2247,7 @@
     a.pair = p.pair;
     if (a.pre_wpk && !(p.ok && a.wpk2 && a.pre_bias && a.pre_sc && a.pre_sh && a.pre_cout > 0)) return IMK_EUNSUPPORTED;
     if (a.wpk2 && a.pair && a.cout2 > 8) return IMK_EUNSUPPORTED;
+    if (a.pool_out && !(a.pool_sc && a.pool_sh && imk_conv_can_pool_out(a))) return IMK_EUNSUPPORTED;
     if (a.wpk2) {
         if (a.epi != EP_RELU || !a.out2 || !a.bias2 || a.cs_out2 % 8) return IMK_EUNSUPPORTED;
         if (p.ok) return a.cout2 > 16 ? IMK_EUNSUPPORTED : launch_conv_pipe_any(a, stream);
diff --git a/inconsistencymasks_amd/csrc/imk_gemm.hip b/inconsistencymasks_amd/csrc/imk_gemm.hip
--- a/inconsistencymasks_amd/csrc/imk_gemm.hip
+++ b/inconsistencymasks_amd/csrc/imk_gemm.hip
@@ -379,6 +379,22 @@
     else if (a.epi == EP_MASK) { if (dystat) sweep(I2{}, I2{}); else sweep(I2{}, I0{}); }
     else { if (dystat) sweep(I1{}, I2{}); else sweep(I1{}, I0{}); }
     IMK_STAMP(6);
+    if constexpr (CH2) {
+        if (a.pool_out) {
+            char *pb = const_cast<char *>(pix_base(a.pool_out, tc.b, H >> 1, W >> 1, tc.ty0 >> 1, tc.tx0 >> 1, pitch));
+            for (int i = t; i < (TH / 2) * 8 * CPP; i += NT) {
+                const int win = i / CPP, ch = i - win * CPP;
+                const int wy = win >> 3, wx = win & 7;
+                if (ch * 8 < cs_o && 2 * wy <= my && 2 * wx <= mx) {
+                    const f16 *s0 = s_out + (2 * wy * 16 + 2 * wx) * OP + ch * 8;
+                    const f16x8 z00 = *reinterpret_cast<const f16x8 *>(s0), z01 = *reinterpret_cast<const f16x8 *>(s0 + OP);
+                    const f16x8 z10 = *reinterpret_cast<const f16x8 *>(s0 + 16 * OP), z11 = *reinterpret_cast<const f16x8 *>(s0 + 17 * OP);
+                    *reinterpret_cast<f16x8 *>(pb + __umul24(__umul24(wy, W >> 1) + wx, pitch) + ch * 16) =
+                        imk_affine_pool8(z00, z01, z10, z11, a.pool_sc + ch * 8, a.pool_sh + ch * 8);
+                }
+            }
+        }
+    }
     if (want_stats) {
         __syncthreads();
         float *s_red = reinterpret_cast<float *>(smem);
@@ -512,7 +528,7 @@
 
 bool imk_conv_gemm_chain_ok(const ImkConvArgs &a) {
     if (!imk_switches().gemm_chain || !a.wpk2 || !a.out2 || a.epi != EP_RELU || a.ksize != 3) return false;
-    if (a.x.lmode != LM_POOL && a.x.lmode != LM_AFFINE) return false;
+    if (imk_route_lmode(a.x) != LM_POOL && a.x.lmode != LM_AFFINE) return false;
     if (a.cout > 128 || a.cout2 > 128 || a.cs_out2 > (a.cout > 64 ? 128 : 64)) return false;
     ImkConvArgs plain = a;
     plain.wpk2 = nullptr; plain.out = a.out2;
@@ -532,6 +548,7 @@
     if (a.wpk2) {
         if (!imk_conv_gemm_chain_ok(a) || gm.gy != 1) return IMK_EUNSUPPORTED;
         rc = a.x.lmode == LM_POOL ? launch_conv_gemm_chain<LM_POOL>(a, gm, pn, lds, grid, stream)
+           : a.x.lmode == LM_RAW  ? launch_conv_gemm_chain<LM_RAW>(a, gm, pn, lds, grid, stream)
                                   : launch_conv_gemm_chain<LM_AFFINE>(a, gm, pn, lds, grid, stream);
         if (rc) return rc;
         IMK_LAUNCH_CHECK();
diff --git a/inconsistencymasks_amd/csrc/imk_kernels.h b/inconsistencymasks_amd/csrc/imk_kernels.h
--- a/inconsistencymasks_amd/csrc/imk_kernels.h
+++ b/inconsistencymasks_amd/csrc/imk_kernels.h
@@ -26,7 +26,9 @@
     float u8_div;
     int u8_c;
     int src_h, src_w;
+    int pooled;
 };
+inline int imk_route_lmode(const ImkInput &x) { return (x.lmode == LM_RAW && x.pooled) ? (int)LM_POOL : x.lmode; }
 
 #define IMK_SCHED_HEADS 32
 #define IMK_SCHED_STRIDE 256
@@ -56,6 +58,8 @@
     const float *wg_sc, *wg_sh;
     f16 *sum2_out;
     const f16 *sum2_z;
+    f16 *pool_out;
+    const float *pool_sc, *pool_sh;
     unsigned *sched;
 };
 inline double imk_conv_flops(const ImkConvArgs &a) {
@@ -68,6 +72,7 @@
 }
 bool imk_conv_can_fuse_wgrad(const ImkConvArgs &dgrad_args);
 bool imk_conv_can_sum2(const ImkConvArgs &dgrad_args);
+bool imk_conv_can_pool_out(const ImkConvArgs &chain_args);
 bool imk_conv_gemm_ok(const ImkConvArgs &a);
 int imk_launch_conv_gemm(const ImkConvArgs &a, hipStream_t stream);
 bool imk_conv_gemm_chain_ok(const ImkConvArgs &a);
@@ -87,6 +92,7 @@
     if (a.wpk2) out_b += px * a.cs_out2 * 2;
     if (a.epi == EP_MASK) out_b += px * a.cs_out * 2;
     if (a.epi != EP_RELU && a.dystat_z) out_b += px * a.cs_out * 2;
+    if (a.pool_out) out_b += 0.25 * px * a.cs_out2 * 2;
     return in_b + out_b;
 }
 int imk_conv_fused_wgrad_rows_max();
diff --git a/inconsistencymasks_amd/csrc/imk_net.h b/inconsistencymasks_amd/csrc/imk_net.h
--- a/inconsistencymasks_amd/csrc/imk_net.h
+++ b/inconsistencymasks_amd/csrc/imk_net.h
@@ -65,6 +65,8 @@
 
 struct LayerWs {
     size_t out = 0;
+    size_t pool = 0;
+    bool has_pool = false;
     size_t dA = 0;
     size_t dy = 0;
     size_t stats_partial = 0;
@@ -144,6 +146,8 @@
     int ovr_conv = -1;
     f16 *ovr_out = nullptr;
     f16 *act(int conv) const { return conv == ovr_conv ? ovr_out : reinterpret_cast<f16 *>(base + ws.L[conv].out); }
+    bool pool_live[64] = {};
+    f16 *pooled(int conv) const { return reinterpret_cast<f16 *>(base + ws.L[conv].pool); }
     f16 *dA(int conv) const { return reinterpret_cast<f16 *>(base + ws.L[conv].dA); }
     f16 *dy(int bn) const { return reinterpret_cast<f16 *>(base + ws.L[bn].dy); }
     const float *bn_scale(int bn) const {
@@ -170,6 +174,12 @@
     in.in = l.src == IMK_SRC_CAT ? reinterpret_cast<const void *>(c.base + c.ws.cat)
           : l.src == IMK_SRC_ONEHOT ? reinterpret_cast<const void *>(c.base + c.ws.onehot) : c.act(l.src);
     if (l.src_bn >= 0) { in.sc = c.bn_scale(l.src_bn); in.sh = c.bn_shift(l.src_bn); }
+    if (l.lmode == LM_POOL && !c.train && l.src >= 0 && l.src < 64 && c.pool_live[l.src]) {
+        in.in = c.pooled(l.src);
+        in.lmode = LM_RAW; in.pooled = 1;
+        in.sc = in.sh = nullptr;
+        return in;
+    }
     if (l.lmode == LM_POOL) { const Dim ds = res_dim(c.p->cfg, c.p->layers[l.src].res); in.src_h = ds.h; in.src_w = ds.w; }
     if (l.src2 >= 0) { in.in2 = c.act(l.src2); in.sc2 = c.bn_scale(l.src2_bn); in.sh2 = c.bn_shift(l.src2_bn); }
     return in;
@@ -201,6 +211,12 @@
             if (!c.train && !c.p->dbg_materialize) a.out = nullptr;
             stat_conv = conv2;
             if (fused) *fused = true;
+            const int bn2 = l2.bn_after;
+            if (!a.out && conv2 < 64 && c.ws.L[conv2].has_pool && bn2 >= 0) {
+                a.pool_out = c.pooled(conv2);
+                a.pool_sc = c.bn_scale(bn2); a.pool_sh = c.bn_shift(bn2);
+                if (!imk_conv_can_pool_out(a)) { a.pool_out = nullptr; a.pool_sc = a.pool_sh = nullptr; }
+            }
         }
     }
     if (x_override && !(a.wpk2 && !a.out)) return IMK_EUNSUPPORTED;
@@ -212,6 +228,7 @@
     }
     int rc = imk_launch_conv(a, c.stream);
     if (rc) return rc;
+    if (a.pool_out) c.pool_live[conv2] = true;
     if (c.train && bn >= 0) {
         const ImkLayer &b = c.p->layers[bn];
         const int cs = imk_pad8(b.cout);
diff --git a/inconsistencymasks_amd/csrc/imk_switches.cpp b/inconsistencymasks_amd/csrc/imk_switches.cpp
--- a/inconsistencymasks_amd/csrc/imk_switches.cpp
+++ b/inconsistencymasks_amd/csrc/imk_switches.cpp
@@ -31,6 +31,7 @@
         v.consistency_fused = on_unless_zero("IMK_CONSISTENCY_FUSED");
         v.dice_fused = on_unless_zero("IMK_DICE_FUSED");
         v.select_shared = on_unless_zero("IMK_SELECT_SHARED");
+        v.pool_out = on_unless_zero("IMK_POOL_OUT");
         const int n = int_or("IMK_SIDE_STREAMS", 1);
         v.side_streams = n < 0 ? 0 : (n > imk_unet_plan::MAX_SIDE ? imk_unet_plan::MAX_SIDE : n);
         return v;
diff --git a/inconsistencymasks_amd/csrc/imk_switches.h b/inconsistencymasks_amd/csrc/imk_switches.h
--- a/inconsistencymasks_amd/csrc/imk_switches.h
+++ b/inconsistencymasks_amd/csrc/imk_switches.h
@@ -16,6 +16,7 @@
     bool consistency_fused;
     bool dice_fused;
     bool select_shared;
+    bool pool_out;
     int side_streams;
 };
 
diff --git a/inconsistencymasks_amd/csrc/imk_unet.hip b/inconsistencymasks_amd/csrc/imk_unet.hip
--- a/inconsistencymasks_amd/csrc/imk_unet.hip
+++ b/inconsistencymasks_amd/csrc/imk_unet.hip
@@ -90,6 +90,14 @@
     auto take = [&](size_t bytes) { size_t o = off; off = up(off + bytes); return o; };
     make_ws_layers(p, B, mode, w, take);
     if (mode == 0) { w.sched = take(IMK_SCHED_BYTES * p->layers.size()); w.has_sched = true; }
+    if (mode == 0 && imk_switches().pool_out) {
+        for (int i = 0; i < 4; ++i) {
+            const ImkLayer &e = p->layers[t.e_c1[i]];
+            const Dim d = res_dim(p->cfg, i + 1);
+            w.L[t.e_c1[i]].pool = take((size_t)B * d.h * d.w * imk_pad8(e.cout) * 2);
+            w.L[t.e_c1[i]].has_pool = true;
+        }
+    }
 
     if (mode == 1) {
         for (int j = 0; j < 4; ++j) {
```
